# jacketsj/expANN

Measured on AMD Instinct MI355X. Metric: queries/sec at recall@10=1.0 (exact brute force), 1Mxd128 fp32, k=10, higher is better.
Workload: dtype f32; 1 GPU; brute_force_engine L2 N=1000000 d=128 fp32, 10000 batched queries, k=10 (BASELINE configs[1]); n=1000000, d=128, m=10000, k=10, metric=l2, launch=one process, one GPU, devices_visible=1, comm_ranks=0

## Files before the change

### expann_amd/csrc/expann_hip.hip

```cpp
#include "../../include/expann_hip.h"

#include <hip/hip_runtime.h>

#include <algorithm>
#include <cmath>
#include <cstdio>
#include <cstdlib>
#include <cstring>
#include <memory>
#include <mutex>
#include <string>
#include <vector>

#include "host_common.hpp"
#include "scan_f32.hpp"
#include "scan_gemm_bf16.hpp"
#include "scan_gemm_f16.hpp"
#include "scan_gemm_f16k.hpp"
#include "scan_gemm_f16x.hpp"
#include "scan_gemm_f16y.hpp"
#include "scan_gemm_f16kx.hpp"
#include "scan_gemm_f16kl.hpp"
#include "scan_direct_f16.hpp"
#include "scan_gemm_i8.hpp"
#include "scan_gemm_i8q.hpp"
#include "scan_gemm_i8x.hpp"
#include "scan_gemm_i8w.hpp"
#include "scan_int8.hpp"
#include "scan_int8_any.hpp"
#include "scan_gemm_i8kl.hpp"
#include "filter_rows.hpp"
#include "score_ids.hpp"
#include "select.hpp"

using namespace expann;

namespace expann {
thread_local std::string g_create_error;
}

namespace {

constexpr uint32_t kMaxCap = 16384;
static_assert(kMaxK == kMaxCap / 2, "the bound on k: a candidate list holds at least 2k keys");
constexpr size_t kMaxQueriesPerPass = 32768;
constexpr int kEventPairs = 64;
constexpr uint32_t kAsyncRing = 256;
constexpr uint32_t kRingWords = 10, kRingScale = 8, kRingMark = 9;
constexpr size_t kFlagCopyBytes = sizeof(uint32_t) * 7;
constexpr uint32_t kFilterListCap = kMaxCap;

struct Level {
	uint32_t n_groups_sel;
	uint32_t group_stride;
	uint32_t classmin_blocks = 0;
	uint32_t list_rows = 0;
	uint32_t list_step = 1;
};

}

struct expann_index {
	int dim = 0, dtype = 0, metric = 0, device = 0;
	size_t elem = 4;
	size_t q_elem = 4;
	int int_mode = -1;
	GrowPtr<uint8_t> d_q8;
	std::vector<unsigned char> staging;
	size_t n_staged = 0;
	void* d_base = nullptr;
	bool owns_base = false;
	size_t n = 0;
	uint64_t id_offset = 0;
	hipStream_t stream = nullptr;
	GrowPtr<uint64_t> d_cand;
	DevPtr<uint32_t> d_cnt;
	DevPtr<float> d_tau[2];
	DevPtr<float> d_tau_s;
	GrowPtr<void> d_redo;
	DevPtr<uint32_t> d_tau_row[2];
	size_t m_alloc = 0;
	DevPtr<uint32_t> d_overflow;
	unsigned long long* d_total = nullptr;
	PinPtr<uint32_t> h_flags;
	PinPtr<void> h_pin;
	bool q_in_pinned_host = false;
	DevPtr<uint32_t> d_ticket;
	size_t h_pin_bytes = 0;
	DevPtr<float> d_bnorm;
	DevPtr<float> d_bnorm_bf;
	DevPtr<float> d_bnmax;
	DevPtr<void> d_base_split;
	int u8_exact = 0;
	expann_index* u8_shadow = nullptr;
	DevPtr<void> d_base_u8;
	bool strict_u8 = false;
	double prof_extra_ms = 0;
	long opt_u8_exact = 1;
	void* d_base_i8q = nullptr;
	bool base_i8q_owned = false;
	DevPtr<int> d_bp_i8q;
	DevPtr<void> d_log;
	DevPtr<uint32_t> d_log_cnt;
	DevPtr<uint32_t> d_work_ctr;
	size_t log_bytes = 0, log_cnt_n = 0;
	struct {
		uint32_t n_logs = 0, log_cap = 0, cap = 0, n_chunks = 0, n_qtiles = 0, xcd_map = 0, m = 0;
		const float* theta = nullptr;
		float key_mul = 0.0f;
		const int *i_thp = nullptr, *i_bias = nullptr, *i_qself = nullptr;
		int i_mode = 0;
		const float* i_rw = nullptr;
	} pending_scatter;
	GrowPtr<float> d_sample;
	GrowPtr<void> d_q_split;
	DevPtr<void> d_base_f16;
	DevPtr<float> d_bnorm_f16;
	DevPtr<float> d_bns_f16;
	DevPtr<float> d_qnrm;
	DevPtr<float> d_qscale;
	float f16_scale = 0.0f;
	size_t f16_n_pad = 0;
	bool filter_on = false;
	DevPtr<uint32_t> d_filter_bits;
	size_t filter_words = 0;
	DevPtr<uint32_t> d_filter_stat;
	DevPtr<uint32_t> d_filter_list;
	uint32_t filter_list_len = 0, filter_list_stride = 1;
	size_t n_allowed = 0;
	uint32_t filter_residues = 0;
	DevPtr<float> d_bnorm_f16_m;
	DevPtr<float> d_bns_f16_m;
	bool filter_terms_valid = false;
	const float* bnorm_f16() const { return filter_on ? d_bnorm_f16_m.p : d_bnorm_f16.p; }
	const float* bns_f16() const { return filter_on ? d_bns_f16_m.p : d_bns_f16.p; }
	float f16_bnmax = 0.0f;
	DevPtr<void> d_base_i8f;
	DevPtr<int> d_bp_i8f;
	DevPtr<float> d_rw_i8f;
	DevPtr<float> d_i8f_q;
	GrowPtr<void> d_q8f;
	size_t i8f_q_m = 0;
	I8fConsts i8f{};
	int i8f_state = 0;
	DevPtr<float> d_theta;
	DevPtr<int> d_bias_i;
	DevPtr<int> d_qself;
	GrowPtr<void> d_q;
	GrowPtr<uint64_t> d_ids;
	GrowPtr<float> d_dists;
	long opt_query_tile = 0, opt_cand_capacity = 0, opt_sample_ratio = 32;
	long opt_scan_chunks = 0;
	long opt_async = 0;
	bool host_call = false;
	PinPtr<uint32_t> h_flag_ring;
	uint32_t async_pending = 0;
	hipStream_t async_stream = nullptr;
	long opt_xcd_tolerance = 3;
	long opt_latency_mode = 1;
	long opt_debug = 0;
	long opt_sample_frac = 0;
	long opt_sample_run = 1;
	long opt_sample_pass = 1;
	long opt_tail_chunks = 1;
	long opt_persist = 1;
	long opt_ip_rescale = 1;
	long opt_spec_rank = 0;
	long opt_redo_bound = 1;
	long opt_select_overlap = 1;
	hipStream_t side_stream = nullptr;
	hipEvent_t side_ev[2] = {nullptr, nullptr};
	uint64_t stat_redo_queries = 0;
	uint64_t stat_redo_candidates = 0;
	uint64_t stat_redo_overflows = 0;
	uint64_t stat_spec_rank = 0;
	long opt_i8_filter = 1;
	long opt_scan_kernel = 0;
	bool profiling = false;
	hipEvent_t ev[kEventPairs][2];
	bool ev_created = false;
	int ev_used = 0;
	expann_profile prof{};
	mutable std::string err;

	int fail(int code, const std::string& msg) const {
		err = msg;
		return code;
	}
};

inline bool f16_rows(const expann_index* h) { return h->dtype == EXPANN_DTYPE_F16; }
inline bool float_rows(const expann_index* h) { return h->dtype == EXPANN_DTYPE_F32 || f16_rows(h); }

namespace expann {
int num_cus(int device) {
	hipDeviceProp_t prop;
	if (hipGetDeviceProperties(&prop, device) != hipSuccess)
		return 256;
	return prop.multiProcessorCount > 0 ? prop.multiProcessorCount : 256;
}
}

namespace {

using ScanFn = void (*)(ScanParams);
struct ScanVariant {
	int d, tq;
	bool ip;
	ScanFn fn;
	const char* name;
	ScanFn fn_bits = nullptr;
	ScanFn fn_list = nullptr;
};
#define SCAN_V(D, TQ)                                                                      \
	{D, TQ, false, scan_filter_f32_kernel<D, TQ, false>, "scan_filter_f32<" #D "," #TQ ",L2>", \
	 scan_filter_f32_kernel<D, TQ, false, kRowsBitmap>, scan_filter_f32_kernel<D, TQ, false, kRowsList>}, \
	{D, TQ, true, scan_filter_f32_kernel<D, TQ, true>, "scan_filter_f32<" #D "," #TQ ",IP>", \
	 scan_filter_f32_kernel<D, TQ, true, kRowsBitmap>, scan_filter_f32_kernel<D, TQ, true, kRowsList>}
const ScanVariant kScanF32[] = {
    SCAN_V(64, 1),  SCAN_V(64, 4),  SCAN_V(64, 16), SCAN_V(128, 1), SCAN_V(128, 2),
    SCAN_V(128, 4), SCAN_V(128, 8), SCAN_V(128, 16), SCAN_V(256, 1), SCAN_V(256, 4),
    SCAN_V(256, 8), SCAN_V(512, 1), SCAN_V(512, 4),  SCAN_V(768, 1), SCAN_V(768, 2),
    SCAN_V(832, 1), SCAN_V(832, 2), SCAN_V(960, 1),  SCAN_V(960, 2), SCAN_V(1024, 1),
    SCAN_V(1024, 2)};
#undef SCAN_V
#define SCAN_ANY_V(TQ)                                                                           \
	{0, TQ, false, scan_filter_f32_any_kernel<TQ, false>, "scan_filter_f32_any<" #TQ ",L2>",   \
	 scan_filter_f32_any_kernel<TQ, false, kRowsBitmap>, scan_filter_f32_any_kernel<TQ, false, kRowsList>}, \
	{0, TQ, true, scan_filter_f32_any_kernel<TQ, true>, "scan_filter_f32_any<" #TQ ",IP>",     \
	 scan_filter_f32_any_kernel<TQ, true, kRowsBitmap>, scan_filter_f32_any_kernel<TQ, true, kRowsList>}
const ScanVariant kScanF32Any[] = {SCAN_ANY_V(1), SCAN_ANY_V(2), SCAN_ANY_V(4)};
#undef SCAN_ANY_V
#define SCAN_ANY_H(TQ)                                                                                              \
	{0, TQ, false, scan_filter_f32_any_kernel<TQ, false, kRowsAll, _Float16>, "scan_filter_f32_any<" #TQ ",L2,F16>", \
	 scan_filter_f32_any_kernel<TQ, false, kRowsBitmap, _Float16>, scan_filter_f32_any_kernel<TQ, false, kRowsList, _Float16>}, \
	{0, TQ, true, scan_filter_f32_any_kernel<TQ, true, kRowsAll, _Float16>, "scan_filter_f32_any<" #TQ ",IP,F16>", \
	 scan_filter_f32_any_kernel<TQ, true, kRowsBitmap, _Float16>, scan_filter_f32_any_kernel<TQ, true, kRowsList, _Float16>}
const ScanVariant kScanF16Any[] = {SCAN_ANY_H(1), SCAN_ANY_H(2), SCAN_ANY_H(4)};
#undef SCAN_ANY_H
inline bool any_dim_f32(int d) { return d >= 16 && d <= kMaxAnyDim && d % 16 == 0; }

const ScanVariant* pick_scan_f32(int d, bool ip, size_t m, long forced_tq, bool rows_f16 = false) {
	const ScanVariant* best = nullptr;
	bool compiled = false;
	for (const auto& v : kScanF32)
		compiled = compiled || (v.d == d && !rows_f16);
	if (!compiled && !any_dim_f32(d))
		return nullptr;
	static_assert(sizeof(kScanF16Any) == sizeof(kScanF32Any), "one F16 instance per run-time-dim F32 instance");
	const ScanVariant* tab = compiled ? kScanF32 : (rows_f16 ? kScanF16Any : kScanF32Any);
	const size_t n_tab = compiled ? sizeof(kScanF32) / sizeof(kScanF32[0]) : sizeof(kScanF32Any) / sizeof(kScanF32Any[0]);
	for (size_t i = 0; i < n_tab; ++i) {
		const ScanVariant& v = tab[i];
		if ((compiled && v.d != d) || v.ip != ip)
			continue;
		if (forced_tq > 0) {
			if (v.tq == forced_tq)
				return &v;
			continue;
		}
		if (!best) {
			best = &v;
			continue;
		}
		const bool v_covers = (size_t)v.tq >= m, b_covers = (size_t)best->tq >= m;
		if (v_covers && (!b_covers || v.tq < best->tq))
			best = &v;
		else if (!v_covers && !b_covers && v.tq > best->tq)
			best = &v;
	}
	return best;
}

using ScoreFn = void (*)(ScoreIdsParams);
struct ScoreVariant {
	int d;
	bool ip;
	ScoreFn fn;
};
#define SCORE_V(D) {D, false, score_ids_f32_kernel<D, false>}, {D, true, score_ids_f32_kernel<D, true>}
const ScoreVariant kScoreF32[] = {SCORE_V(64),  SCORE_V(128), SCORE_V(256), SCORE_V(512),
                                  SCORE_V(768), SCORE_V(832), SCORE_V(960), SCORE_V(1024)};
#undef SCORE_V
const ScoreVariant kScoreF32Any[] = {{0, false, score_ids_f32_any_kernel<false>}, {0, true, score_ids_f32_any_kernel<true>}};
const ScoreVariant kScoreF16Any[] = {{0, false, score_ids_f32_any_kernel<false, _Float16>},
                                     {0, true, score_ids_f32_any_kernel<true, _Float16>}};

struct ScanI8Variant {
	int d, tq, mode;
	ScanFn fn;
	const char* name;
};
#define SCAN_I8_M(D, TQ, MODE, MN) {D, TQ, MODE, scan_filter_i8_kernel<D, TQ, MODE>, "scan_filter_i8<" #D "," #TQ "," MN ">"}
#define SCAN_I8(D, TQ) SCAN_I8_M(D, TQ, kU8L2, "U8L2"), SCAN_I8_M(D, TQ, kI8L2, "I8L2"), \
	SCAN_I8_M(D, TQ, kI8L2Ref, "I8L2REF"), SCAN_I8_M(D, TQ, kI8IP, "I8IP")
#define SCAN_I16(DE, TQ) {DE, TQ, kI16L2Ref, scan_filter_i8_kernel<2 * DE, TQ, kI16L2Ref>, \
	"scan_filter_i16<" #DE "," #TQ ",L2REF>"}
const ScanI8Variant kScanI8[] = {SCAN_I8(64, 1),  SCAN_I8(64, 16), SCAN_I8(128, 1), SCAN_I8(128, 4),
                                 SCAN_I8(128, 16), SCAN_I8(256, 1), SCAN_I8(256, 8), SCAN_I8(768, 1),
                                 SCAN_I8(768, 4),  SCAN_I8(768, 8), SCAN_I8(832, 1), SCAN_I8(832, 4),
                                 SCAN_I8(960, 1),  SCAN_I8(960, 4),
                                 SCAN_I16(64, 1),  SCAN_I16(64, 4), SCAN_I16(64, 16), SCAN_I16(128, 1),
                                 SCAN_I16(128, 8)};
#undef SCAN_I16
#undef SCAN_I8
#undef SCAN_I8_M
#define SCAN_I8_ANY_M(TQ, MODE, MN) {0, TQ, MODE, scan_filter_i8_any_kernel<TQ, MODE>, "scan_filter_i8_any<" #TQ "," MN ">"}
#define SCAN_I8_ANY(TQ) SCAN_I8_ANY_M(TQ, kU8L2, "U8L2"), SCAN_I8_ANY_M(TQ, kI8L2, "I8L2"), \
	SCAN_I8_ANY_M(TQ, kI8L2Ref, "I8L2REF"), SCAN_I8_ANY_M(TQ, kI8IP, "I8IP")
const ScanI8Variant kScanI8Any[] = {SCAN_I8_ANY(1), SCAN_I8_ANY(4), SCAN_I8_ANY(8)};
#undef SCAN_I8_ANY
#undef SCAN_I8_ANY_M
inline bool any_dim_i8(int d, int mode) {
	if (mode < 0 || mode == kI16L2Ref || d < 64 || d > kMaxAnyDim || d % 64 != 0)
		return false;
	for (const auto& v : kScanI8)
		if (v.d == d && v.mode == mode)
			return false;
	return true;
}

const ScanI8Variant* pick_scan_i8(int d, int mode, size_t m, long forced_tq) {
	const ScanI8Variant* best = nullptr;
	const bool any = any_dim_i8(d, mode);
	const ScanI8Variant* tab = any ? kScanI8Any : kScanI8;
	const size_t n_tab = any ? sizeof(kScanI8Any) / sizeof(kScanI8Any[0]) : sizeof(kScanI8) / sizeof(kScanI8[0]);
// ... 317 lines not shown
	const float abs_coef = std::ldexp(1.0f, -24) / scale * std::sqrt((float)h->dim);
	const int ipm = h->metric == EXPANN_METRIC_IP ? 1 : 0;
	hipLaunchKernelGGL(f16_terms_kernel, dim3((uint32_t)((h->n + kBlock - 1) / kBlock)), dim3(kBlock),
	                   0, st, (const float*)nrm.p, (uint32_t)h->n, gemm_f16_filter_eps(h->dim), abs_coef,
	                   (const float*)nullptr, 0.5f * scale * scale, h->d_bnorm_f16, ipm, (const float*)nullptr);
	hipLaunchKernelGGL(f16_terms_kernel, dim3((uint32_t)((h->n + kBlock - 1) / kBlock)), dim3(kBlock),
	                   0, st, (const float*)nrm.p, (uint32_t)h->n, -gemm_f16_filter_eps(h->dim), -abs_coef,
	                   (const float*)nullptr, 0.5f * scale * scale, h->d_bns_f16, ipm, (const float*)nullptr);
	HIP_TRY(h, hipGetLastError());
	HIP_TRY(h, hipStreamSynchronize(st));
	h->f16_scale = scale;
	h->f16_n_pad = n_pad;
	return EXPANN_OK;
}

int ensure_filter_terms(expann_index* h, hipStream_t st) {
	if (!h->filter_on || !h->d_bnorm_f16 || (h->filter_terms_valid && h->d_bnorm_f16_m))
		return EXPANN_OK;
	if (h->f16_n_pad > h->filter_words * 32)
		return h->fail(EXPANN_ERR_HIP, "row filter: the bitmap is shorter than the fp16 copy");
	if (!h->d_bnorm_f16_m) {
		HIP_TRY(h, hipMalloc(&h->d_bnorm_f16_m, sizeof(float) * h->f16_n_pad));
		HIP_TRY(h, hipMalloc(&h->d_bns_f16_m, sizeof(float) * h->f16_n_pad));
	}
	const dim3 grid((uint32_t)std::min<size_t>((h->f16_n_pad + kBlock - 1) / kBlock, 4096));
	hipLaunchKernelGGL(filter_row_terms_kernel, grid, dim3(kBlock), 0, st, h->d_filter_bits.as<const uint32_t>(),
	                   h->d_bnorm_f16.as<const float>(), h->d_bnorm_f16_m.as<float>(), (uint32_t)h->f16_n_pad);
	hipLaunchKernelGGL(filter_row_terms_kernel, grid, dim3(kBlock), 0, st, h->d_filter_bits.as<const uint32_t>(),
	                   h->d_bns_f16.as<const float>(), h->d_bns_f16_m.as<float>(), (uint32_t)h->f16_n_pad);
	HIP_TRY(h, hipGetLastError());
	h->filter_terms_valid = true;
	return EXPANN_OK;
}
void drop_row_filter(expann_index* h) {
	h->filter_on = false;
	h->filter_terms_valid = false;
	h->d_bnorm_f16_m.reset();
	h->d_bns_f16_m.reset();
	h->d_filter_bits.reset();
	h->filter_words = 0;
	h->filter_list_len = 0;
	h->filter_list_stride = 1;
	h->n_allowed = 0;
	h->filter_residues = 0;
}

const GemmVariant* pick_gemm(const expann_index* h, size_t m) {
	if (h->opt_scan_kernel == 1 || !float_rows(h))
		return nullptr;
	if (f16_rows(h) && !f16_choice(h->opt_scan_kernel))
		return nullptr;
	if (h->metric == EXPANN_METRIC_IP) {
		const bool ok = f16_choice(h->opt_scan_kernel) && h->f16_scale >= 0.0f &&
		                !(h->opt_scan_kernel == 0 && ((m < 5 && !pick_direct_f16(h->dim, m)) || h->n < 4096));
		if (ok) {
			for (const auto& v : kGemmF16Only)
				if (v.d == h->dim)
					return &v;
			if (f16kl_dim(h->dim))
				return &kGemmF16KLOnly;
		}
		return nullptr;
	}
	bool f16_dims = f16kl_dim(h->dim) && h->f16_scale >= 0.0f;
	for (const auto& v : kGemmF16Only)
		f16_dims = f16_dims || (v.d == h->dim && h->f16_scale >= 0.0f);
	if (h->opt_scan_kernel == 0 &&
	    ((m < (f16_dims ? 5u : 24u) && !(f16_dims && pick_direct_f16(h->dim, m))) || h->n < 4096))
		return nullptr;
	for (const auto& v : kGemmF32)
		if (v.d == h->dim)
			return &v;
	if (f16_choice(h->opt_scan_kernel)) {
		for (const auto& v : kGemmF16Only)
			if (v.d == h->dim)
				return &v;
		if (f16kl_dim(h->dim))
			return &kGemmF16KLOnly;
	}
	return nullptr;
}

int ensure_bnorm(expann_index* h, const GemmVariant* gv, bool bf16, hipStream_t st) {
	DevPtr<float>& dst = bf16 ? h->d_bnorm_bf : h->d_bnorm;
	const uint32_t blocks = (uint32_t)((h->n + kRowsPerGroup - 1) / kRowsPerGroup);
	if (!dst) {
		HIP_TRY(h, hipMalloc(&dst, sizeof(float) * h->n));
		const float eps = bf16 ? gemm_bf16_filter_eps(h->dim) : gemm_filter_eps(h->dim);
		hipLaunchKernelGGL(gv->norms, dim3(blocks), dim3(kBlock), 0, st, (const float*)h->d_base,
		                   (uint32_t)h->n, 1.0f - eps, dst);
		if (!h->d_bnmax)
			HIP_TRY(h, hipMalloc(&h->d_bnmax, 4 * sizeof(float)));
		hipLaunchKernelGGL(max_f32_kernel, dim3(1), dim3(1024), 0, st, (const float*)dst, h->n,
		                   h->d_bnmax + (bf16 ? 1 : 0));
		HIP_TRY(h, hipGetLastError());
	}
	if (bf16 && !h->d_base_split) {
		const size_t nv = h->n * (size_t)h->dim;
		HIP_TRY(h, hipMalloc(&h->d_base_split, nv * 4));
		hipLaunchKernelGGL(split_bf16_kernel, dim3((uint32_t)((nv + kBlock - 1) / kBlock)),
		                   dim3(kBlock), 0, st, (const float*)h->d_base, h->n, h->dim,
		                   h->d_base_split.as<__bf16>());
		HIP_TRY(h, hipGetLastError());
	}
	return EXPANN_OK;
}

using GemmI8Fn = void (*)(GemmI8Params);
using SelfI8Fn = void (*)(const void*, uint32_t, int*);
using ThetaI8Fn = void (*)(const void*, uint32_t, const float*, int*, int*);
struct GemmI8Variant {
	int d, mode;
	GemmI8Fn scan;
	SelfI8Fn self;
	ThetaI8Fn theta;
	const char* name;
};
#define GEMM_I8(D, MODE, MN) {D, MODE, scan_gemm_i8_kernel<D, MODE>, row_self_i8_kernel<D, MODE>, \
	query_theta_i8_kernel<D, MODE>, "scan_gemm_i8<" #D "," MN ">"}
const GemmI8Variant kGemmI8[] = {
    GEMM_I8(128, kU8L2, "U8L2"), GEMM_I8(128, kI8L2, "I8L2"), GEMM_I8(128, kI8IP, "I8IP"),
    GEMM_I8(256, kU8L2, "U8L2"), GEMM_I8(256, kI8L2, "I8L2"), GEMM_I8(256, kI8IP, "I8IP"),
    GEMM_I8(768, kU8L2, "U8L2"), GEMM_I8(768, kI8L2, "I8L2"), GEMM_I8(768, kI8IP, "I8IP")};
#undef GEMM_I8

const GemmI8Variant* pick_gemm_i8(const expann_index* h, size_t m) {
	if (h->opt_scan_kernel == 1 || float_rows(h))
		return nullptr;
	if (h->opt_scan_kernel == 0 && (m < 96 || h->n < 4096))
		return nullptr;
	for (const auto& v : kGemmI8)
		if (v.d == h->dim && v.mode == h->int_mode)
			return &v;
	return nullptr;
}

int ensure_bias_i8(expann_index* h, const GemmI8Variant* gv, hipStream_t st) {
	if (h->d_bias_i || h->int_mode == kI8IP)
		return EXPANN_OK;
	HIP_TRY(h, hipMalloc(&h->d_bias_i, sizeof(int) * h->n));
	const uint32_t blocks = (uint32_t)((h->n + kRowsPerGroup - 1) / kRowsPerGroup);
	hipLaunchKernelGGL(gv->self, dim3(blocks), dim3(kBlock), 0, st, (const void*)h->d_base,
	                   (uint32_t)h->n, h->d_bias_i);
	HIP_TRY(h, hipGetLastError());
	return EXPANN_OK;
}

uint32_t select_longest_list(double expect, uint32_t spec_j) {
	return spec_j ? (uint32_t)(expect * (1.0 + 4.5 / std::sqrt((double)spec_j))) : 2u * (uint32_t)expect;
}
void launch_select_wave(SelectParams& sel, size_t m, uint32_t cap, hipStream_t st, uint32_t longest, bool rows_f16 = false,
                        hipStream_t side = nullptr) {
	using WaveFn = void (*)(SelectParams, uint32_t);
	const WaveFn w8 = rows_f16 ? select_wave_kernel<8, 4, _Float16> : select_wave_kernel<8, 4>;
	const WaveFn w16 = rows_f16 ? select_wave_kernel<16, 2, _Float16> : select_wave_kernel<16, 2>;
	const WaveFn w32 = rows_f16 ? select_wave_kernel<32, 1, _Float16> : select_wave_kernel<32, 1>;
	const hipStream_t st2 = side ? side : st;
	sel.wave_done = 0;
	hipLaunchKernelGGL(w8, dim3((uint32_t)((m + 3) / 4)), dim3(256), 0, st, sel, (uint32_t)m);
	sel.wave_done = 512;
	if (longest <= 512)
		return;
	if (cap > 512) {
		hipLaunchKernelGGL(w16, dim3((uint32_t)((m + 1) / 2)), dim3(128), 0, st2, sel, (uint32_t)m);
		sel.wave_done = 1024;
	}
	if (cap > 1024 && longest > 1024) {
		hipLaunchKernelGGL(w32, dim3((uint32_t)m), dim3(64), 0, st2, sel, (uint32_t)m);
		sel.wave_done = 2048;
	}
}
using SelectTopkFn = void (*)(SelectParams);
inline SelectTopkFn select_topk_fn(const expann_index* h) {
	return f16_rows(h) ? select_topk_kernel<_Float16> : select_topk_kernel<float>;
}
int launch_select(expann_index* h, SelectParams& sel, size_t m, uint32_t cap, hipStream_t st, uint32_t longest,
                  bool sum_counts) {
	hipStream_t side = nullptr;
	if (h->opt_select_overlap && longest > 512 && cap > 512) {
		if (!h->side_stream) {
			HIP_TRY(h, hipStreamCreateWithFlags(&h->side_stream, hipStreamNonBlocking));
			for (hipEvent_t& e : h->side_ev)
				HIP_TRY(h, hipEventCreateWithFlags(&e, hipEventDisableTiming));
		}
		side = h->side_stream;
		HIP_TRY(h, hipEventRecord(h->side_ev[0], st));
		HIP_TRY(h, hipStreamWaitEvent(side, h->side_ev[0], 0));
	}
	const hipStream_t st2 = side ? side : st;
	if (sum_counts)
		hipLaunchKernelGGL(sum_u32_kernel, dim3(1), dim3(1024), 0, st2, sel.cand_cnt, (uint32_t)m, h->d_total);
	launch_select_wave(sel, m, cap, st, longest, f16_rows(h), side);
	hipLaunchKernelGGL(select_topk_fn(h), dim3((uint32_t)m), dim3(kBlock), sizeof(uint64_t) * cap + 16, st2, sel);
	HIP_TRY(h, hipGetLastError());
	if (side) {
		HIP_TRY(h, hipEventRecord(h->side_ev[1], side));
		HIP_TRY(h, hipStreamWaitEvent(st, h->side_ev[1], 0));
	}
	return EXPANN_OK;
}

int ensure_hit_logs(expann_index* h, uint32_t grid, int waves, size_t m, uint32_t cap, uint32_t n_chunks,
                    uint32_t n_qtiles, uint32_t xcd_map, hipStream_t st, uint4** log, uint32_t** log_cnt,
                    uint32_t* log_cap_out) {
	const uint32_t n_logs = grid * (uint32_t)waves;
	const uint32_t log_cap = std::max<uint32_t>(
	    4096, pow2ceil((uint32_t)std::min<size_t>(4 * ((m * (size_t)cap + n_logs - 1) / n_logs), 1u << 20)));
	const size_t need = (size_t)n_logs * log_cap * 16;
	if (need > h->log_bytes || n_logs > h->log_cnt_n) {
		HIP_TRY(h, hipStreamSynchronize(st));
		h->d_log.reset();
		h->d_log_cnt.reset();
		h->log_bytes = h->log_cnt_n = 0;
		HIP_TRY(h, hipMalloc(&h->d_log, need));
		HIP_TRY(h, hipMalloc(&h->d_log_cnt, sizeof(uint32_t) * n_logs));
		h->log_bytes = need;
		h->log_cnt_n = n_logs;
	}
	*log = h->d_log.as<uint4>();
	*log_cnt = h->d_log_cnt;
	*log_cap_out = log_cap;
	h->pending_scatter.n_logs = n_logs;
	h->pending_scatter.log_cap = log_cap;
	h->pending_scatter.cap = cap;
	h->pending_scatter.n_chunks = n_chunks;
	h->pending_scatter.n_qtiles = n_qtiles;
	h->pending_scatter.xcd_map = xcd_map;
	h->pending_scatter.m = (uint32_t)m;
	h->pending_scatter.theta = nullptr;
	h->pending_scatter.key_mul = 0.0f;
	h->pending_scatter.i_mode = 0;
	return EXPANN_OK;
}

void launch_gather_logs(expann_index* h, hipStream_t st) {
	if (!h->pending_scatter.n_logs)
		return;
	const auto ps = h->pending_scatter;
	h->pending_scatter.n_logs = 0;
	const uint32_t want = std::max<uint32_t>(1, (1024 + ps.n_qtiles * 4 - 1) / (ps.n_qtiles * 4));
	const uint32_t cpb = std::max<uint32_t>(1, (ps.n_chunks + want - 1) / want);
	const uint32_t n_groups = (ps.n_chunks + cpb - 1) / cpb;
	GatherLogParams gp{h->d_log.as<const uint4>(), h->d_log_cnt.as<const uint32_t>(), ps.log_cap, ps.n_chunks,
	                   ps.n_qtiles, ps.xcd_map, ps.m, n_groups, cpb, h->d_cnt, h->d_cand, ps.cap, ps.theta, ps.key_mul,
	                   ps.i_thp, ps.i_bias, ps.i_qself, ps.i_mode, ps.i_rw};
	hipLaunchKernelGGL(gather_logs_kernel, dim3(ps.n_qtiles * 4 * n_groups), dim3(kBlock), 0, st, gp);
}

bool defer_flags(expann_index* h, hipStream_t st, int attempt) {
	if (!h->opt_async || h->host_call || attempt != 0 || h->strict_u8 || h->async_pending >= kAsyncRing)
		return false;
	if (hipMemcpyAsync(h->h_flag_ring + kRingWords * h->async_pending, h->d_overflow, kFlagCopyBytes,
	                   hipMemcpyDeviceToHost, st) != hipSuccess)
		return false;
	h->h_flag_ring[kRingWords * h->async_pending + kRingScale] = 0;
	h->h_flag_ring[kRingWords * h->async_pending + kRingMark] = h->dtype == EXPANN_DTYPE_U8 ? 1u : 0u;
	h->async_pending++;
	h->async_stream = st;
	h->prof.deferred_searches++;
	return true;
}

uint32_t pick_row_chunks(uint32_t n_tiles, uint32_t n_qtiles, uint32_t slots, double overhead, uint32_t min_tiles,
                         uint32_t g_limit, long tol_pct, uint32_t* xcd) {
	const uint32_t gmax = std::max<uint32_t>(1, n_tiles / min_tiles);
	uint32_t chunks = 1, g8 = 0;
	double best = 1e300, best8 = 1e300;
	for (uint32_t g = 1; g <= std::min<uint32_t>(gmax, g_limit); ++g) {
		const uint32_t steps = (n_tiles + g - 1) / g;
		const uint64_t rounds = ((uint64_t)g * n_qtiles + slots - 1) / slots;
		const double cost = (double)rounds * (steps + overhead);
		if (cost < best * 0.999) {
			best = cost;
			chunks = g;
		}
		if (xcd && g % 8 == 0 && cost < best8 * 0.999 && (n_tiles + steps - 1) / steps == g) {
			best8 = cost;
			g8 = g;
		}
	}
	if (xcd) {
		*xcd = 0;
		if (g8 && best8 <= best * (1.0 + 0.01 * (double)tol_pct)) {
			chunks = g8;
			*xcd = 1;
		}
	}
	return chunks;
}

bool pick_tail_chunks(uint32_t n_tiles, uint32_t g, uint32_t n_qtiles, uint32_t slots, uint32_t min_tiles,
                      uint32_t* tiles_big, uint32_t* n_big, uint32_t* tiles_small, uint32_t* n_small) {
	const uint64_t rounds = ((uint64_t)g * n_qtiles + slots - 1) / slots;
	if (rounds < 3 || g % 8 != 0 || g < 24)
		return false;
	uint32_t nb = (uint32_t)(((rounds - 1) * slots / n_qtiles) / 8) * 8;
	nb = std::min(nb, g - 8);
	if (nb < 8)
		return false;
	const uint32_t ns = (3 * (g - nb) + 7) / 8 * 8;
	const uint32_t big = (uint32_t)(((uint64_t)n_tiles * 3 + (3 * nb + ns) - 1) / (3 * nb + ns));
	if ((uint64_t)nb * big >= n_tiles)
		return false;
	const uint32_t rest = n_tiles - nb * big;
	const uint32_t small = (rest + ns - 1) / ns;
	if (small < min_tiles || (uint64_t)(ns - 1) * small >= rest)
		return false;
	*tiles_big = big;
	*n_big = nb;
	*tiles_small = small;
	*n_small = ns;
	return true;
}

constexpr double kSpecFailTarget = 0.01;
double spec_fail_share(size_t k, double f, uint32_t j) {
	if (j == 0)
		return 1.0;
	if (k <= 1 || j > k - 1)
		return 0.0;
	f = std::min(1.0, std::max(0.0, f));
	const double n = (double)(k - 1);
	double term = std::pow(1.0 - f, n), below = 0.0;
	for (uint32_t i = 0; i < j; ++i) {
		below += term;
		term = f < 1.0 ? term * (n - i) / (i + 1.0) * f / (1.0 - f) : 0.0;
	}
	return f < 1.0 ? std::max(0.0, 1.0 - below) : 1.0;
}
uint32_t spec_rank_auto(size_t k, double f) {
	for (uint32_t j = 1; j < k; ++j)
		if (spec_fail_share(k, f, j) <= kSpecFailTarget)
			return j;
	return (uint32_t)k;
}
uint32_t spec_redo_slots(size_t m) {
	const size_t want = (size_t)std::ceil(4.0 * kSpecFailTarget * (double)m);
	return (uint32_t)(std::max<size_t>(1, (want + kF16TQ - 1) / kF16TQ) * kF16TQ);
}

uint32_t sample_frac_for(const expann_index* h, size_t k) {
	if (h->opt_sample_frac > 0)
		return (uint32_t)h->opt_sample_frac;
	const double expo = float_rows(h) ? 0.3 : 0.5;
	const double bytes = (double)h->n * (double)h->dim * (float_rows(h) ? 2.0 : 1.0);
	double size = (bytes >= 8 * 2.56e8 && k <= 32) ? std::min(3.0, std::pow(bytes / 2.56e8, 0.3)) : 1.0;
// ... 600 lines not shown
	fp.n_tiles_sel = nt;
	fp.tile_stride = 1;
	fp.tile_run = 1;
	fp.n_qtiles = nqt;
	fp.queries = h->d_q8f;
	fp.thp = reinterpret_cast<const int*>(h->d_i8f_q + 3 * h->i8f_q_m);
	fp.m = (uint32_t)m;
	fp.cand_cnt = h->d_cnt;
	fp.cand = h->d_cand;
	fp.cap = cap;
	uint32_t fchunks = pick_row_chunks(nt, nqt, (uint32_t)gs->wg_per_cu_w * (uint32_t)cus, 4.0, 8, 2048,
	                                   h->opt_xcd_tolerance, (h->opt_debug & 1024) ? nullptr : &fp.xcd_map);
	fp.tiles_per_block = (nt + fchunks - 1) / fchunks;
	fchunks = (nt + fp.tiles_per_block - 1) / fp.tiles_per_block;
	GemmI8wParams wp{};
	wp.q = fp;
	const int rc = ensure_hit_logs(h, fchunks * nqt, 4, m, cap, fchunks, nqt, fp.xcd_map, st, &wp.log, &wp.log_cnt,
	                               &wp.log_cap);
	if (rc != EXPANN_OK)
		return rc;
	wp.lost = h->d_overflow;
	h->pending_scatter.i_thp = fp.thp;
	h->pending_scatter.i_bias = fp.bp;
	h->pending_scatter.i_qself = nullptr;
	h->pending_scatter.i_rw = h->d_rw_i8f;
	h->pending_scatter.i_mode = 3;
	hipLaunchKernelGGL(gs->scan_w, dim3(fchunks * nqt), dim3((uint32_t)gs->threads_w), gs->lds_w, st, wp);
	return EXPANN_OK;
}

int launch_scan_f16(expann_index* h, const GemmF16Variant* gvf, uint32_t rows_sel, bool last, size_t m, int cus,
                    bool ip, uint32_t cap, hipStream_t st, const char** kname, uint32_t* n_qtiles,
                    uint32_t* query_tile) {
	*query_tile = (uint32_t)gvf->wgq;
	GemmF16Params fp{};
	fp.base_f16 = h->d_base_f16;
	fp.bnorm = h->bnorm_f16();
	fp.n_rows = (uint32_t)h->n;
	const uint32_t nt = (uint32_t)((h->n + gvf->tb - 1) / gvf->tb);
	fp.n_tiles_sel = last ? nt : std::min(nt, (rows_sel + gvf->tb - 1) / gvf->tb);
	fp.tile_stride = std::max<uint32_t>(1, nt / fp.n_tiles_sel);
	fp.tile_run = 1;
	if (!last && fp.tile_stride >= 16 && fp.n_tiles_sel >= 16) {
		fp.tile_run = 16;
		fp.n_tiles_sel = (fp.n_tiles_sel / 16) * 16;
	}
	fp.n_qtiles = (uint32_t)((m + gvf->wgq - 1) / gvf->wgq);
	uint32_t fchunks = pick_row_chunks(fp.n_tiles_sel, fp.n_qtiles, (uint32_t)gvf->wg_per_cu * (uint32_t)cus,
	                                   4.0, 8, 2048, h->opt_xcd_tolerance,
	                                   (h->opt_debug & 1024) ? nullptr : &fp.xcd_map);
	if (h->opt_scan_chunks > 0) {
		fchunks = (uint32_t)std::min<long>(h->opt_scan_chunks, std::max<uint32_t>(1, fp.n_tiles_sel / 8));
		fp.xcd_map = (fchunks % 8 == 0 && !(h->opt_debug & 1024)) ? 1 : 0;
		const uint32_t tpb = (fp.n_tiles_sel + fchunks - 1) / fchunks;
		if ((fp.n_tiles_sel + tpb - 1) / tpb != fchunks)
			fp.xcd_map = 0;
	}
	fp.tiles_per_block = (fp.n_tiles_sel + fchunks - 1) / fchunks;
	fchunks = (fp.n_tiles_sel + fp.tiles_per_block - 1) / fp.tiles_per_block;
	if (gvf->hit_log && fp.xcd_map && h->opt_tail_chunks && !h->opt_scan_chunks) {
		uint32_t big, nb, small, ns;
		if (pick_tail_chunks(fp.n_tiles_sel, fchunks, fp.n_qtiles, (uint32_t)gvf->wg_per_cu * (uint32_t)cus, 64, &big, &nb,
		                     &small, &ns)) {
			fp.tiles_per_block = big;
			fp.n_big = nb;
			fp.tiles_small = small;
			fchunks = nb + ns;
		}
	}
	fp.queries_f16 = h->d_q_split;
	fp.ksteps = (uint32_t)f16_ld(h->dim) / 32;
	fp.theta = h->d_theta;
	fp.two_inv_s2 = (ip ? 1.0f : 2.0f) / (h->f16_scale * h->f16_scale);
	fp.m = (uint32_t)m;
	fp.cand_cnt = h->d_cnt;
	fp.cand = h->d_cand;
	fp.cap = cap;
	fp.debug = (uint32_t)h->opt_debug & ~16u;
	DevBuf clk;
	if (h->opt_debug & 16) {
		HIP_TRY(h, clk.alloc((18 + 3 * 65536) * 8));
		HIP_TRY(h, hipMemsetAsync(clk.p, 0, (18 + 3 * 65536) * 8, st));
		fp.clk = clk.as<unsigned long long>();
	}
	const DirectF16Variant* dv =
	    (last && h->opt_scan_kernel == 0) ? pick_direct_f16(h->dim, m) : nullptr;
	if (dv) {
		fp.n_qtiles = (uint32_t)((m + dv->tq - 1) / dv->tq);
		fp.n_tiles_sel = (uint32_t)((h->n + dv->rps - 1) / dv->rps);
		const uint32_t want = std::max<uint32_t>(1, (16u * (uint32_t)cus) / fp.n_qtiles);
		fp.tiles_per_block = std::max<uint32_t>(8, (fp.n_tiles_sel + want - 1) / want);
		fchunks = (fp.n_tiles_sel + fp.tiles_per_block - 1) / fp.tiles_per_block;
		fp.xcd_map = 0;
		hipLaunchKernelGGL(dv->fn, dim3(fchunks * fp.n_qtiles), dim3(kBlock), 0, st, fp);
		*kname = dv->name;
		*query_tile = (uint32_t)dv->tq;
	} else {
		const uint32_t grid = fchunks * fp.n_qtiles;
		if (gvf->hit_log) {
			const int lrc = ensure_hit_logs(h, grid, gvf->threads / 64, m, cap, fchunks, fp.n_qtiles, fp.xcd_map, st,
			                                &fp.log, &fp.log_cnt, &fp.log_cap);
			if (lrc != EXPANN_OK)
				return lrc;
			fp.lost = h->d_overflow;
			h->pending_scatter.theta = fp.theta;
			h->pending_scatter.key_mul = fp.two_inv_s2;
		}
		uint32_t launch_grid = grid;
		const uint32_t resident = (uint32_t)gvf->wg_per_cu * (uint32_t)cus;
		if (gvf->hit_log && gvf->d == 128 && h->opt_persist && grid > resident &&
		    (fp.tiles_per_block >= 160 || h->opt_persist > 1)) {
			if (!h->d_work_ctr)
				HIP_TRY(h, hipMalloc(&h->d_work_ctr, sizeof(uint32_t) * 8 * 16));
			HIP_TRY(h, hipMemsetAsync(h->d_work_ctr, 0, sizeof(uint32_t) * 8 * 16, st));
			fp.work_ctr = h->d_work_ctr;
			fp.n_items = grid;
			launch_grid = resident;
		}
		hipLaunchKernelGGL(gvf->scan, dim3(launch_grid), dim3((uint32_t)gvf->threads), gvf->lds, st, fp);
		*kname = gvf->name;
	}
	*n_qtiles = fp.n_qtiles;
	if (fp.clk) {
		int occ = -1;
		hipOccupancyMaxActiveBlocksPerMultiprocessor(&occ, (const void*)gvf->scan, gvf->threads, gvf->lds);
		std::fprintf(stderr, "scan_gemm_f16: %d workgroups per CU resident, grid %u\n", occ,
		             fchunks * fp.n_qtiles);
		unsigned long long c[18] = {0};
		HIP_TRY(h, hipMemcpy(c, fp.clk, sizeof(c), hipMemcpyDeviceToHost));
		std::fprintf(stderr, "scan_gemm_f16 wg0: %llu shader clocks in %.1f us = %.0f MHz\n", c[0],
		             c[1] / 100.0, c[1] ? c[0] * 100.0 / c[1] : 0.0);
		if (c[6])
			std::fprintf(stderr, "  per step (%llu steps): columns 0-1 %.0f, stage wait + barrier %.0f, columns 2-3 %.0f, tail + queue work %.0f cycles\n",
			             c[6], (double)c[2] / c[6], (double)c[3] / c[6], (double)c[4] / c[6], (double)c[5] / c[6]);
		if (const char* dump = std::getenv("EXPANN_WG_TIMES")) {
			const uint32_t grid = std::min<uint32_t>(fchunks * fp.n_qtiles, 65536);
			std::vector<unsigned long long> rec(3 * (size_t)grid);
			HIP_TRY(h, hipMemcpy(rec.data(), fp.clk + 18, rec.size() * 8, hipMemcpyDeviceToHost));
			if (FILE* f = std::fopen(dump, "w")) {
				for (uint32_t b = 0; b < grid; ++b)
					std::fprintf(f, "%u %llu %llu %llu\n", b, rec[3 * b], rec[3 * b + 1], rec[3 * b + 2]);
				std::fclose(f);
			}
		}
		if (c[14])
			std::fprintf(stderr, "scan_gemm_f16 last wg: %llu shader clocks in %.1f us = %.0f MHz, started %.1f us after wg0; per step (%llu): %.0f / %.0f / %.0f / %.0f\n",
			             c[8], c[9] / 100.0, c[9] ? c[8] * 100.0 / c[9] : 0.0, (double)(c[15] - c[7]) / 100.0, c[14],
			             (double)c[10] / c[14], (double)c[11] / c[14], (double)c[12] / c[14], (double)c[13] / c[14]);
	}
	return EXPANN_OK;
}

struct RedoWs {
	size_t list, cnt, theta, qnrm, wq, thp, bound, q16, q8, cand, total;
	RedoWs(uint32_t R, int dim, uint32_t cap) {
		list = 0;
		cnt = 4 * (size_t)R;
		theta = 8 * (size_t)R;
		qnrm = 12 * (size_t)R;
		wq = 16 * (size_t)R;
		thp = 20 * (size_t)R;
		bound = 24 * (size_t)R;
		q16 = 28 * (size_t)R;
		q8 = q16 + 2 * (size_t)R * (size_t)dim;
		cand = q8 + (size_t)R * (size_t)dim;
		total = cand + 8 * (size_t)R * (size_t)cap;
	}
};
bool spec_auto_region(const expann_index* h, size_t m, size_t k, bool i8f) {
	(void)h;
	if (m < 4096)
		return false;
	return i8f || k > 32;
}

struct ScanSel {
	ScanFn fn = nullptr;
	int tq = 0;
	const char* name = "";
	ScanFn fn_bits = nullptr, fn_list = nullptr;
};
struct SearchPass {
	expann_index* h;
	const void* d_queries;
	size_t m, k;
	uint64_t* d_ids;
	float* d_dists;
	hipStream_t st;
	bool ip;
	int cus;
	uint32_t cap;
	ScanSel svs;
	const ScanSel* sv = &svs;
	const GemmVariant* gv = nullptr;
	const GemmI8Variant* gvi = nullptr;
	const GemmBf16Variant* gvb = nullptr;
	const GemmF16Variant* gvf = nullptr;
	bool i8f = false;
	bool i8f_ready = false;
	bool i8f_off = false;
	bool i8f_ran = false;
	bool flags_clean = false;
	bool force_direct = false;
	bool no_f16 = false;
	std::vector<Level> levels;
	uint32_t n_qtiles = 0;
	size_t li_start = 0;
	bool theta_ready = false;
	uint32_t spec_j = 0;
	bool spec_off = false;
	uint32_t redo_slots = 0;

	enum Next { kDone, kRestart, kRetry };
	int choose_kernels();
	int prepare_queries(bool* restart);
	int plan_thresholds();
	int run_level(size_t li);
	int run_redo(bool use_i8f);
	int check(int attempt, Next* next);
	int run();
};

int SearchPass::choose_kernels() {
	const bool filt = h->filter_on;
	gv = force_direct ? nullptr : pick_gemm(h, m);
	if (filt && (no_f16 || !f16_choice(h->opt_scan_kernel) || h->n_allowed <= cap))
		gv = nullptr;
	gvi = force_direct ? nullptr : pick_gemm_i8(h, m);
	gvb = nullptr;
	gvf = nullptr;
	if (h->opt_scan_kernel == 2 && !gvi)
		return h->fail(EXPANN_ERR_UNSUPPORTED,
		               "GEMM-form scan (scan_kernel=2): 8-bit L2/IP with dim 128/256/768 (the fp32-input MFMA form of "
		               "rounds 1-2 is gone: scan_kernel 3 = bf16x3, 4 = fp16)");
	if (gvi) {
		int rc = ensure_bias_i8(h, gvi, st);
		if (rc != EXPANN_OK)
			return rc;
	}
	if (gv && h->dtype == EXPANN_DTYPE_F32)
		for (const auto& v : kGemmBf16)
			if (v.d == h->dim)
				gvb = &v;
	if (h->opt_scan_kernel == 3 && !gvb && !filt && !f16_rows(h))
		return h->fail(EXPANN_ERR_UNSUPPORTED, "bf16x3 GEMM-form scan: f32 L2 with dim 64 or 128 only");
	if (gv && !no_f16 && f16_choice(h->opt_scan_kernel)) {
		const bool dbg = (h->opt_debug & ~16L) != 0;
		for (const auto& v : kGemmF16X)
			if (v.d == h->dim && !(dbg && v.d == kGemmF16XDbg[0].d))
				gvf = &v;
		if (dbg && kGemmF16XDbg[0].d == h->dim)
			gvf = &kGemmF16XDbg[0];
		if (!gvf && f16kl_dim(h->dim))
			gvf = &kGemmF16KL;
	}
	i8f = gvf && !i8f_off && !filt && i8f_wanted(h, m, k);
	if (filt && !gvf)
		gv = nullptr;
	if ((h->opt_scan_kernel == 4 || h->opt_scan_kernel == 6) && !gvf && !no_f16 && !(filt && h->n_allowed <= cap))
		return h->fail(EXPANN_ERR_UNSUPPORTED, "fp16 GEMM-form scan: f32 with dim a multiple of 16 from 64 to 4096 only");
	if (gvf)
		gvb = nullptr;
	else if ((h->opt_scan_kernel == 0 && m < 24) || !gvb)
		gv = nullptr, gvb = nullptr;
	if (gv && !gvf) {
		int rc = ensure_bnorm(h, gv, gvb != nullptr, st);
		if (rc != EXPANN_OK)
			return rc;
	}
	return EXPANN_OK;
}

int SearchPass::prepare_queries(bool* restart) {
	*restart = false;
	if (gvf) {
		int rc = ensure_f16(h, gvf, st);
		if (rc != EXPANN_OK)
			return rc;
		if (h->f16_scale < 0.0f) {
			no_f16 = true;
			*restart = true;
			return EXPANN_OK;
		}
		rc = ensure_filter_terms(h, st);
		if (rc != EXPANN_OK)
			return rc;
		rc = ensure_workspace(h, m, cap);
		if (rc != EXPANN_OK)
			return rc;
		I8fQueryArgs qa{};
		if (i8f) {
			rc = ensure_i8f(h, st);
			if (rc != EXPANN_OK)
				return rc;
			i8f = h->i8f_state > 0;
			if (i8f && h->opt_cand_capacity <= 0)
				cap = std::max<uint32_t>(cap, 4096);
		}
		if (i8f) {
			HIP_TRY(h, grow_ws(h, h->d_q8f, m * (size_t)h->dim));
			if (m > h->i8f_q_m) {
				if (h->async_pending > 0)
					HIP_TRY(h, hipStreamSynchronize(h->async_stream));
				h->d_i8f_q.reset();
				h->i8f_q_m = 0;
				HIP_TRY(h, hipMalloc(&h->d_i8f_q, 4 * sizeof(float) * m));
				h->i8f_q_m = m;
			}
			qa.q8 = h->d_q8f.as<int8_t>();
			qa.aq = h->d_i8f_q;
			qa.wq = h->d_i8f_q + h->i8f_q_m;
			qa.k = h->i8f;
		}
		const size_t nv = m * (size_t)h->dim;
		HIP_TRY(h, grow_ws(h, h->d_q_split, nv * 4));
		const bool one_wg = m <= (size_t)kRowsPerGroup;
		const bool from_host = h->q_in_pinned_host && one_wg;
		if (!one_wg)
			HIP_TRY(h, hipMemsetAsync(h->d_overflow, 0, 32, st));
		flags_clean = true;
		const dim3 prep_grid((uint32_t)((m + kRowsPerGroup - 1) / kRowsPerGroup));
		const float* ip_ref = (ip && h->opt_ip_rescale) ? (const float*)(h->d_bnmax + 2) : (const float*)nullptr;
		if (gvf->d == 0)
			hipLaunchKernelGGL(f16_query_prep_any_kernel, prep_grid, dim3(kBlock), 0, st, (const float*)d_queries,
			                   (uint32_t)m, (uint32_t)h->dim, (uint32_t)f16_ld(h->dim), h->f16_scale,
			                   h->d_q_split.as<_Float16>(), h->d_qnrm, h->d_overflow + 2,
			                   from_host ? h->d_q.as<float>() : (float*)nullptr, one_wg ? h->d_overflow : (uint32_t*)nullptr,
			                   ip_ref, h->d_qscale.as<float>());
		else
			hipLaunchKernelGGL(gvf->prep, prep_grid, dim3(kBlock), 0, st, (const float*)d_queries, (uint32_t)m,
			                   h->f16_scale, h->d_q_split.as<_Float16>(), h->d_qnrm, h->d_overflow + 2,
			                   from_host ? h->d_q.as<float>() : (float*)nullptr, one_wg ? h->d_overflow : (uint32_t*)nullptr,
			                   ip_ref, h->d_qscale.as<float>(), qa);
		HIP_TRY(h, hipGetLastError());
		if (from_host) {
			d_queries = h->d_q;
			h->q_in_pinned_host = false;
		}
	}
	if (gvb) {
		const size_t nv = m * (size_t)h->dim;
		HIP_TRY(h, grow_ws(h, h->d_q_split, nv * 4));
		hipLaunchKernelGGL(split_bf16_kernel, dim3((uint32_t)((nv + kBlock - 1) / kBlock)),
		                   dim3(kBlock), 0, st, (const float*)d_queries, m, h->dim,
		                   h->d_q_split.as<__bf16>());
		HIP_TRY(h, hipGetLastError());
	}
	return EXPANN_OK;
}

int SearchPass::plan_thresholds() {
	int rc = ensure_workspace(h, m, cap);
	if (rc != EXPANN_OK)
		return rc;
	const bool filt = h->filter_on;
	levels = filt ? plan_levels_filtered(h->n, h->n_allowed, h->filter_list_len, k, cap, h->opt_sample_ratio)
	              : plan_levels(h->n, k, cap, h->opt_sample_ratio);
	n_qtiles = (uint32_t)((m + sv->tq - 1) / sv->tq);
	if (!gv && !gvi && levels.size() >= 3 && h->opt_sample_pass && !filt) {
		const uint32_t n_groups = (uint32_t)((h->n + kRowsPerGroup - 1) / kRowsPerGroup);
		const uint32_t sel = n_groups / 16;
		uint32_t blocks = std::min<uint32_t>({128u, cap / 16, sel / 8});
		if (blocks * 16 >= 8 * k && blocks >= 16) {
			Level l0;
// ... 96 lines not shown
			hipLaunchKernelGGL(gv->theta, dim3((uint32_t)((m + kRowsPerGroup - 1) / kRowsPerGroup)),
			                   dim3(kBlock), 0, st, (const float*)d_queries, (uint32_t)m,
			                   (const float*)sp.tau,
			                   1.0f - (gvb ? gemm_bf16_filter_eps(h->dim) : gemm_filter_eps(h->dim)),
			                   h->d_theta);
		GemmScanParams gp{};
		gp.base = (const float*)h->d_base;
		gp.bnorm = h->d_bnorm;
		gp.n_rows = (uint32_t)h->n;
		const uint32_t n_tiles = (uint32_t)((h->n + kGemmTB - 1) / kGemmTB);
		gp.n_tiles_sel = last ? n_tiles
		                      : std::min(n_tiles, (L.n_groups_sel * kRowsPerGroup + kGemmTB - 1) / kGemmTB);
		gp.tile_stride = std::max<uint32_t>(1, n_tiles / gp.n_tiles_sel);
		const uint32_t tq_wg = gvf ? (uint32_t)gvf->wgq : (gvb ? kGemmBf16TQ : kGemmTQ);
		uint32_t tq_small = 0;
		gp.n_qtiles = (uint32_t)((m + tq_wg - 1) / tq_wg);
		gp.queries = (const float*)d_queries;
		gp.theta = h->d_theta;
		gp.m = (uint32_t)m;
		gp.cand_cnt = h->d_cnt;
		gp.cand = h->d_cand;
		gp.cap = cap;
		uint32_t gchunks = pick_row_chunks(gp.n_tiles_sel, gp.n_qtiles, (uint32_t)cus, 2.0, 4, 1024, 0, nullptr);
		gp.tiles_per_block = (gp.n_tiles_sel + gchunks - 1) / gchunks;
		gchunks = (gp.n_tiles_sel + gp.tiles_per_block - 1) / gp.tiles_per_block;
		if (timed)
			HIP_TRY(h, hipEventRecord(h->ev[h->ev_used][0], st));
		if (use_i8f) {
			const int rl = launch_scan_i8f(h, m, cus, cap, st);
			if (rl != EXPANN_OK)
				return rl;
			kname = kGemmI8F.name;
			gp.n_qtiles = (uint32_t)((m + kF16TQ - 1) / kF16TQ);
		} else if (gvf) {
			const int rl = launch_scan_f16(h, gvf, L.n_groups_sel * kRowsPerGroup, last, m, cus, ip, cap, st, &kname,
			                               &gp.n_qtiles, &tq_small);
			if (rl != EXPANN_OK)
				return rl;
		} else if (gvb) {
			GemmBf16Params bp{};
			bp.base_split = h->d_base_split;
			bp.bnorm = h->d_bnorm_bf;
			bp.n_rows = gp.n_rows;
			bp.n_tiles_sel = gp.n_tiles_sel;
			bp.tile_stride = gp.tile_stride;
			bp.tile_run = 1;
			if (!last && gp.tile_stride >= 8) {
				bp.tile_run = 8;
				bp.n_tiles_sel = (gp.n_tiles_sel / 8) * 8;
				if (bp.n_tiles_sel == 0) {
					bp.n_tiles_sel = gp.n_tiles_sel;
					bp.tile_run = 1;
				}
			}
			bp.tiles_per_block = gp.tiles_per_block;
			bp.n_qtiles = gp.n_qtiles;
			bp.queries_split = h->d_q_split;
			bp.theta = gp.theta;
			bp.m = gp.m;
			bp.cand_cnt = gp.cand_cnt;
			bp.cand = gp.cand;
			bp.cap = gp.cap;
			bp.debug = (uint32_t)h->opt_debug;
			hipLaunchKernelGGL(gvb->scan, dim3(gchunks * gp.n_qtiles), dim3(kGemmThreads),
			                   2 * kGemmTB * h->dim * sizeof(float), st, bp);
			kname = gvb->name;
		} else {
			return h->fail(EXPANN_ERR_UNSUPPORTED, "no GEMM-form scan kernel for this index");
		}
		passes = gp.n_qtiles;
		qt_used = tq_small ? tq_small : tq_wg;
	} else if (gvi && !first) {
		hipLaunchKernelGGL(gvi->theta, dim3((uint32_t)((m + kRowsPerGroup - 1) / kRowsPerGroup)),
		                   dim3(kBlock), 0, st, d_queries, (uint32_t)m, (const float*)sp.tau,
		                   h->d_theta.as<int>(), h->d_qself);
		const uint32_t tb = (uint32_t)gemm_i8_tb(h->dim);
		GemmI8Params gp{};
		gp.base = h->d_base;
		gp.bias = h->d_bias_i;
		gp.n_rows = (uint32_t)h->n;
		const uint32_t n_tiles = (uint32_t)((h->n + tb - 1) / tb);
		gp.n_tiles_sel = last ? n_tiles
		                      : std::min(n_tiles, (L.n_groups_sel * kRowsPerGroup + tb - 1) / tb);
		gp.tile_stride = std::max<uint32_t>(1, n_tiles / gp.n_tiles_sel);
		gp.n_qtiles = (uint32_t)((m + kGemmI8TQ - 1) / kGemmI8TQ);
		gp.queries = d_queries;
		gp.theta = h->d_theta.as<const int>();
		gp.qself = h->d_qself;
		gp.m = (uint32_t)m;
		gp.cand_cnt = h->d_cnt;
		gp.cand = h->d_cand;
		gp.cap = cap;
		uint32_t gchunks = pick_row_chunks(gp.n_tiles_sel, gp.n_qtiles, (uint32_t)cus, 2.0, 4, 4096, 0, nullptr);
		gp.tiles_per_block = (gp.n_tiles_sel + gchunks - 1) / gchunks;
		gchunks = (gp.n_tiles_sel + gp.tiles_per_block - 1) / gp.tiles_per_block;
		if (timed)
			HIP_TRY(h, hipEventRecord(h->ev[h->ev_used][0], st));
		hipLaunchKernelGGL(gvi->scan, dim3(gchunks * gp.n_qtiles), dim3(kGemmThreads),
		                   2 * tb * h->dim, st, gp);
		passes = gp.n_qtiles;
		kname = gvi->name;
		qt_used = kGemmI8TQ;
	} else {
		if (timed)
			HIP_TRY(h, hipEventRecord(h->ev[h->ev_used][0], st));
		hipLaunchKernelGGL(scan_fn, dim3(n_chunks * n_qtiles), dim3(kBlock), 0, st, sp);
	}
	if (timed) {
		HIP_TRY(h, hipEventRecord(h->ev[h->ev_used][1], st));
		h->ev_used++;
	}
	launch_gather_logs(h, st);
	if (last && (timed || !h->profiling)) {
		h->prof.scan_launches++;
		h->prof.scan_rows += h->n;
		h->prof.scan_query_tiles += passes;
		h->prof.query_tile = qt_used;
		h->prof.levels = (uint32_t)(levels.size() - li_start + (li_start ? 1 : 0));
		std::snprintf(h->prof.scan_kernel, sizeof(h->prof.scan_kernel), "%s", kname);
	}
	HIP_TRY(h, hipGetLastError());

	SelectParams sel{};
	sel.cand = h->d_cand;
	sel.cand_cnt = first ? nullptr : h->d_cnt;
	sel.fixed_count = (first && L.classmin_blocks) ? n_chunks * 16 : L.n_groups_sel * kRowsPerGroup;
	sel.cap = cap;
	sel.k = (uint32_t)k;
	sel.id_offset = h->id_offset;
	sel.out_ids = last ? d_ids : nullptr;
	sel.out_dists = last ? d_dists : nullptr;
	sel.tau_out = last ? nullptr : h->d_tau[li & 1];
	sel.tau_prev = first ? nullptr : h->d_tau[(li + 1) & 1];
	sel.tau_row_out = last ? nullptr : h->d_tau_row[li & 1];
	sel.tau_row_prev = first ? nullptr : h->d_tau_row[(li + 1) & 1];
	sel.rerank_base = use_gemm ? (const float*)h->d_base : nullptr;
	sel.rerank_queries = use_gemm ? (const float*)d_queries : nullptr;
	sel.dim = (uint32_t)h->dim;
	sel.metric_ip = ip ? 1u : 0u;
	const float pr = ip ? 1.0f : 2.0f;
	sel.prune_eps = use_gemm ? (gvf ? pr * gemm_f16_filter_eps(h->dim)
	                                : (gvb ? gemm_bf16_filter_eps(h->dim) : gemm_filter_eps(h->dim)))
	                         : 0.0f;
	sel.prune_abs = (use_gemm && gvf)
	                    ? pr * std::ldexp(1.0f, -24) / h->f16_scale * std::sqrt((float)h->dim)
	                    : 0.0f;
	sel.bn_max = h->d_bnmax ? h->d_bnmax + (gvf ? 2 : (gvb ? 1 : 0)) : nullptr;
	sel.qnrm = (use_gemm && gvf) ? h->d_qnrm : nullptr;
	if (use_i8f) {
		sel.prune_eps = 0.0f;
		sel.prune_abs = 0.0f;
		sel.row_w = h->d_rw_i8f;
		sel.q_w = h->d_i8f_q + 2 * h->i8f_q_m;
	}
	sel.overflow = h->d_overflow;
	if (last && spec_j) {
		const RedoWs ws(redo_slots, h->dim, cap);
		sel.spec_tau = h->d_tau_s;
		sel.redo_word = h->d_overflow + 3;
		sel.redo_list = reinterpret_cast<uint32_t*>(h->d_redo.as<unsigned char>() + ws.list);
		sel.redo_cap = redo_slots;
		sel.redo_bound = reinterpret_cast<float*>(h->d_redo.as<unsigned char>() + ws.bound);
	}
	const bool sum_counts = last && sel.cand_cnt && (h->profiling || use_i8f);
	if (m > 64 && sel.rerank_base && sel.cand_cnt) {
		const uint32_t sj = last ? spec_j : 0u;
		const double expect = (use_i8f ? kI8fListRatio : 1.0) * 1.2 * (sj ? (double)sj : (double)k) * sample_frac_for(h, k);
		const int rs = launch_select(h, sel, m, cap, st, select_longest_list(expect, sj), sum_counts);
		if (rs != EXPANN_OK)
			return rs;
	} else {
		if (sum_counts)
			hipLaunchKernelGGL(sum_u32_kernel, dim3(1), dim3(1024), 0, st, sel.cand_cnt, (uint32_t)m, h->d_total);
		if (m <= 64)
			sel.wave0_short = 1;
		hipLaunchKernelGGL(select_topk_fn(h), dim3((uint32_t)m), dim3(kBlock), sizeof(uint64_t) * cap + 16, st, sel);
		HIP_TRY(h, hipGetLastError());
	}
	if (last && spec_j)
		return run_redo(use_i8f);
	return EXPANN_OK;
}

int SearchPass::run_redo(bool use_i8f) {
	const RedoWs ws(redo_slots, h->dim, cap);
	unsigned char* const b = h->d_redo.as<unsigned char>();
	uint32_t* const word = h->d_overflow + 3;
	const uint32_t R = redo_slots;
	RedoCompactParams cp{};
	cp.word = word;
	cp.list = reinterpret_cast<const uint32_t*>(b + ws.list);
	cp.n_slots = R;
	cp.row_bytes = (uint32_t)h->dim * 2;
	cp.q16 = h->d_q_split;
	cp.rq16 = b + ws.q16;
	cp.qnrm = h->d_qnrm;
	cp.r_qnrm = reinterpret_cast<float*>(b + ws.qnrm);
	cp.tau = h->d_tau[levels.size() & 1];
	cp.bound = h->opt_redo_bound ? reinterpret_cast<const float*>(b + ws.bound) : nullptr;
	cp.qscale = (ip && h->opt_ip_rescale) ? h->d_qscale.as<const float>() : nullptr;
	cp.eps = gemm_f16_filter_eps(h->dim);
	cp.abs_coef = std::ldexp(1.0f, -24) / h->f16_scale * std::sqrt((float)h->dim);
	cp.mul = 0.5f * h->f16_scale * h->f16_scale;
	cp.ip = ip ? 1 : 0;
	cp.r_theta = reinterpret_cast<float*>(b + ws.theta);
	cp.r_cnt = reinterpret_cast<uint32_t*>(b + ws.cnt);
	if (use_i8f) {
		cp.q8 = h->d_q8f;
		cp.rq8 = b + ws.q8;
		cp.i8_aq = h->d_i8f_q;
		cp.i8_wq_in = h->d_i8f_q + h->i8f_q_m;
		cp.r_thp = reinterpret_cast<int*>(b + ws.thp);
		cp.r_wq = reinterpret_cast<float*>(b + ws.wq);
		cp.i8_inv_2s2 = h->i8f.inv_2s2;
	}
	hipLaunchKernelGGL(redo_compact_kernel, dim3(R / (kBlock / 64)), dim3(kBlock), 0, st, cp);

	const uint32_t nt = (uint32_t)((h->n + kF16TB - 1) / kF16TB);
	const uint32_t nqt = R / kF16TQ;
	const uint32_t wg_per_cu = use_i8f ? (uint32_t)kGemmI8F.wg_per_cu_w : (uint32_t)gvf->wg_per_cu;
	uint32_t chunks = pick_row_chunks(nt, 1, wg_per_cu * (uint32_t)cus, 4.0, 8, 2048, 0, nullptr);
	chunks = std::min<uint32_t>(chunks, (uint32_t)(h->log_cnt_n / (4 * (size_t)nqt)));
	if (chunks == 0 || !h->d_log)
		return h->fail(EXPANN_ERR_HIP, "redo pass: the main scan left no hit logs");
	const uint32_t tpb = (nt + chunks - 1) / chunks;
	chunks = (nt + tpb - 1) / tpb;
	const uint32_t n_logs = chunks * nqt * 4;
	const uint32_t log_cap = (uint32_t)std::min<size_t>(1u << 16, h->log_bytes / ((size_t)n_logs * 16));
	GatherLogParams gp{};
	gp.log = h->d_log.as<const uint4>();
	gp.log_cnt = h->d_log_cnt.as<const uint32_t>();
	gp.log_cap = log_cap;
	gp.n_chunks = chunks;
	gp.n_qtiles = nqt;
	gp.m = R;
	gp.cand_cnt = cp.r_cnt;
	gp.cand = reinterpret_cast<uint64_t*>(b + ws.cand);
	gp.cap = cap;
	gp.live_q = word;
	if (use_i8f) {
		GemmI8wParams wp{};
		wp.q.base = h->d_base_i8f;
		wp.q.bp = h->d_bp_i8f;
		wp.q.n_rows = (uint32_t)h->n;
		wp.q.n_tiles_sel = nt;
		wp.q.tile_stride = 1;
		wp.q.tile_run = 1;
		wp.q.tiles_per_block = tpb;
		wp.q.n_qtiles = nqt;
		wp.q.queries = cp.rq8;
		wp.q.thp = cp.r_thp;
		wp.q.m = R;
		wp.q.cand_cnt = gp.cand_cnt;
		wp.q.cand = gp.cand;
		wp.q.cap = cap;
		wp.q.live_q = word;
		wp.log = h->d_log.as<uint4>();
		wp.log_cnt = h->d_log_cnt;
		wp.log_cap = log_cap;
		wp.lost = h->d_overflow;
		hipLaunchKernelGGL(kGemmI8FRedo, dim3(chunks * nqt), dim3((uint32_t)kGemmI8F.threads_w), kGemmI8F.lds_w, st, wp);
		gp.i_thp = cp.r_thp;
		gp.i_bias = h->d_bp_i8f;
		gp.i_rw = h->d_rw_i8f;
		gp.i_mode = 3;
	} else {
		GemmF16Params fp{};
		fp.base_f16 = h->d_base_f16;
		fp.bnorm = h->bnorm_f16();
		fp.n_rows = (uint32_t)h->n;
		fp.n_tiles_sel = nt;
		fp.tile_stride = 1;
		fp.tile_run = 1;
		fp.tiles_per_block = tpb;
		fp.n_qtiles = nqt;
		fp.queries_f16 = cp.rq16;
		fp.theta = cp.r_theta;
		fp.two_inv_s2 = (ip ? 1.0f : 2.0f) / (h->f16_scale * h->f16_scale);
		fp.m = R;
		fp.cand_cnt = gp.cand_cnt;
		fp.cand = gp.cand;
		fp.cap = cap;
		fp.ksteps = (uint32_t)f16_ld(h->dim) / 32;
		fp.log = h->d_log.as<uint4>();
		fp.log_cnt = h->d_log_cnt;
		fp.log_cap = log_cap;
		fp.lost = h->d_overflow;
		fp.live_q = word;
		hipLaunchKernelGGL(gvf->scan_redo, dim3(chunks * nqt), dim3((uint32_t)gvf->threads), gvf->lds, st, fp);
		gp.theta = cp.r_theta;
		gp.key_mul = fp.two_inv_s2;
	}
	const uint32_t want = std::max<uint32_t>(1, (1024 + nqt * 4 - 1) / (nqt * 4));
	gp.chunks_per_block = std::max<uint32_t>(1, (chunks + want - 1) / want);
	gp.n_groups = (chunks + gp.chunks_per_block - 1) / gp.chunks_per_block;
	hipLaunchKernelGGL(gather_logs_kernel, dim3(nqt * 4 * gp.n_groups), dim3(kBlock), 0, st, gp);

	SelectParams sel{};
	sel.cand = gp.cand;
	sel.cand_cnt = gp.cand_cnt;
	sel.cap = cap;
	sel.k = (uint32_t)k;
	sel.id_offset = h->id_offset;
	sel.out_ids = d_ids;
	sel.out_dists = d_dists;
	sel.rerank_base = (const float*)h->d_base;
	sel.rerank_queries = (const float*)d_queries;
	sel.dim = (uint32_t)h->dim;
	sel.metric_ip = ip ? 1u : 0u;
	const float pr = ip ? 1.0f : 2.0f;
	sel.bn_max = h->d_bnmax + 2;
	sel.qnrm = cp.r_qnrm;
	if (use_i8f) {
		sel.row_w = h->d_rw_i8f;
		sel.q_w = cp.r_wq;
	} else {
		sel.prune_eps = pr * gemm_f16_filter_eps(h->dim);
		sel.prune_abs = pr * std::ldexp(1.0f, -24) / h->f16_scale * std::sqrt((float)h->dim);
	}
	sel.overflow = word;
	sel.wave0_short = 1;
	sel.slot_map = cp.list;
	sel.live_slots = word;
	sel.redo_cand = h->d_overflow + 6;
	hipLaunchKernelGGL(select_topk_fn(h), dim3(R), dim3(kBlock), sizeof(uint64_t) * cap + 16, st, sel);
	HIP_TRY(h, hipGetLastError());
	return EXPANN_OK;
}

int SearchPass::check(int attempt, Next* next) {
	*next = kDone;
	if (defer_flags(h, st, attempt)) {
		float sc = gvf ? h->f16_scale : 0.0f;
		uint32_t* const slot = h->h_flag_ring + kRingWords * (h->async_pending - 1);
		std::memcpy(&slot[kRingScale], &sc, sizeof(float));
		if (i8f_ran && h->opt_i8_filter == 1)
			slot[kRingMark] = 0x80000000u | (uint32_t)std::min<uint64_t>(i8f_cand_limit(h, m, k, spec_j), 0x3FFFFFFFu);
		if (spec_j)
			slot[kRingMark] |= 0x40000000u;
		return EXPANN_OK;
	}
	HIP_TRY(h, hipMemcpyAsync(h->h_flags, h->d_overflow, kFlagCopyBytes, hipMemcpyDeviceToHost, st));
	HIP_TRY(h, hipStreamSynchronize(st));
	unsigned long long tot;
	std::memcpy(&tot, h->h_flags + 4, sizeof(tot));
	h->prof.candidates = tot;
	if (i8f_ran && h->opt_i8_filter == 1 && tot > i8f_cand_limit(h, m, k, spec_j))
		h->i8f_state = 2;
	if (std::getenv("EXPANN_DEBUG_LISTS")) {
		std::vector<uint32_t> cnt(m);
		HIP_TRY(h, hipMemcpy(cnt.data(), h->d_cnt, sizeof(uint32_t) * m, hipMemcpyDeviceToHost));
		std::sort(cnt.begin(), cnt.end());
		std::fprintf(stderr, "[lists] attempt %d cap %u: min %u median %u p90 %u p99 %u max %u, overflow flag %u\n", attempt, cap,
		             cnt.front(), cnt[m / 2], cnt[m * 9 / 10], cnt[m * 99 / 100], cnt.back(), h->h_flags[0]);
	}
	if (gvf) {
		float qmax;
		std::memcpy(&qmax, &h->h_flags[2], sizeof(float));
		if (!(qmax * h->f16_scale <= 60000.0f)) {
			no_f16 = true;
			h->prof.retries++;
			*next = kRestart;
			return EXPANN_OK;
		}
	}
	if (h->strict_u8 && (h->h_flags[1] != 0 || h->h_flags[3] != 0))
		return kStrictReject;
	if (h->dtype == EXPANN_DTYPE_U8 && h->h_flags[1] != 0)
		return h->fail(EXPANN_ERR_UNSUPPORTED,
		               std::to_string(h->h_flags[1]) +
		                   " query values outside [0,255]: the uint8 metric "
		                   "(dist2_compressed) is only defined for 8-bit valued queries");
	const uint32_t redo_word = spec_j ? h->h_flags[3] : 0u;
	if (h->h_flags[0] == 0 && redo_word < kRedoOverflowUnit) {
		h->stat_redo_queries += redo_word;
		h->stat_redo_candidates += spec_j ? h->h_flags[6] : 0u;
		return EXPANN_OK;
	}
	h->prof.retries++;
	if (spec_j) {
		spec_off = true;
		if (redo_word >= kRedoOverflowUnit)
			h->stat_redo_overflows++;
		if (h->h_flags[0] == 0) {
			*next = kRestart;
			return EXPANN_OK;
		}
	}
	if (i8f_ran) {
		i8f_off = true;
		*next = kRestart;
		return EXPANN_OK;
	}
	if ((cap >= kMaxCap || attempt >= 3) && (gv || gvi) && h->opt_scan_kernel == 0) {
		force_direct = true;
		*next = kRestart;
		return EXPANN_OK;
	}
	if (cap >= kMaxCap || attempt >= 3)
		return h->fail(EXPANN_ERR_OVERFLOW,
		               "candidate lists overflowed (" + std::to_string(h->h_flags[0]) +
		                   " queries) at capacity " + std::to_string(cap) +
		                   "; the data has more near-ties than the threshold filter supports");
	cap = std::min(cap * 4, kMaxCap);
	*next = kRetry;
	return EXPANN_OK;
}

int SearchPass::run() {
	for (;;) {
		int rc = choose_kernels();
		if (rc != EXPANN_OK)
			return rc;
		bool restart = false;
		rc = prepare_queries(&restart);
		if (rc != EXPANN_OK)
			return rc;
		if (restart)
			continue;
		Next next = kDone;
		for (int attempt = 0;; ++attempt) {
			rc = ensure_workspace(h, m, cap);
			if (rc == EXPANN_OK)
				rc = plan_thresholds();
			for (size_t li = li_start; rc == EXPANN_OK && li < levels.size(); ++li)
				rc = run_level(li);
			if (rc == EXPANN_OK)
				rc = check(attempt, &next);
			if (rc != EXPANN_OK || next != kRetry)
				break;
		}
		if (rc != EXPANN_OK || next == kDone)
			return rc;
	}
}

int search_pass(expann_index* h, const void* d_queries, size_t m, size_t k, uint64_t* d_ids,
                float* d_dists, hipStream_t st) {
	const bool ip = (h->metric == EXPANN_METRIC_IP);
	if (h->filter_on && h->n_allowed == 0) {
		hipLaunchKernelGGL(fill_pad_kernel, dim3((uint32_t)std::min<size_t>((m * k + kBlock - 1) / kBlock, 1024)), dim3(kBlock),
		                   0, st, d_ids, d_dists, m * k);
		HIP_TRY(h, hipGetLastError());
		if (!h->opt_async || h->host_call)
			HIP_TRY(h, hipStreamSynchronize(st));
		return EXPANN_OK;
	}
	if (h->dtype == EXPANN_DTYPE_F32 && !ip && h->opt_scan_kernel == 0 && h->opt_u8_exact && !h->filter_on &&
	    (h->dim == 128 || h->dim == 256) && m >= 96 && h->n >= 65536 && k <= 256 && h->u8_exact >= 0) {
		if (h->u8_exact == 0) {
			const int rb = build_u8_shadow(h, st);
			if (rb != EXPANN_OK)
				return rb;
		}
		if (h->u8_exact == 1) {
			const int rq = search_pass(h->u8_shadow, d_queries, m, k, d_ids, d_dists, st);
			const int ra = absorb_shadow_profile(h);
			if (rq == EXPANN_OK)
				return ra;
			if (rq != kStrictReject)
				return h->fail(rq, h->u8_shadow->err);
		}
	}
	ScanSel svs;
	if (float_rows(h)) {
		const ScanVariant* v = pick_scan_f32(h->dim, ip, m, h->opt_query_tile, f16_rows(h));
		if (v)
			svs = ScanSel{v->fn, v->tq, v->name, v->fn_bits, v->fn_list};
	} else {
		const ScanI8Variant* v = pick_scan_i8(h->dim, h->int_mode, m, h->opt_query_tile);
		if (v)
			svs = ScanSel{v->fn, v->tq, v->name};
	}
	if (!svs.fn)
		return h->fail(EXPANN_ERR_UNSUPPORTED,
		               "no scan kernel for dim " + std::to_string(h->dim) +
		                   " / query_tile " + std::to_string(h->opt_query_tile));
	if (h->dtype == EXPANN_DTYPE_U8) {
		const size_t nv = m * (size_t)h->dim;
		HIP_TRY(h, grow_ws(h, h->d_q8, nv));
		int rcw = ensure_workspace(h, m, 2048);
		if (rcw != EXPANN_OK)
			return rcw;
		HIP_TRY(h, hipMemsetAsync(h->d_overflow + 1, 0, sizeof(uint32_t), st));
		HIP_TRY(h, hipMemsetAsync(h->d_overflow + 3, 0, sizeof(uint32_t), st));
		hipLaunchKernelGGL(u8_query_prep_kernel, dim3((uint32_t)((nv + kBlock - 1) / kBlock)),
		                   dim3(kBlock), 0, st, (const float*)d_queries, nv, h->d_q8,
		                   h->d_overflow + 1, h->strict_u8 ? h->d_overflow + 3 : (uint32_t*)nullptr);
		HIP_TRY(h, hipGetLastError());
		d_queries = h->d_q8;
	}
	uint32_t cap = h->opt_cand_capacity > 0
	                   ? (uint32_t)h->opt_cand_capacity
	                   : pow2ceil((uint32_t)std::max<size_t>(2048, 64 * k));
	cap = std::min(pow2ceil(cap), kMaxCap);
	if (h->opt_cand_capacity > 0 && (size_t)cap < 2 * k)
		cap = std::min(pow2ceil((uint32_t)(2 * k)), kMaxCap);
	if ((size_t)cap < 2 * k)
		return h->fail(EXPANN_ERR_UNSUPPORTED, k_too_large());
	const int cus = num_cus(h->device);
	if (const GemmI8qVariant* gq = pick_gemm_i8q(h, m, k)) {
		const int rq = search_i8q(h, gq, d_queries, m, k, d_ids, d_dists, st, cap);
		if (rq != kRetryGeneric)
			return rq;
	}
	SearchPass pass{h, d_queries, m, k, d_ids, d_dists, st, ip, cus, cap, svs};
	return pass.run();
}

}

extern "C" {

int expann_abi_version(void) { return EXPANN_ABI_VERSION; }

int expann_device_count(void) {
	int n = 0;
	if (hipGetDeviceCount(&n) != hipSuccess)
		return 0;
	return n;
}

int expann_create(int dim, int dtype, int metric, int device, expann_index** out) {
	if (!out) {
		g_create_error = "out == NULL";
		return EXPANN_ERR_INVALID_ARG;
	}
	*out = nullptr;
	if (dim <= 0 || dim % 16 != 0) {
		g_create_error = "dim must be a positive multiple of 16 (the reference kernels require it)";
		return EXPANN_ERR_INVALID_ARG;
	}
	int int_mode = -1;
	if (dtype == EXPANN_DTYPE_F32 || dtype == EXPANN_DTYPE_F16) {
		if (metric != EXPANN_METRIC_L2 && metric != EXPANN_METRIC_IP) {
			g_create_error = "metric must be EXPANN_METRIC_L2 or EXPANN_METRIC_IP for f32 / f16 rows";
			return EXPANN_ERR_INVALID_ARG;
		}
		if (dim > kMaxAnyDim) {
			g_create_error = "unsupported dim " + std::to_string(dim) + ": f32 / f16 rows take dim <= " +
			                 std::to_string(kMaxAnyDim);
			return EXPANN_ERR_UNSUPPORTED;
		}
	} else if (dtype == EXPANN_DTYPE_U8) {
		if (metric != EXPANN_METRIC_L2) {
			g_create_error = "uint8 rows support EXPANN_METRIC_L2 only (dist2_compressed)";
			return EXPANN_ERR_INVALID_ARG;
		}
		int_mode = kU8L2;
	} else if (dtype == EXPANN_DTYPE_I16) {
		if (metric != EXPANN_METRIC_L2) {
			g_create_error = "int16 rows support EXPANN_METRIC_L2 only (src/distance.h:14-27 semantics)";
			return EXPANN_ERR_INVALID_ARG;
		}
		int_mode = kI16L2Ref;
	} else if (dtype == EXPANN_DTYPE_I8) {
		if (metric == EXPANN_METRIC_L2)
			int_mode = kI8L2;
		else if (metric == EXPANN_METRIC_IP)
			int_mode = kI8IP;
		else if (metric == EXPANN_METRIC_L2_I8_REFCOMPAT)
			int_mode = kI8L2Ref;
		else {
			g_create_error = "unknown metric for int8 rows";
			return EXPANN_ERR_INVALID_ARG;
		}
	} else {
		g_create_error = "unknown dtype";
		return EXPANN_ERR_INVALID_ARG;
	}
	if (int_mode >= 0 && dim % 64 != 0) {
		g_create_error = "8-bit rows need dim % 64 == 0 (src/distance.h:29-53, antitopo_engine.h:726)";
		return EXPANN_ERR_INVALID_ARG;
	}
	if (int_mode >= 0 && int_mode != kI16L2Ref && dim > kMaxAnyDim) {
		g_create_error = "unsupported dim " + std::to_string(dim) + ": 8-bit rows take dim <= " +
		                 std::to_string(kMaxAnyDim);
		return EXPANN_ERR_UNSUPPORTED;
	}
	int ndev = expann_device_count();
	if (ndev <= 0) {
		g_create_error = "no HIP device visible: libexpann_hip has no CPU fallback";
		return EXPANN_ERR_NO_DEVICE;
	}
	if (device < 0 || device >= ndev) {
		g_create_error = "device index out of range";
		return EXPANN_ERR_INVALID_ARG;
	}
	if ((int_mode < 0 && !pick_scan_f32(dim, metric == EXPANN_METRIC_IP, 1, 0, dtype == EXPANN_DTYPE_F16)) ||
	    (int_mode >= 0 && !pick_scan_i8(dim, int_mode, 1, 0))) {
		g_create_error = "unsupported dim " + std::to_string(dim) +
		                 " (built: f32 any multiple of 16 up to 4096; 8-bit any multiple of 64 up to 4096; int16 64,128)";
		return EXPANN_ERR_UNSUPPORTED;
	}
	expann_index* h = new expann_index();
	h->dim = dim;
	h->dtype = dtype;
	h->metric = metric;
	h->device = device;
	h->elem = (dtype == EXPANN_DTYPE_F32) ? 4 : ((dtype == EXPANN_DTYPE_I16 || dtype == EXPANN_DTYPE_F16) ? 2 : 1);
	h->q_elem = (dtype == EXPANN_DTYPE_I8) ? 1 : (dtype == EXPANN_DTYPE_I16 ? 2 : 4);
	h->int_mode = int_mode;
	if (const char* e = std::getenv("EXPANN_TAIL_CHUNKS"))
		h->opt_tail_chunks = std::atol(e);
	if (const char* e = std::getenv("EXPANN_PERSIST"))
		h->opt_persist = std::atol(e);
	if (const char* e = std::getenv("EXPANN_SPEC_RANK"))
		h->opt_spec_rank = std::max(0L, std::atol(e));
	if (const char* e = std::getenv("EXPANN_REDO_BOUND"))
		h->opt_redo_bound = std::atol(e);
	if (const char* e = std::getenv("EXPANN_SELECT_OVERLAP"))
		h->opt_select_overlap = std::atol(e);
	if (const char* e = std::getenv("EXPANN_I8_FILTER"))
		h->opt_i8_filter = std::min(2L, std::max(0L, std::atol(e)));
	if (hipSetDevice(device) != hipSuccess || hipStreamCreate(&h->stream) != hipSuccess) {
		g_create_error = "hipSetDevice/hipStreamCreate failed";
		delete h;
		return EXPANN_ERR_HIP;
	}
	if (hipFuncSetAttribute((const void*)select_topk_kernel<float>, hipFuncAttributeMaxDynamicSharedMemorySize,
	                        (int)(sizeof(uint64_t) * kMaxCap + 16)) != hipSuccess ||
	    hipFuncSetAttribute((const void*)select_topk_kernel<_Float16>, hipFuncAttributeMaxDynamicSharedMemorySize,
	                        (int)(sizeof(uint64_t) * kMaxCap + 16)) != hipSuccess) {
		g_create_error = "hipFuncSetAttribute(select_topk_kernel) failed";
		hipStreamDestroy(h->stream);
		delete h;
		return EXPANN_ERR_HIP;
	}
	for (const auto& v : kGemmF16X)
		if (v.d == dim &&
		    (hipFuncSetAttribute((const void*)v.scan, hipFuncAttributeMaxDynamicSharedMemorySize, v.lds) != hipSuccess ||
		     hipFuncSetAttribute((const void*)v.sample, hipFuncAttributeMaxDynamicSharedMemorySize, v.lds) != hipSuccess ||
		     (v.scan_redo &&
		      hipFuncSetAttribute((const void*)v.scan_redo, hipFuncAttributeMaxDynamicSharedMemorySize, v.lds) != hipSuccess))) {
			g_create_error = "hipFuncSetAttribute(scan_gemm_f16x_kernel) failed";
			hipStreamDestroy(h->stream);
			delete h;
			return EXPANN_ERR_HIP;
		}
	if ((dtype == EXPANN_DTYPE_F32 || dtype == EXPANN_DTYPE_F16) && f16kl_dim(dim) &&
	    (hipFuncSetAttribute((const void*)kGemmF16KL.scan, hipFuncAttributeMaxDynamicSharedMemorySize, kGemmF16KL.lds) != hipSuccess ||
	     hipFuncSetAttribute((const void*)kGemmF16KL.sample, hipFuncAttributeMaxDynamicSharedMemorySize, kGemmF16KL.lds) != hipSuccess)) {
		g_create_error = "hipFuncSetAttribute(scan_gemm_f16kl_kernel) failed";
		hipStreamDestroy(h->stream);
		delete h;
		return EXPANN_ERR_HIP;
	}
	for (const auto* tab : {kGemmF16XDbg})
		if (tab[0].d == dim)
			if (hipFuncSetAttribute((const void*)tab[0].scan, hipFuncAttributeMaxDynamicSharedMemorySize, tab[0].lds) !=
			    hipSuccess) {
				g_create_error = "hipFuncSetAttribute(scan_gemm_f16x_kernel) failed";
				hipStreamDestroy(h->stream);
				delete h;
				return EXPANN_ERR_HIP;
			}
	for (const auto& v : kGemmI8x)
		if (v.d == dim &&
		    (hipFuncSetAttribute((const void*)v.scan, hipFuncAttributeMaxDynamicSharedMemorySize, v.lds) != hipSuccess ||
		     hipFuncSetAttribute((const void*)v.sample, hipFuncAttributeMaxDynamicSharedMemorySize, v.lds) != hipSuccess)) {
			g_create_error = "hipFuncSetAttribute(scan_gemm_i8x_kernel) failed";
			hipStreamDestroy(h->stream);
			delete h;
			return EXPANN_ERR_HIP;
		}
	for (const auto& v : kGemmI8w)
		if (v.d == dim &&
		    (hipFuncSetAttribute((const void*)v.scan_w, hipFuncAttributeMaxDynamicSharedMemorySize, v.lds_w) != hipSuccess ||
		     hipFuncSetAttribute((const void*)v.sample_w, hipFuncAttributeMaxDynamicSharedMemorySize, v.lds_w) != hipSuccess)) {
			g_create_error = "hipFuncSetAttribute(scan_gemm_i8w_kernel) failed";
			hipStreamDestroy(h->stream);
			delete h;
			return EXPANN_ERR_HIP;
		}
	if (dim == kGemmI8F.d && hipFuncSetAttribute((const void*)kGemmI8FRedo, hipFuncAttributeMaxDynamicSharedMemorySize,
	                                             kGemmI8F.lds_w) != hipSuccess) {
		g_create_error = "hipFuncSetAttribute(scan_gemm_i8w_kernel, redo instance) failed";
		hipStreamDestroy(h->stream);
		delete h;
		return EXPANN_ERR_HIP;
	}
	if (any_dim_i8(dim, int_mode))
		for (const auto& v : kGemmI8KL)
			if (v.mode == int_mode &&
			    (hipFuncSetAttribute((const void*)v.scan_w, hipFuncAttributeMaxDynamicSharedMemorySize, v.lds_w) != hipSuccess ||
			     hipFuncSetAttribute((const void*)v.sample_w, hipFuncAttributeMaxDynamicSharedMemorySize, v.lds_w) != hipSuccess)) {
				g_create_error = "hipFuncSetAttribute(scan_gemm_i8kl_kernel) failed";
				hipStreamDestroy(h->stream);
				delete h;
				return EXPANN_ERR_HIP;
			}
	for (const auto& v : kGemmBf16)
		if (v.d == dim)
			if (hipFuncSetAttribute((const void*)v.scan, hipFuncAttributeMaxDynamicSharedMemorySize,
			                        2 * kGemmTB * dim * (int)sizeof(float)) != hipSuccess) {
				g_create_error = "hipFuncSetAttribute(scan_gemm_bf16x3_kernel) failed";
				hipStreamDestroy(h->stream);
				delete h;
				return EXPANN_ERR_HIP;
			}
	for (const auto& v : kGemmI8)
		if (v.d == dim && v.mode == int_mode)
			if (hipFuncSetAttribute((const void*)v.scan, hipFuncAttributeMaxDynamicSharedMemorySize,
			                        2 * gemm_i8_tb(dim) * dim) != hipSuccess) {
				g_create_error = "hipFuncSetAttribute(scan_gemm_i8_kernel) failed";
				hipStreamDestroy(h->stream);
				delete h;
				return EXPANN_ERR_HIP;
			}
	*out = h;
	return EXPANN_OK;
}

void expann_destroy(expann_index* h) {
	if (!h)
		return;
	hipSetDevice(h->device);
	if (h->stream) hipStreamSynchronize(h->stream);
	drop_u8_shadow(h);
	if (h->owns_base && h->d_base) hipFree(h->d_base);
	if (h->d_base_i8q && h->base_i8q_owned) hipFree(h->d_base_i8q);
	if (h->ev_created)
		for (int i = 0; i < kEventPairs; ++i) {
			hipEventDestroy(h->ev[i][0]);
			hipEventDestroy(h->ev[i][1]);
		}
	if (h->side_stream) {
		hipStreamSynchronize(h->side_stream);
		hipStreamDestroy(h->side_stream);
	}
	for (hipEvent_t e : h->side_ev)
		if (e) hipEventDestroy(e);
	if (h->stream) hipStreamDestroy(h->stream);
	delete h;
}

const char* expann_last_error(const expann_index* h) {
	return h ? h->err.c_str() : g_create_error.c_str();
}

int expann_add(expann_index* h, const void* rows, size_t n) {
	if (!h)
		return EXPANN_ERR_INVALID_ARG;
	if (!rows && n)
		return h->fail(EXPANN_ERR_INVALID_ARG, "rows == NULL");
	if (h->d_base)
		return h->fail(EXPANN_ERR_INVALID_ARG, "index already built");
	const size_t bytes = n * (size_t)h->dim * h->elem;
	const unsigned char* src = static_cast<const unsigned char*>(rows);
	h->staging.insert(h->staging.end(), src, src + bytes);
	h->n_staged += n;
	return EXPANN_OK;
}

int expann_build(expann_index* h) {
	if (!h)
		return EXPANN_ERR_INVALID_ARG;
	if (h->d_base)
		return h->fail(EXPANN_ERR_INVALID_ARG, "index already built");
	if (h->n_staged == 0)
		return h->fail(EXPANN_ERR_INVALID_ARG, "build() on an empty index");
	if (h->n_staged >= (1ull << 32) - 32)
		return h->fail(EXPANN_ERR_UNSUPPORTED, "more than 2^32 rows per shard");
	HIP_TRY(h, hipSetDevice(h->device));
	drop_row_filter(h);
	HIP_TRY(h, hipMalloc(&h->d_base, h->staging.size()));
	h->owns_base = true;
	HIP_TRY(h, hipMemcpy(h->d_base, h->staging.data(), h->staging.size(), hipMemcpyHostToDevice));
	h->n = h->n_staged;
	std::vector<unsigned char>().swap(h->staging);
	if (float_rows(h) && h->n >= 4096 && h->opt_scan_kernel == 0) {
		for (const auto& v : kGemmF16X)
			if (v.d == h->dim) {
				const int rc = ensure_f16(h, &v, h->stream);
				if (rc != EXPANN_OK)
					return rc;
			}
		if (f16kl_dim(h->dim)) {
			const int rc = ensure_f16(h, &kGemmF16KL, h->stream);
			if (rc != EXPANN_OK)
				return rc;
		}
	}
	return EXPANN_OK;
}

int expann_set_base_device(expann_index* h, const void* d_rows, size_t n, uint64_t id_offset) {
	if (!h)
		return EXPANN_ERR_INVALID_ARG;
	if (!d_rows || n == 0)
		return h->fail(EXPANN_ERR_INVALID_ARG, "empty device base");
	if (n >= (1ull << 32) - 32)
		return h->fail(EXPANN_ERR_UNSUPPORTED, "more than 2^32 rows per shard");
	if (h->owns_base && h->d_base)
		hipFree(h->d_base);
	drop_u8_shadow(h);
	h->d_bnorm.reset();
	h->d_bias_i.reset();
	h->d_bnorm_bf.reset();
	h->d_base_split.reset();
	h->d_base_f16.reset();
	h->d_base_i8f.reset();
	h->d_bp_i8f.reset();
	h->d_rw_i8f.reset();
	h->i8f_state = 0;
	if (h->d_base_i8q && h->base_i8q_owned)
		hipFree(h->d_base_i8q);
	h->d_base_i8q = nullptr;
	h->base_i8q_owned = false;
	h->d_bp_i8q.reset();
	h->d_bnorm_f16.reset();
	h->d_bns_f16.reset();
	h->f16_scale = 0.0f;
	h->f16_n_pad = 0;
	drop_row_filter(h);
	h->d_base = const_cast<void*>(d_rows);
	h->owns_base = false;
	h->n = n;
	h->id_offset = id_offset;
	return EXPANN_OK;
}

size_t expann_size(const expann_index* h) { return h ? (h->d_base ? h->n : h->n_staged) : 0; }

int expann_search_device(expann_index* h, const void* d_queries, size_t m, size_t k,
                         uint64_t* d_ids, float* d_dists, void* stream) {
	if (!h)
		return EXPANN_ERR_INVALID_ARG;
	if (!h->d_base)
		return h->fail(EXPANN_ERR_NOT_BUILT, "search before build()");
	if (k == 0)
		return h->fail(EXPANN_ERR_INVALID_ARG, "k == 0");
	if (k > kMaxK)
		return h->fail(EXPANN_ERR_UNSUPPORTED, k_too_large());
	if (m == 0)
		return EXPANN_OK;
	if (!d_queries || !d_ids)
		return h->fail(EXPANN_ERR_INVALID_ARG, "NULL query/ids pointer");
	HIP_TRY(h, hipSetDevice(h->device));
	hipStream_t st = stream ? (hipStream_t)stream : h->stream;
	if (h->async_pending > 0 && h->async_stream != st) {
		HIP_TRY(h, hipStreamSynchronize(h->async_stream));
		h->async_stream = st;
	}
	const size_t qbytes = (size_t)h->dim * h->q_elem;
	h->stat_redo_queries = 0;
	h->stat_redo_candidates = 0;
	for (size_t q0 = 0; q0 < m; q0 += kMaxQueriesPerPass) {
		const size_t mm = std::min(kMaxQueriesPerPass, m - q0);
		int rc = search_pass(h, (const char*)d_queries + q0 * qbytes, mm, k, d_ids + q0 * k,
		                     d_dists ? d_dists + q0 * k : nullptr, st);
		if (rc != EXPANN_OK)
			return rc;
	}
	return EXPANN_OK;
}

int expann_sync(expann_index* h) {
	if (!h)
		return EXPANN_ERR_INVALID_ARG;
	if (h->async_pending == 0)
		return EXPANN_OK;
	HIP_TRY(h, hipSetDevice(h->device));
	const uint32_t n = h->async_pending;
	h->async_pending = 0;
	HIP_TRY(h, hipStreamSynchronize(h->async_stream));
	uint32_t bad = 0;
	uint64_t redo_queries = 0, redo_candidates = 0;
	for (uint32_t i = 0; i < n; ++i) {
		const uint32_t* f = h->h_flag_ring + kRingWords * i;
		const uint32_t mark = f[kRingMark];
		float qmax, scale;
		std::memcpy(&qmax, &f[2], sizeof(float));
		std::memcpy(&scale, &f[kRingScale], sizeof(float));
		const bool redo_word = (mark & 0x40000000u) != 0;
		if (redo_word && f[3] >= kRedoOverflowUnit)
			h->stat_redo_overflows++;
		else if (redo_word)
			redo_queries += f[3], redo_candidates += f[6];
		if (f[0] != 0 || (mark == 1 && f[1] != 0) || (scale > 0.0f && !(qmax * scale <= 60000.0f)) ||
		    (redo_word && f[3] >= kRedoOverflowUnit))
			++bad;
		unsigned long long tot;
		std::memcpy(&tot, f + 4, sizeof(tot));
		h->prof.candidates = tot;
		if ((mark & 0x80000000u) && tot > (mark & 0x3FFFFFFFu) && h->i8f_state == 1)
			h->i8f_state = 2;
	}
	h->stat_redo_queries = redo_queries;
	h->stat_redo_candidates = redo_candidates;
	if (bad)
		return h->fail(EXPANN_ERR_OVERFLOW, std::to_string(bad) + " of " + std::to_string(n) +
		                                        " deferred searches need the synchronous retry "
		                                        "(candidate overflow or queries outside the filter's range): "
		                                        "repeat them with async_search = 0");
	return EXPANN_OK;
}

int expann_search(expann_index* h, const void* queries, size_t m, size_t k, uint64_t* ids,
                  float* dists) {
	if (!h)
		return EXPANN_ERR_INVALID_ARG;
	if (!h->d_base)
		return h->fail(EXPANN_ERR_NOT_BUILT, "search before build()");
	if (k == 0)
		return h->fail(EXPANN_ERR_INVALID_ARG, "k == 0");
	if (k > kMaxK)
		return h->fail(EXPANN_ERR_UNSUPPORTED, k_too_large());
	if (m == 0)
		return EXPANN_OK;
	if (!queries || !ids)
		return h->fail(EXPANN_ERR_INVALID_ARG, "NULL query/ids pointer");
	if (h->async_pending) {
		const int rs = expann_sync(h);
		if (rs != EXPANN_OK)
			return rs;
	}
	HIP_TRY(h, hipSetDevice(h->device));
	const size_t qbytes = m * (size_t)h->dim * h->q_elem;
	HIP_TRY(h, h->d_q.ensure(qbytes));
	if (m * k <= 16384 && qbytes <= (256u << 10) && m <= kMaxQueriesPerPass && h->opt_latency_mode) {
		const size_t ids_off = (qbytes + 63) / 64 * 64;
		const size_t dists_off = ids_off + sizeof(uint64_t) * m * k;
		const size_t need = dists_off + sizeof(float) * m * k;
		if (need > h->h_pin_bytes) {
			h->h_pin.reset();
			h->h_pin_bytes = 0;
			const size_t want = std::max<size_t>(need, 64u << 10);
			HIP_TRY(h, hipHostMalloc(&h->h_pin, want, hipHostMallocDefault));
			h->h_pin_bytes = want;
		}
		char* pin = h->h_pin.as<char>();
		std::memcpy(pin, queries, qbytes);
		const void* dq = h->d_q;
		if (float_rows(h) && h->d_base_f16 && h->f16_scale > 0.0f && h->opt_scan_kernel == 0 &&
		    m <= (size_t)kRowsPerGroup && h->n >= 4096 && pick_gemm(h, m) != nullptr &&
		    !(h->filter_on && h->n_allowed <= kMaxCap)) {
			h->q_in_pinned_host = true;
			dq = pin;
		} else {
			HIP_TRY(h, hipMemcpyAsync(h->d_q, pin, qbytes, hipMemcpyHostToDevice, h->stream));
		}
		h->host_call = true;
		int rc = expann_search_device(h, dq, m, k, (uint64_t*)(pin + ids_off), (float*)(pin + dists_off),
		                              h->stream);
		h->host_call = false;
		if (h->q_in_pinned_host) {
			h->q_in_pinned_host = false;
		}
		if (rc != EXPANN_OK)
			return rc;
		std::memcpy(ids, pin + ids_off, sizeof(uint64_t) * m * k);
		if (dists)
			std::memcpy(dists, pin + dists_off, sizeof(float) * m * k);
		return EXPANN_OK;
	}
	HIP_TRY(h, h->d_ids.ensure(sizeof(uint64_t) * m * k));
	HIP_TRY(h, h->d_dists.ensure(sizeof(float) * m * k));
	HIP_TRY(h, hipMemcpyAsync(h->d_q, queries, qbytes, hipMemcpyHostToDevice, h->stream));
	h->host_call = true;
	int rc = expann_search_device(h, h->d_q, m, k, h->d_ids, h->d_dists, h->stream);
	h->host_call = false;
	if (rc != EXPANN_OK)
		return rc;
	HIP_TRY(h, hipMemcpyAsync(ids, h->d_ids, sizeof(uint64_t) * m * k, hipMemcpyDeviceToHost,
	                          h->stream));
	if (dists)
		HIP_TRY(h, hipMemcpyAsync(dists, h->d_dists, sizeof(float) * m * k,
		                          hipMemcpyDeviceToHost, h->stream));
	HIP_TRY(h, hipStreamSynchronize(h->stream));
	return EXPANN_OK;
}

int expann_merge_topk_strided_device(int device, const uint64_t* d_in_ids, const float* d_in_dists,
                                     size_t ids_stride, size_t dists_stride, size_t n_lists, size_t m,
                                     size_t k, uint64_t* d_out_ids, float* d_out_dists, void* stream) {
	if (!d_in_ids || !d_in_dists || !d_out_ids || !d_out_dists || n_lists == 0 || n_lists > 64 ||
	    k == 0) {
		g_create_error = "expann_merge_topk_device: bad arguments (1 <= n_lists <= 64)";
		return EXPANN_ERR_INVALID_ARG;
	}
	if (m == 0)
		return EXPANN_OK;
	if (hipSetDevice(device) != hipSuccess) {
		g_create_error = "hipSetDevice failed";
		return EXPANN_ERR_HIP;
	}
	if (m >= (1ull << 31) || n_lists * k >= (1ull << 31)) {
		g_create_error = "expann_merge_topk_device: m or n_lists * k beyond 2^31";
		return EXPANN_ERR_INVALID_ARG;
	}
	const size_t lds = n_lists * k * 12;
	if (lds <= (48u << 10))
		hipLaunchKernelGGL(merge_topk_kernel<true>, dim3((uint32_t)m), dim3(kWave), lds, (hipStream_t)stream, d_in_ids,
		                   d_in_dists, ids_stride, dists_stride, (uint32_t)n_lists, (uint32_t)m, (uint32_t)k, d_out_ids,
		                   d_out_dists);
	else
		hipLaunchKernelGGL(merge_topk_kernel<false>, dim3((uint32_t)m), dim3(kWave), 0, (hipStream_t)stream, d_in_ids,
		                   d_in_dists, ids_stride, dists_stride, (uint32_t)n_lists, (uint32_t)m, (uint32_t)k, d_out_ids,
		                   d_out_dists);
// ... 4 lines not shown
	return EXPANN_OK;
}

int expann_merge_topk_device(int device, const uint64_t* d_in_ids, const float* d_in_dists,
                             size_t n_lists, size_t m, size_t k, uint64_t* d_out_ids,
                             float* d_out_dists, void* stream) {
	return expann_merge_topk_strided_device(device, d_in_ids, d_in_dists, m * k, m * k, n_lists, m, k,
	                                        d_out_ids, d_out_dists, stream);
}

int expann_score_ids(expann_index* h, const void* query, const uint64_t* ids, size_t n_ids,
                     float cutoff, uint64_t* kept_ids, float* kept_scores, size_t* n_kept) {
	if (!h)
		return EXPANN_ERR_INVALID_ARG;
	if (!h->d_base)
		return h->fail(EXPANN_ERR_NOT_BUILT, "score_ids before build()");
	if (!n_kept || (n_ids && (!query || !ids || !kept_ids || !kept_scores)))
		return h->fail(EXPANN_ERR_INVALID_ARG, "NULL pointer");
	*n_kept = 0;
	if (n_ids == 0)
		return EXPANN_OK;
	if (n_ids >= (1ull << 32))
		return h->fail(EXPANN_ERR_INVALID_ARG, "more than 2^32 ids");
	for (size_t i = 0; i < n_ids; ++i)
		if (ids[i] < h->id_offset || ids[i] - h->id_offset >= h->n)
			return h->fail(EXPANN_ERR_INVALID_ARG, "id out of range");
	HIP_TRY(h, hipSetDevice(h->device));
	DevBuf b_query, b_idl, b_sc, b_q8s, b_bad;
	const size_t qb = (size_t)h->dim * h->q_elem;
	HIP_TRY(h, b_query.alloc(qb));
	HIP_TRY(h, b_idl.alloc(sizeof(uint64_t) * n_ids));
	HIP_TRY(h, b_sc.alloc(sizeof(float) * n_ids));
	void *d_query = b_query.p, *d_idl = b_idl.p, *d_sc = b_sc.p, *d_q8s = nullptr;
	uint32_t* d_bad = nullptr;
	HIP_TRY(h, hipMemcpyAsync(d_query, query, qb, hipMemcpyHostToDevice, h->stream));
	HIP_TRY(h, hipMemcpyAsync(d_idl, ids, sizeof(uint64_t) * n_ids, hipMemcpyHostToDevice, h->stream));
	const uint32_t blocks = (uint32_t)((n_ids + kRowsPerGroup - 1) / kRowsPerGroup);
	uint32_t bad_host = 0;
	if (float_rows(h)) {
		const ScoreVariant* sv = nullptr;
		for (const auto& v : kScoreF32)
			if (v.d == h->dim && v.ip == (h->metric == EXPANN_METRIC_IP) && !f16_rows(h))
				sv = &v;
		if (!sv && any_dim_f32(h->dim))
			sv = f16_rows(h) ? &kScoreF16Any[h->metric == EXPANN_METRIC_IP ? 1 : 0]
			                 : &kScoreF32Any[h->metric == EXPANN_METRIC_IP ? 1 : 0];
		if (!sv)
			return h->fail(EXPANN_ERR_UNSUPPORTED, "no score kernel for this dim");
		ScoreIdsParams sp{h->d_base, d_query, (const uint64_t*)d_idl, h->id_offset,
		                  (uint32_t)n_ids, (float*)d_sc, (uint32_t)h->dim};
		hipLaunchKernelGGL(sv->fn, dim3(blocks), dim3(kBlock), 0, h->stream, sp);
	} else {
		const ScoreI8Variant* sv = nullptr;
		for (const auto& v : kScoreI8)
			if (v.d == h->dim && v.mode == h->int_mode)
				sv = &v;
		if (!sv && any_dim_i8(h->dim, h->int_mode))
			for (const auto& v : kScoreI8Any)
				if (v.mode == h->int_mode)
					sv = &v;
		if (!sv)
			return h->fail(EXPANN_ERR_UNSUPPORTED, "no 8-bit score kernel for this dim");
		const void* qptr = d_query;
		if (h->dtype == EXPANN_DTYPE_U8) {
			HIP_TRY(h, b_q8s.alloc((size_t)h->dim));
			HIP_TRY(h, b_bad.alloc(sizeof(uint32_t)));
			d_q8s = b_q8s.p;
			d_bad = b_bad.as<uint32_t>();
			HIP_TRY(h, hipMemsetAsync(d_bad, 0, sizeof(uint32_t), h->stream));
			hipLaunchKernelGGL(u8_query_prep_kernel, dim3((uint32_t)((h->dim + kBlock - 1) / kBlock)),
			                   dim3(kBlock), 0, h->stream, (const float*)d_query, (size_t)h->dim,
			                   (uint8_t*)d_q8s, d_bad, (uint32_t*)nullptr);
			HIP_TRY(h, hipMemcpyAsync(&bad_host, d_bad, sizeof(uint32_t), hipMemcpyDeviceToHost,
			                          h->stream));
			qptr = d_q8s;
		}
		ScoreIdsI8Params sp{h->d_base, qptr, (const uint64_t*)d_idl, h->id_offset, (uint32_t)n_ids,
		                    (float*)d_sc, (uint32_t)h->dim};
		hipLaunchKernelGGL(sv->fn, dim3(blocks), dim3(kBlock), 0, h->stream, sp);
	}
	DevBuf b_kid, b_ksc, b_cnt;
	HIP_TRY(h, b_kid.alloc(sizeof(uint64_t) * n_ids));
	HIP_TRY(h, b_ksc.alloc(sizeof(float) * n_ids));
	HIP_TRY(h, b_cnt.alloc(sizeof(uint32_t)));
	FilterScoresParams fp{(const uint64_t*)d_idl, (const float*)d_sc, (uint32_t)n_ids, cutoff, b_kid.as<uint64_t>(),
	                      b_ksc.as<float>(), b_cnt.as<uint32_t>()};
	hipLaunchKernelGGL(filter_scores_kernel, dim3(1), dim3(1024), 0, h->stream, fp);
	HIP_TRY(h, hipGetLastError());
	uint32_t kept = 0;
	HIP_TRY(h, hipMemcpyAsync(&kept, b_cnt.p, sizeof(uint32_t), hipMemcpyDeviceToHost, h->stream));
	HIP_TRY(h, hipStreamSynchronize(h->stream));
	if (bad_host)
		return h->fail(EXPANN_ERR_UNSUPPORTED, "query values outside [0,255] for the uint8 metric");
	if (kept) {
		HIP_TRY(h, hipMemcpyAsync(kept_ids, b_kid.p, sizeof(uint64_t) * kept, hipMemcpyDeviceToHost, h->stream));
		HIP_TRY(h, hipMemcpyAsync(kept_scores, b_ksc.p, sizeof(float) * kept, hipMemcpyDeviceToHost, h->stream));
		HIP_TRY(h, hipStreamSynchronize(h->stream));
	}
	*n_kept = kept;
	return EXPANN_OK;
}


int expann_set_profiling(expann_index* h, int enable) {
	if (!h)
		return EXPANN_ERR_INVALID_ARG;
	HIP_TRY(h, hipSetDevice(h->device));
	if (enable && !h->ev_created) {
		for (int i = 0; i < kEventPairs; ++i) {
			HIP_TRY(h, hipEventCreate(&h->ev[i][0]));
			HIP_TRY(h, hipEventCreate(&h->ev[i][1]));
		}
		h->ev_created = true;
	}
	h->profiling = enable != 0;
	h->ev_used = 0;
	h->prof = expann_profile{};
	h->prof_extra_ms = 0;
	if (h->u8_shadow)
		return expann_set_profiling(h->u8_shadow, enable);
	return EXPANN_OK;
}

int expann_get_profile(expann_index* h, expann_profile* out) {
	if (!h || !out)
		return EXPANN_ERR_INVALID_ARG;
	HIP_TRY(h, hipSetDevice(h->device));
	double ms = 0;
	for (int i = 0; i < h->ev_used; ++i) {
		HIP_TRY(h, hipEventSynchronize(h->ev[i][1]));
		float t = 0;
		HIP_TRY(h, hipEventElapsedTime(&t, h->ev[i][0], h->ev[i][1]));
		ms += t;
	}
	h->prof.scan_ms = ms + h->prof_extra_ms;
	*out = h->prof;
	h->ev_used = 0;
	h->prof_extra_ms = 0;
	h->prof = expann_profile{};
	return EXPANN_OK;
}

int expann_get_stat(expann_index* h, const char* name, uint64_t* out) {
	if (!h || !name || !out)
		return EXPANN_ERR_INVALID_ARG;
	if (!std::strcmp(name, "redo_queries"))
		*out = h->stat_redo_queries;
	else if (!std::strcmp(name, "redo_candidates"))
		*out = h->stat_redo_candidates;
	else if (!std::strcmp(name, "redo_overflows"))
		*out = h->stat_redo_overflows;
	else if (!std::strcmp(name, "spec_rank"))
		*out = h->stat_spec_rank;
	else if (!std::strcmp(name, "base_bytes"))
		*out = h->d_base ? (uint64_t)h->n * (uint64_t)h->dim * h->elem : 0;
	else if (!std::strcmp(name, "filter_active"))
		*out = h->filter_on ? 1 : 0;
	else if (!std::strcmp(name, "filter_rows"))
		*out = h->filter_on ? h->n_allowed : expann_size(h);
	else
		return h->fail(EXPANN_ERR_INVALID_ARG, std::string("unknown statistic ") + name);
	return EXPANN_OK;
}

uint32_t expann_spec_rank_auto(size_t k, uint32_t sample_frac) {
	return spec_rank_auto(k, sample_frac ? 1.0 / (double)sample_frac : 1.0);
}

namespace {
int set_row_filter(expann_index* h, const uint32_t* bits, size_t n_words, bool on_device, hipStream_t user_st) {
	if (!h)
		return EXPANN_ERR_INVALID_ARG;
	if (!bits)
		return h->fail(EXPANN_ERR_INVALID_ARG, "row filter: NULL bits");
	if (!float_rows(h))
		return h->fail(EXPANN_ERR_UNSUPPORTED,
		               "row filter: fp32 / fp16 rows only (8-bit and int16 rows have integer row terms)");
	if (!h->d_base)
		return h->fail(EXPANN_ERR_NOT_BUILT, "row filter before build()");
	const size_t need_words = (h->n + 31) / 32;
	if (n_words < need_words)
		return h->fail(EXPANN_ERR_INVALID_ARG, "row filter: " + std::to_string(n_words) + " words for " +
		                                           std::to_string(h->n) + " rows (need " + std::to_string(need_words) + ")");
	HIP_TRY(h, hipSetDevice(h->device));
	if (h->async_pending > 0)
		HIP_TRY(h, hipStreamSynchronize(h->async_stream));
	HIP_TRY(h, hipStreamSynchronize(h->stream));
	hipStream_t st = user_st ? user_st : h->stream;
	const size_t words = (h->n + 127) / 128 * 4;
	if (words != h->filter_words || !h->d_filter_bits) {
		h->filter_on = false;
		h->d_filter_bits.reset();
		h->filter_words = 0;
		HIP_TRY(h, hipMalloc(&h->d_filter_bits, sizeof(uint32_t) * words));
		h->filter_words = words;
	}
	if (!h->d_filter_stat)
		HIP_TRY(h, hipMalloc(&h->d_filter_stat, sizeof(uint32_t) * (2 + kFilterSegs)));
	if (!h->d_filter_list)
		HIP_TRY(h, hipMalloc(&h->d_filter_list, sizeof(uint32_t) * kFilterListCap));
	h->filter_on = false;
	h->filter_terms_valid = false;
	HIP_TRY(h, hipMemsetAsync(h->d_filter_bits, 0, sizeof(uint32_t) * words, st));
	HIP_TRY(h, hipMemcpyAsync(h->d_filter_bits, bits, sizeof(uint32_t) * need_words,
	                          on_device ? hipMemcpyDeviceToDevice : hipMemcpyHostToDevice, st));
	HIP_TRY(h, hipMemsetAsync(h->d_filter_stat, 0, sizeof(uint32_t) * (2 + kFilterSegs), st));
	hipLaunchKernelGGL(filter_count_kernel, dim3(kFilterSegs), dim3(kBlock), 0, st, h->d_filter_bits.as<uint32_t>(),
	                   (uint32_t)h->n, (uint32_t)words, h->d_filter_stat.as<uint32_t>(), h->d_filter_stat + 2);
	HIP_TRY(h, hipGetLastError());
	uint32_t stat[2] = {0, 0};
	HIP_TRY(h, hipMemcpyAsync(stat, h->d_filter_stat, sizeof(stat), hipMemcpyDeviceToHost, st));
	HIP_TRY(h, hipStreamSynchronize(st));
	h->n_allowed = stat[0];
	h->filter_residues = stat[1];
	h->filter_list_stride = (uint32_t)std::max<size_t>(1, (h->n_allowed + kFilterListCap - 1) / kFilterListCap);
	h->filter_list_len = (uint32_t)((h->n_allowed + h->filter_list_stride - 1) / h->filter_list_stride);
	if (h->n_allowed) {
		hipLaunchKernelGGL(filter_compact_kernel, dim3(kFilterSegs), dim3(kBlock), 0, st, h->d_filter_bits.as<const uint32_t>(),
		                   (uint32_t)words, h->d_filter_stat.as<const uint32_t>() + 2, h->filter_list_stride,
		                   h->d_filter_list.as<uint32_t>(), kFilterListCap);
		HIP_TRY(h, hipGetLastError());
		HIP_TRY(h, hipStreamSynchronize(st));
	}
	h->filter_on = true;
	return EXPANN_OK;
}
}

int expann_set_row_filter(expann_index* h, const uint32_t* allow_bits, size_t n_words) {
	return set_row_filter(h, allow_bits, n_words, false, nullptr);
}

int expann_set_row_filter_device(expann_index* h, const uint32_t* d_allow_bits, size_t n_words, void* stream) {
	return set_row_filter(h, d_allow_bits, n_words, true, (hipStream_t)stream);
}

int expann_clear_row_filter(expann_index* h) {
	if (!h)
		return EXPANN_ERR_INVALID_ARG;
	if (h->async_pending > 0) {
		HIP_TRY(h, hipSetDevice(h->device));
		HIP_TRY(h, hipStreamSynchronize(h->async_stream));
	}
	h->filter_on = false;
	return EXPANN_OK;
}

int expann_set_option(expann_index* h, const char* name, long value) {
	if (!h || !name)
		return EXPANN_ERR_INVALID_ARG;
	if (!std::strcmp(name, "query_tile"))
		h->opt_query_tile = value;
	else if (!std::strcmp(name, "cand_capacity"))
		h->opt_cand_capacity = value;
	else if (!std::strcmp(name, "debug"))
		h->opt_debug = value;
	else if (!std::strcmp(name, "scan_kernel"))
		h->opt_scan_kernel = value;
	else if (!std::strcmp(name, "f16x") || !std::strcmp(name, "i8x") || !std::strcmp(name, "i8w")) {
		if (value == 0)
			return h->fail(EXPANN_ERR_UNSUPPORTED, std::string(name) + " = 0: the 32 x 32 MFMA forms of rounds 1-2 were removed in round 3");
	}
	else if (!std::strcmp(name, "tail_chunks"))
		h->opt_tail_chunks = value;
	else if (!std::strcmp(name, "persist"))
		h->opt_persist = value;
	else if (!std::strcmp(name, "i8_filter"))
		h->opt_i8_filter = value < 0 ? 0 : (value > 2 ? 2 : value);
	else if (!std::strcmp(name, "spec_rank"))
		h->opt_spec_rank = value < 0 ? 0 : value;
	else if (!std::strcmp(name, "redo_bound"))
		h->opt_redo_bound = value;
	else if (!std::strcmp(name, "select_overlap"))
		h->opt_select_overlap = value;
	else if (!std::strcmp(name, "ip_rescale"))
		h->opt_ip_rescale = value;
	else if (!std::strcmp(name, "sample_pass"))
		h->opt_sample_pass = value;
	else if (!std::strcmp(name, "u8_exact"))
		h->opt_u8_exact = value;
	else if (!std::strcmp(name, "latency_mode"))
		h->opt_latency_mode = value;
	else if (!std::strcmp(name, "async_search"))
		h->opt_async = value;
	else if (!std::strcmp(name, "scan_chunks"))
		h->opt_scan_chunks = value;
	else if (!std::strcmp(name, "xcd_tolerance"))
		h->opt_xcd_tolerance = value < 0 ? 0 : value;
	else if (!std::strcmp(name, "sample_run"))
		h->opt_sample_run = value < 1 ? 1 : (value > 64 ? 64 : value);
	else if (!std::strcmp(name, "sample_frac"))
		h->opt_sample_frac = value < 0 ? 0 : value;
	else if (!std::strcmp(name, "sample_ratio"))
		h->opt_sample_ratio = value < 2 ? 2 : value;
	else
		return h->fail(EXPANN_ERR_INVALID_ARG, std::string("unknown option ") + name);
	return EXPANN_OK;
}

}
```

### expann_amd/csrc/scan_gemm_f16.hpp

```cpp
#pragma once
#include "common.hpp"
#include "scan_gemm_bf16.hpp"
#include "scan_gemm_i8f.hpp"
#include "select.hpp"

namespace expann {

typedef _Float16 f16x8 __attribute__((ext_vector_type(8)));

__host__ __device__ inline float gemm_f16_filter_eps(int d) {
	return d <= 256 ? 1.125f * 0.0009765625f
	                : 0.0009765625f + (4.0f + 4.25f * (float)d + 256.0f) * 5.9604644775390625e-08f;
}

__global__ __launch_bounds__(kBlock) void convert_f16_kernel(const float* in, size_t n_values,
                                                             float scale, _Float16* out,
                                                             uint32_t* maxabs_bits) {
	uint32_t b = 0;
	for (size_t i = (size_t)blockIdx.x * kBlock + threadIdx.x; i < n_values;
	     i += (size_t)gridDim.x * kBlock) {
		const float v = in[i];
		out[i] = (_Float16)(v * scale);
		const uint32_t vb = __builtin_bit_cast(uint32_t, v) & 0x7fffffffu;
		b = vb > b ? vb : b;
// ... 163 lines not shown
		const uint32_t vb = __builtin_bit_cast(uint32_t, v) & 0x7fffffffu;
		b = vb > b ? vb : b;
	}
	acc = reduce16_ref_order(acc);
	acc = __shfl(acc, lane & ~15);
	float c = 1.0f;
	if (ip_ref) {
		const float ref = ip_ref[0];
		if (acc > 0.0f && ref > 0.0f && acc < 3.0e38f && ref < 3.0e38f) {
			int e = (int)__builtin_rintf(0.5f * (__builtin_log2f(ref) - __builtin_log2f(acc)));
			e = e < -40 ? -40 : (e > 40 ? 40 : e);
			c = __builtin_ldexpf(1.0f, e);
		}
	}
	if (i < m) {
		for (uint32_t t = 0; t < ld / 16; ++t) {
			const uint32_t col = l + 16 * t;
			const float v = col < d ? src[16 * t] : 0.0f;
			q16[(size_t)i * ld + col] = (_Float16)(v * c * scale);
			if (q_copy && col < d)
				q_copy[(size_t)i * d + col] = v;
		}
		if (l == 0) {
			qnrm[i] = acc * c * c;
			if (qscale)
				qscale[i] = c;
		}
	}
	b = __builtin_bit_cast(uint32_t, __builtin_bit_cast(float, b) * c);
	for (int off = 32; off > 0; off >>= 1) {
		const uint32_t o = (uint32_t)__shfl_xor((int)b, off);
		b = o > b ? o : b;
	}
	if (lane == 0)
		red[wave] = b;
	__syncthreads();
	if (threadIdx.x == 0) {
		for (int w = 1; w < kBlock / 64; ++w)
			b = red[w] > b ? red[w] : b;
		if (b != 0)
			atomicMax(maxabs_bits, b);
	}
}

__global__ __launch_bounds__(kBlock) void f16_terms_kernel(const float* nrm, uint32_t n, float eps,
                                                           float abs_coef, const float* tau,
                                                           float mul, float* out, int ip, const float* qscale) {
	const uint32_t i = blockIdx.x * kBlock + threadIdx.x;
	if (i >= n)
		return;
	const float v = nrm[i];
	if (ip) {
		const float e = v * eps + abs_coef * __builtin_sqrtf(v);
		out[i] = (tau ? 2.0f * tau[i] * (qscale ? qscale[i] : 1.0f) + e : -e) * mul;
		return;
	}
	const float t = v * (1.0f - eps) - abs_coef * __builtin_sqrtf(v);
	out[i] = (tau ? tau[i] - t : t) * mul;
}

struct GemmF16Params {
	const void* base_f16;
	const float* bnorm;
	uint32_t n_rows;
	uint32_t n_tiles_sel;
	uint32_t tile_stride;
	uint32_t tile_run;
	uint32_t tiles_per_block;
	uint32_t n_qtiles;
	const void* queries_f16;
	const float* theta;
	float two_inv_s2;
	uint32_t m;
	uint32_t* cand_cnt;
	uint64_t* cand;
	uint32_t cap;
	uint32_t debug;
	unsigned long long* clk;
	float* sample_out;
	uint32_t n_chunks;
	uint32_t xcd_map;
	uint32_t n_big, tiles_small;
	uint4* log;
	uint32_t* log_cnt;
	uint32_t log_cap;
	uint32_t* lost;
	uint32_t* work_ctr;
	uint32_t n_items;
	uint32_t ksteps;
	const uint32_t* live_q;
};

struct GatherLogParams {
	const uint4* log;
	const uint32_t* log_cnt;
	uint32_t log_cap, n_chunks, n_qtiles, xcd_map, m;
	uint32_t n_groups, chunks_per_block;
	uint32_t* cand_cnt;
	uint64_t* cand;
	uint32_t cap;
	const float* theta;
	float key_mul;
	const int* i_thp;
	const int* i_bias;
	const int* i_qself;
	int i_mode;
	const float* i_rw;
	const uint32_t* live_q;
};
__global__ __launch_bounds__(kBlock) void gather_logs_kernel(GatherLogParams p) {
	__shared__ uint32_t cnt[64], base[64];
	const uint32_t grp = blockIdx.x % p.n_groups, qw = blockIdx.x / p.n_groups;
	const uint32_t qtile = qw >> 2, w = qw & 3;
	const uint32_t q0 = qtile * 256 + w * 64;
	if (p.live_q && qtile * 256 >= (*p.live_q & kRedoCountMask))
		return;
	if (threadIdx.x < 64)
		cnt[threadIdx.x] = 0;
	__syncthreads();
	const uint32_t lane = threadIdx.x & 63, wv = threadIdx.x >> 6;
	const uint32_t c0 = grp * p.chunks_per_block;
	const uint32_t c1 = c0 + p.chunks_per_block < p.n_chunks ? c0 + p.chunks_per_block : p.n_chunks;
	auto log_of = [&](uint32_t c, uint32_t& n) -> const uint4* {
		const uint32_t bid = p.xcd_map ? ((c >> 3) * p.n_qtiles + qtile) * 8 + (c & 7) : c * p.n_qtiles + qtile;
		const uint32_t li = bid * 4 + w;
		n = p.log_cnt[li];
		if (n > p.log_cap)
			n = p.log_cap;
		return p.log + (size_t)li * p.log_cap;
	};
	for (uint32_t c = c0 + wv; c < c1; c += kBlock / 64) {
		uint32_t n;
		const uint4* src = log_of(c, n);
		for (uint32_t i = lane; i < n; i += 64)
			atomicAdd(&cnt[(src[i].z - q0) & 63], 1u);
	}
	__syncthreads();
	if (threadIdx.x < 64) {
		const uint32_t n = cnt[threadIdx.x];
		base[threadIdx.x] = n ? atomicAdd(&p.cand_cnt[q0 + threadIdx.x], n) : 0u;
		cnt[threadIdx.x] = 0;
	}
	__syncthreads();
	for (uint32_t c = c0 + wv; c < c1; c += kBlock / 64) {
		uint32_t n;
		const uint4* src = log_of(c, n);
		for (uint32_t i = lane; i < n; i += 64) {
			const uint4 e = src[i];
			const uint32_t ql = (e.z - q0) & 63;
			const uint32_t slot = base[ql] + atomicAdd(&cnt[ql], 1u);
			if (slot < p.cap) {
				uint64_t key;
				if (p.i_mode == 3) {
					const float kappa = (float)(p.i_bias[e.y] - (int)e.x);
					key = make_key(p.i_rw[e.y] < __builtin_inff() ? kappa : -__builtin_inff(), e.y);
				} else if (p.i_mode) {
					const int dot = (int)e.x - p.i_thp[e.z];
					const int score = p.i_mode == 1 ? p.i_bias[e.y] - 2 * dot + p.i_qself[e.z] : -dot;
					key = make_key((float)score, e.y);
				} else {
					key = make_key((__builtin_bit_cast(float, e.x) + p.theta[e.z]) * p.key_mul, e.y);
				}
				p.cand[(size_t)e.z * p.cap + slot] = key;
			}
		}
	}
}

__device__ inline float max3f(float a, float b, float c) {
	return __builtin_fmaxf(__builtin_fmaxf(a, b), c);
}

template <int N> __device__ inline void wait_vm_then_barrier() {
	asm volatile("s_waitcnt vmcnt(%0) lgkmcnt(0)\n\ts_barrier" ::"n"(N) : "memory");
}

#ifndef EXPANN_F16_THREADS
#define EXPANN_F16_THREADS 256
#endif
constexpr int kF16Threads = EXPANN_F16_THREADS;
constexpr int kF16WgPerCu = 512 / kF16Threads;
constexpr int kF16Waves = kF16Threads / 64;
constexpr int kF16TQ = 64 * kF16Waves;
static_assert(kF16Waves == 4 && kF16TQ == 256, "gather_logs_kernel files the logs of 4 waves x 64 queries per workgroup");
constexpr int kF16TB = 64;
constexpr int kF16Prefetch = 2;
constexpr int kF16Bufs = kF16Prefetch + 1;
constexpr int kF16WaveQueue = 88;
constexpr int kF16EntryBytes = 80;
constexpr int kF16FlushEvery = 8;
template <int D> struct F16Geom {
	static constexpr int THREADS = D >= 256 ? 512 : kF16Threads;
	static constexpr int WAVES = THREADS / 64;
	static constexpr int TQW = D >= 256 ? 1 : 2;
	static constexpr int WGQ = WAVES * 32 * TQW;
	static constexpr int NBUF = D >= 512 ? 2 : kF16Bufs;
	static constexpr bool TH_LDS = D == 64;
	static constexpr int QCAP = D >= 512 ? 32 : ((D >= 256 || TH_LDS) ? 56 : kF16WaveQueue);
	static constexpr bool NATURAL = D >= 256;
	static constexpr int WG_PER_CU = TH_LDS ? 3 : 512 / THREADS;
};
static_assert(F16Geom<128>::WGQ == kF16TQ && F16Geom<256>::WGQ == kF16TQ, "one query-tile size");
template <int D> constexpr int gemm_f16_lds_bytes() {
	using G = F16Geom<D>;
	return G::NBUF * (kF16TB * D * 2 + G::WAVES * 256) + G::WAVES * G::QCAP * kF16EntryBytes + G::WGQ * 4 + 64 +
	       (G::TH_LDS ? G::WAVES * 2 * G::TQW * 16 * 4 : 0);
}
static_assert(gemm_f16_lds_bytes<64>() * 3 <= 160 * 1024 &&
                  gemm_f16_lds_bytes<128>() * F16Geom<128>::WG_PER_CU <= 160 * 1024 &&
                  gemm_f16_lds_bytes<256>() <= 160 * 1024 && gemm_f16_lds_bytes<512>() <= 160 * 1024,
              "LDS budget per CU");


struct SampleTauParams {
	const float* vals;
	uint32_t n_vals;
	uint32_t m;
	uint32_t k;
	const float* qnrm;
	float eps, abs_coef, inv_mul;
	int ip;
	float* tau;
	uint32_t* tau_row;
	float* theta;
	float mul;
	uint32_t* cand_cnt;
	const float* qscale;
	int* i8_thp;
	const float* i8_aq;
	const float* i8_wq_in;
	float* i8_wq;
	double i8_inv_2s2;
	uint32_t j;
	float* tau_s;
};
__device__ inline float sample_tau_of(const SampleTauParams& p, float qn, uint32_t ord) {
	float tau = __builtin_inff();
	if (ord != 0) {
		const float g = ordered_to_float(ord);
		if (p.ip)
			tau = 0.5f * (qn * p.eps + p.abs_coef * __builtin_sqrtf(qn)) - g * (0.5f * p.inv_mul);
		else
			tau = qn * (1.0f + p.eps) + p.abs_coef * __builtin_sqrtf(qn) - g * p.inv_mul;
		if (!(tau == tau))
			tau = __builtin_inff();
	}
	return tau;
}
__device__ inline void sample_tau_finish(const SampleTauParams& p, uint32_t qi, uint32_t ord, uint32_t ord_s) {
	const float qn = p.qnrm[qi];
	const float tau_k = sample_tau_of(p, qn, ord);
	const float tau = (p.tau_s && ord_s != ord) ? sample_tau_of(p, qn, ord_s) : tau_k;
	p.tau[qi] = (p.ip && p.qscale) ? tau_k / p.qscale[qi] : tau_k;
	if (p.tau_s)
		p.tau_s[qi] = (p.ip && p.qscale) ? tau / p.qscale[qi] : tau;
	p.tau_row[qi] = 0xFFFFFFFFu;
	p.theta[qi] = p.ip ? (2.0f * tau + qn * p.eps + p.abs_coef * __builtin_sqrtf(qn)) * p.mul
	                   : (tau - (qn * (1.0f - p.eps) - p.abs_coef * __builtin_sqrtf(qn))) * p.mul;
	if (p.i8_thp)
		i8f_thresholds(p.i8_aq[qi], p.i8_wq_in[qi], tau, p.i8_inv_2s2, &p.i8_thp[qi], &p.i8_wq[qi]);
	p.cand_cnt[qi] = 0;
}
__device__ inline void sample_tau_query_wg(const SampleTauParams& p, uint32_t qi, uint32_t* hist, uint32_t* ctl) {
	const uint32_t tid = threadIdx.x;
	const float* v = p.vals + (size_t)qi * p.n_vals;
	uint32_t ord[8];
#pragma unroll
	for (int j = 0; j < 8; ++j) {
		const uint32_t i = j * kBlock + tid;
		ord[j] = i < p.n_vals ? float_to_ordered(v[i]) : 0u;
	}
	uint32_t prefix = 0, mask = 0, krem = p.k;
	for (int pass = 3; pass >= 0; --pass) {
		const int sh = 8 * pass;
		__syncthreads();
		hist[tid] = 0;
		if (tid == 0)
			ctl[0] = 0xFFFFFFFFu;
		__syncthreads();
#pragma unroll
		for (int j = 0; j < 8; ++j)
			if ((ord[j] & mask) == prefix)
				atomicAdd(&hist[(ord[j] >> sh) & 255u], 1u);
		__syncthreads();
		const uint32_t mine = hist[tid];
		for (int off = 1; off < 256; off <<= 1) {
			const uint32_t add = tid + off < 256 ? hist[tid + off] : 0u;
			__syncthreads();
			hist[tid] += add;
			__syncthreads();
		}
		const uint32_t above = hist[tid] - mine;
		if (mine != 0 && above < krem && krem <= above + mine) {
			ctl[0] = tid;
			ctl[1] = krem - above;
		}
		__syncthreads();
		const uint32_t digit = ctl[0];
		if (digit == 0xFFFFFFFFu) {
			prefix = 0;
			break;
		}
		krem = ctl[1];
		prefix |= digit << sh;
		mask |= 0xFFu << sh;
	}
	if (tid == 0)
		sample_tau_finish(p, qi, prefix, prefix);
}
template <int PER>
__device__ inline void sample_tau_query(const SampleTauParams& p, uint32_t qi, int lane, uint32_t* scratch) {
	const float* v = p.vals + (size_t)qi * p.n_vals;
	uint64_t keys[PER];
#pragma unroll
	for (int j = 0; j < PER; ++j) {
		const uint32_t i = j * 64 + lane;
		keys[j] = i < p.n_vals ? ((uint64_t)float_to_ordered(v[i]) << 32) | (0xFFFFFFFFu - i) : 0ull;
	}
	uint32_t ord[PER];
#pragma unroll
	for (int j = 0; j < PER; ++j)
		ord[j] = (uint32_t)(keys[j] >> 32);
	const bool spec = p.tau_s != nullptr && p.j < p.k;
	uint2 kj;
	if (p.k <= 64) {
		kj = wave_kth_largest_sparse_u32<PER>(ord, p.k, scratch, lane, spec ? p.j : 0u);
	} else {
		kj.x = wave_kth_largest_u32<PER>(ord, p.k);
		kj.y = spec ? wave_kth_largest_u32<PER>(ord, p.j) : 0u;
	}
	if (lane == 0)
		sample_tau_finish(p, qi, kj.x, spec ? kj.y : kj.x);
}
template <int PER>
__global__ __launch_bounds__(kBlock) void sample_tau_kernel(SampleTauParams p) {
	__shared__ uint32_t scratch[kBlock / 64][64];
	const uint32_t qi = blockIdx.x * (kBlock / 64) + (threadIdx.x >> 6);
	if (qi >= p.m)
		return;
	sample_tau_query<PER>(p, qi, threadIdx.x & 63, scratch[threadIdx.x >> 6]);
}

struct RedoCompactParams {
	uint32_t* word;
	const uint32_t* list;
	uint32_t n_slots;
	uint32_t row_bytes;
	const void* q16;
	void* rq16;
	const float* qnrm;
	float* r_qnrm;
	const float* tau;
	const float* bound;
	const float* qscale;
	float eps, abs_coef, mul;
	int ip;
	float* r_theta;
	uint32_t* r_cnt;
	const void* q8;
	void* rq8;
	const float* i8_aq;
	const float* i8_wq_in;
	int* r_thp;
	float* r_wq;
	double i8_inv_2s2;
};
__global__ __launch_bounds__(kBlock) void redo_compact_kernel(RedoCompactParams p) {
	const uint32_t lane = threadIdx.x & 63;
	const uint32_t s = blockIdx.x * (kBlock / 64) + (threadIdx.x >> 6);
	const uint32_t failed = *p.word & kRedoCountMask;
	if (blockIdx.x == 0 && threadIdx.x == 0 && failed > p.n_slots)
		atomicAdd(p.word, kRedoOverflowUnit);
	if (s >= p.n_slots)
		return;
	const bool live = s < failed;
	const uint32_t qi = live ? p.list[s] : 0u;
	const uint4* src = reinterpret_cast<const uint4*>((const unsigned char*)p.q16 + (size_t)qi * p.row_bytes);
	uint4* dst = reinterpret_cast<uint4*>((unsigned char*)p.rq16 + (size_t)s * p.row_bytes);
	for (uint32_t i = lane; i < p.row_bytes / 16; i += 64) {
		uint4 v = make_uint4(0u, 0u, 0u, 0u);
		if (live)
			v = src[i];
		dst[i] = v;
	}
	if (p.q8) {
		const uint32_t rb = p.row_bytes / 2;
		const uint32_t* s8 = reinterpret_cast<const uint32_t*>((const unsigned char*)p.q8 + (size_t)qi * rb);
		uint32_t* d8 = reinterpret_cast<uint32_t*>((unsigned char*)p.rq8 + (size_t)s * rb);
		for (uint32_t i = lane; i < rb / 4; i += 64)
			d8[i] = live ? s8[i] : 0u;
	}
	if (lane != 0)
		return;
	p.r_cnt[s] = 0;
	if (!live) {
		p.r_qnrm[s] = 0.0f;
		p.r_theta[s] = -__builtin_inff();
		if (p.q8) {
			p.r_thp[s] = (-2147483647 - 1) / 2;
			p.r_wq[s] = __builtin_inff();
		}
		return;
	}
	const float qn = p.qnrm[qi];
	const float tau = p.bound ? __builtin_fminf(p.tau[qi], p.bound[s]) : p.tau[qi];
	const float tau_f = (p.ip && p.qscale) ? tau * p.qscale[qi] : tau;
	p.r_qnrm[s] = qn;
	p.r_theta[s] = p.ip ? (2.0f * tau_f + qn * p.eps + p.abs_coef * __builtin_sqrtf(qn)) * p.mul
	                    : (tau_f - (qn * (1.0f - p.eps) - p.abs_coef * __builtin_sqrtf(qn))) * p.mul;
	if (p.q8)
		i8f_thresholds(p.i8_aq[qi], p.i8_wq_in[qi], tau, p.i8_inv_2s2, p.r_thp + s, p.r_wq + s);
}

}
```

### expann_amd/csrc/scan_gemm_i8w.hpp

```cpp
#pragma once
#include "scan_gemm_i8q.hpp"

namespace expann {

template <int D> struct I8wGeom {
	static constexpr int WG_PER_CU = D == 128 ? 3 : 2;
	static constexpr int QCAP = D == 128 ? 64 : kF16WaveQueue;
};
template <int D> constexpr int gemm_i8w_lds_bytes() {
	return kF16Bufs * (kF16TB * D + kF16Waves * 256) + kF16Waves * I8wGeom<D>::QCAP * kF16EntryBytes + kF16TQ * 4 + 64;
}
static_assert(gemm_i8w_lds_bytes<128>() * 3 <= 160 * 1024 && gemm_i8w_lds_bytes<256>() * 2 <= 160 * 1024,
              "LDS budget per CU");

struct GemmI8wParams {
	GemmI8qParams q;
	uint4* log;
	uint32_t* log_cnt;
	uint32_t log_cap;
	uint32_t* lost;
};

template <int D, bool L2FORM, bool SAMPLE = false, bool REDO = false>
__global__ __launch_bounds__(kF16Threads, I8wGeom<D>::WG_PER_CU) void scan_gemm_i8w_kernel(GemmI8wParams pw) {
	static_assert(D == 128 || D == 256, "built for d = 128, 256");
	const GemmI8qParams& p = pw.q;
	constexpr int THREADS = kF16Threads, WAVES = kF16Waves, WGQ = kF16TQ, QCAP = I8wGeom<D>::QCAP;
	constexpr int ROWB = D, CH = ROWB / 16;
	constexpr int KS = D / 64;
	constexpr int TILE_BYTES = kF16TB * ROWB;
	constexpr int RPB = (ROWB < 256) ? 256 / ROWB : 1;
	constexpr int SWM = (CH < 16 ? CH : 16) - 1;
	constexpr int NBUF = kF16Bufs;
	constexpr int kNever = -2147483647 - 1;
	extern __shared__ __attribute__((aligned(16))) unsigned char smem[];

	const int tid = threadIdx.x;
	const int lane = tid & 63;
	const int wave = __builtin_amdgcn_readfirstlane(tid >> 6);
	const int l15 = lane & 15, lq = lane >> 4;
	uint32_t qtile = blockIdx.x % p.n_qtiles;
	uint32_t chunk = blockIdx.x / p.n_qtiles;
	if (p.xcd_map) {
		const uint32_t j = blockIdx.x >> 3;
		qtile = j % p.n_qtiles;
		chunk = (blockIdx.x & 7) + 8 * (j / p.n_qtiles);
	}
	const uint32_t wg_q0 = qtile * WGQ;
	if (!SAMPLE && p.live_q && wg_q0 >= (*p.live_q & kRedoCountMask))
		return;
	const uint32_t q0 = wg_q0 + wave * 64;

	const uint32_t t0 = chunk * p.tiles_per_block;
	uint32_t t1 = t0 + p.tiles_per_block;
	if (t1 > p.n_tiles_sel)
		t1 = p.n_tiles_sel;
	uint32_t* const my_log_cnt = SAMPLE ? nullptr : pw.log_cnt + (size_t)blockIdx.x * WAVES + wave;
	if (t0 >= t1) {
		if (SAMPLE) {
			for (uint32_t i = lane; i < 64 * 32; i += 64)
				if (q0 + (i >> 5) < p.m)
					p.sample_out[((size_t)(q0 + (i >> 5)) * p.n_chunks + chunk) * 32 + (i & 31)] = kNever;
		} else if (lane == 0) {
			*my_log_cnt = 0;
		}
		return;
	}

	unsigned char* const bn_slots = smem + NBUF * TILE_BYTES;
	struct QEntry {
		int acc[16];
		int bp;
		uint32_t row;
		uint32_t qrow0;
		uint32_t pad;
	};
	static_assert(sizeof(QEntry) == kF16EntryBytes, "queue entry size");
	QEntry* const queue = reinterpret_cast<QEntry*>(bn_slots + NBUF * WAVES * 256) + wave * QCAP;
	uint32_t* const fills = reinterpret_cast<uint32_t*>(bn_slots + NBUF * WAVES * 256 + WAVES * QCAP * kF16EntryBytes) + WGQ;

	i32x4 a[4][KS];
#pragma unroll
	for (int tq = 0; tq < 4; ++tq) {
		uint32_t qi = q0 + tq * 16 + l15;
		if (qi >= p.m)
			qi = p.m - 1;
		const i32x4* src = reinterpret_cast<const i32x4*>((const unsigned char*)p.queries + (size_t)qi * ROWB);
#pragma unroll
		for (int s = 0; s < KS; ++s)
			a[tq][s] = src[4 * s + lq];
	}
	i32x4 th[4];
#pragma unroll
	for (int tq = 0; tq < 4; ++tq)
#pragma unroll
		for (int r = 0; r < 4; ++r) {
			const uint32_t qi = q0 + tq * 16 + 4 * lq + r;
			th[tq][r] = (qi < p.m && !SAMPLE) ? p.thp[qi] : kNever / 2;
		}
#pragma unroll
	for (int tq = 0; tq < 4; ++tq) {
#pragma unroll
		for (int s = 0; s < KS; ++s)
			asm volatile("" : "+v"(a[tq][s]));
		asm volatile("" : "+v"(th[tq]));
	}
	uint32_t aoff[KS];
#pragma unroll
	for (int s = 0; s < KS; ++s)
		aoff[s] = l15 * ROWB + (((4 * s + lq) ^ ((l15 / RPB) & SWM)) * 16);
	static_assert((16 / RPB) % (SWM + 1) == 0, "the swizzle term repeats every 16 rows");

	auto tile_row0 = [&](uint32_t t) -> uint32_t {
		return ((t / p.tile_run) * (p.tile_stride * p.tile_run) + (t % p.tile_run)) * kF16TB;
	};
	constexpr int N_STAGE = kF16TB * CH / THREADS;
	static_assert(kF16TB * CH % THREADS == 0, "whole staging rounds");
	constexpr int LOADS = N_STAGE + 1;
	uint32_t soff[N_STAGE];
#pragma unroll
	for (int i = 0; i < N_STAGE; ++i) {
		const uint32_t S = i * THREADS + tid;
		const uint32_t r = S / CH, pc = S % CH;
		soff[i] = r * ROWB + ((pc ^ ((r / RPB) & SWM)) * 16);
	}
	auto stage_piece = [&](const unsigned char* tb, uint32_t row0, int buf, int i) {
		if (i < N_STAGE) {
			unsigned char* dst0 = smem + buf * TILE_BYTES + wave * 64 * 16;
			__builtin_amdgcn_global_load_lds((const __attribute__((address_space(1))) void*)(tb + soff[i < N_STAGE ? i : 0]),
			                                 (__attribute__((address_space(3))) void*)(dst0 + i * THREADS * 16), 16, 0, 0);
		} else {
			__builtin_amdgcn_global_load_lds((const __attribute__((address_space(1))) void*)(p.bp + row0 + lane),
			                                 (__attribute__((address_space(3))) void*)(bn_slots + (buf * WAVES + wave) * 256),
			                                 4, 0, 0);
		}
	};
	auto stage_src = [&](uint32_t t, uint32_t& row0) -> const unsigned char* {
		if (t > t1 - 1)
			t = t1 - 1;
		row0 = tile_row0(t);
		return (const unsigned char*)p.base + (size_t)row0 * ROWB;
	};
	auto stage = [&](uint32_t t, int buf) {
		uint32_t row0;
		const unsigned char* tb = stage_src(t, row0);
#pragma unroll
		for (int i = 0; i < LOADS; ++i)
			stage_piece(tb, row0, buf, i);
	};

	uint32_t wfill = 0;
	uint32_t glog_n = 0;
	uint4* const my_log = SAMPLE ? nullptr : pw.log + ((size_t)blockIdx.x * WAVES + wave) * pw.log_cap;
	auto flush_own = [&]() {
		const uint32_t n = wfill < (uint32_t)QCAP ? wfill : (uint32_t)QCAP;
		for (uint32_t base = 0; base < n * 16; base += 128) {
			bool hit[2];
			int cv[2];
			uint32_t row[2], qi[2];
#pragma unroll
			for (int u = 0; u < 2; ++u) {
				const uint32_t i = base + 64 * u + lane;
				const QEntry& e = queue[i < n * 16 ? i >> 4 : 0];
				const uint32_t v = i & 15;
				cv[u] = e.acc[v];
				row[u] = e.row;
				hit[u] = i < n * 16 && cv[u] >= e.bp && row[u] < p.n_rows;
				qi[u] = e.qrow0 + 16 * (v >> 2) + (v & 3);
			}
#pragma unroll
			for (int u = 0; u < 2; ++u) {
				const unsigned long long mask = __builtin_amdgcn_ballot_w64(hit[u]);
				if (mask == 0)
					continue;
				const uint32_t pos = glog_n + __builtin_amdgcn_mbcnt_hi((uint32_t)(mask >> 32),
				                                                        __builtin_amdgcn_mbcnt_lo((uint32_t)mask, 0u));
				if (hit[u] && pos < pw.log_cap)
					my_log[pos] = make_uint4((uint32_t)cv[u], row[u], qi[u], 0u);
				glog_n += (uint32_t)__builtin_popcountll(mask);
			}
		}
		wfill = 0;
	};
	auto push_hits = [&](const i32x4 (&acc)[4][4], int tc, unsigned long long mask, bool mine, int bp,
	                     uint32_t row0) {
		static_assert(QCAP >= 64, "a tile column's hits fit an empty queue");
		if (wfill + (uint32_t)__builtin_popcountll(mask) > (uint32_t)QCAP)
			flush_own();
		uint32_t qrow0 = q0 + 4 * lq;
		asm volatile("" : "+v"(qrow0));
		const uint32_t brow = row0 + tc * 16 + l15;
		const uint32_t slot = wfill + __builtin_amdgcn_mbcnt_hi((uint32_t)(mask >> 32),
		                                                        __builtin_amdgcn_mbcnt_lo((uint32_t)mask, 0u));
		if (mine) {
			if (slot < (uint32_t)QCAP) {
				QEntry& e = queue[slot];
#pragma unroll
				for (int tq = 0; tq < 4; ++tq)
#pragma unroll
					for (int r = 0; r < 4; ++r)
						e.acc[tq * 4 + r] = acc[tq][tc][r];
				e.bp = bp;
				e.row = brow;
				e.qrow0 = qrow0;
			}
		}
		wfill += (uint32_t)__builtin_popcountll(mask);
	};

	const bool idle = REDO && p.live_q && q0 >= (*p.live_q & kRedoCountMask);
	if (REDO && idle && lane == 0)
		fills[wave] = 0;
	stage(t0, 0);
	stage(t0 + 1, 1);
	asm volatile("s_waitcnt vmcnt(0) lgkmcnt(0)\n\ts_barrier" ::: "memory");
	if (REDO && idle) {
		int ibuf = 0;
		for (uint32_t t = t0; t < t1; ++t) {
			const int pbuf = ibuf == 0 ? NBUF - 1 : ibuf - 1;
			asm volatile("" ::: "memory");
			__builtin_amdgcn_s_waitcnt(0x0070);
			__builtin_amdgcn_s_barrier();
			asm volatile("" ::: "memory");
			stage(t + 2, pbuf);
			ibuf = ibuf + 1 == NBUF ? 0 : ibuf + 1;
		}
		if (lane == 0)
			*my_log_cnt = 0;
		asm volatile("s_waitcnt vmcnt(0)" ::: "memory");
		return;
	}

	i32x4 acc[4][4];
	int buf = 0;
	uint32_t since_look = 0;
	auto frag_at = [&](int b, int tc, int s) -> i32x4 {
		return *reinterpret_cast<const i32x4*>(smem + ((uint32_t)b * TILE_BYTES + aoff[s]) + tc * 16 * ROWB);
	};
	auto read_bp = [&](int (&bp)[4], int b) {
		const int* slot = reinterpret_cast<const int*>(bn_slots + (b * WAVES + wave) * 256);
#pragma unroll
		for (int tc = 0; tc < 4; ++tc)
			bp[tc] = slot[tc * 16 + l15];
	};
	auto col_max = [&](int pc) -> int {
		int m0 = max3i(acc[0][pc][0], acc[0][pc][1], acc[0][pc][2]);
		int m1 = max3i(acc[0][pc][3], acc[1][pc][0], acc[1][pc][1]);
		int m2 = max3i(acc[1][pc][2], acc[1][pc][3], acc[2][pc][0]);
		int m3 = max3i(acc[2][pc][1], acc[2][pc][2], acc[2][pc][3]);
		int m4 = max3i(acc[3][pc][0], acc[3][pc][1], acc[3][pc][2]);
		m0 = max3i(m0, m1, acc[3][pc][3]);
		m2 = max3i(m2, m3, m4);
		return max(m0, m2);
	};
	int bpv[4];
	i32x4 smax[2][4];
#pragma unroll
	for (int par = 0; par < 2; ++par)
#pragma unroll
		for (int tq = 0; tq < 4; ++tq)
			smax[par][tq] = i32x4{kNever, kNever, kNever, kNever};
	auto fold = [&](int par) {
#pragma unroll
		for (int tq = 0; tq < 4; ++tq)
#pragma unroll
			for (int r = 0; r < 4; ++r)
				smax[par][tq][r] = max3i(smax[par][tq][r], acc[tq][par][r], acc[tq][par + 2][r]);
	};
	auto mfma_part = [&](int tc, const i32x4 (&f)[KS], int s0, int s1) {
		const int nb = -bpv[tc];
		const i32x4 c0 = {nb, nb, nb, nb};
#pragma unroll
		for (int s = s0; s < s1; ++s)
#pragma unroll
			for (int tq = 0; tq < 4; ++tq)
				acc[tq][tc] = __builtin_amdgcn_mfma_i32_16x16x64_i8(a[tq][s], f[s], s == 0 ? (SAMPLE ? c0 : th[tq]) : acc[tq][tc], 0, 0, 0);
	};

	i32x4 fb[2][KS];
#pragma unroll
	for (int s = 0; s < KS; ++s)
		fb[0][s] = frag_at(0, 0, s);
	read_bp(bpv, 0);
	__builtin_amdgcn_s_waitcnt(0xC07F);
	for (uint32_t t = t0; t < t1; ++t) {
		const int nbuf = buf + 1 == NBUF ? 0 : buf + 1;
		const int pbuf = buf == 0 ? NBUF - 1 : buf - 1;
		int gmax[4];
		int bpn[4];
		__builtin_amdgcn_s_setprio(1);
		mfma_part(0, fb[0], 0, 1);
		__builtin_amdgcn_sched_barrier(0);
#pragma unroll
		for (int s = 0; s < KS; ++s)
			fb[1][s] = frag_at(buf, 1, s);
		__builtin_amdgcn_sched_barrier(0);
		mfma_part(0, fb[0], 1, KS);
		__builtin_amdgcn_sched_barrier(0);
		mfma_part(1, fb[1], 0, 1);
		__builtin_amdgcn_sched_barrier(0);
#pragma unroll
		for (int s = 0; s < KS; ++s)
			fb[0][s] = frag_at(buf, 2, s);
		__builtin_amdgcn_sched_barrier(0);
		mfma_part(1, fb[1], 1, KS);
		if (!SAMPLE) {
			gmax[0] = col_max(0);
			asm volatile("" : "+v"(gmax[0]));
		}
		__builtin_amdgcn_sched_barrier(0);
		__builtin_amdgcn_s_setprio(0);
		const bool look = !SAMPLE && ++since_look == kF16FlushEvery;
		if (look && lane == 0)
			fills[wave] = wfill;
		asm volatile("" ::: "memory");
		__builtin_amdgcn_s_waitcnt(0x0070);
		__builtin_amdgcn_s_barrier();
		asm volatile("" ::: "memory");
		if (look) {
			since_look = 0;
			const uint32_t f = fills[lane & (WAVES - 1)];
			if (__builtin_amdgcn_ballot_w64(f >= (uint32_t)QCAP / 2) != 0)
				flush_own();
		}
		uint32_t srow0;
		const unsigned char* stb = stage_src(t + 2, srow0);
		__builtin_amdgcn_s_setprio(1);
		mfma_part(2, fb[0], 0, 1);
		__builtin_amdgcn_sched_barrier(0);
#pragma unroll
		for (int s = 0; s < KS; ++s)
// ... 72 lines not shown
```

### expann_amd/csrc/select.hpp

```cpp
#pragma once
#include "common.hpp"

namespace expann {

struct SelectParams {
	const uint64_t* cand;
	const uint32_t* cand_cnt;
	uint32_t fixed_count;
	uint32_t cap;
	uint32_t k;
	uint64_t id_offset;
	uint64_t* out_ids;
	float* out_dists;
	float* tau_out;
	const float* tau_prev;
	uint32_t* tau_row_out;
	const uint32_t* tau_row_prev;
	const float* rerank_base;
	const float* rerank_queries;
	uint32_t dim;
	uint32_t metric_ip;
	float prune_eps;
	float prune_abs;
	const float* bn_max;
	uint32_t* overflow;
	uint32_t wave_done;
	uint32_t wave0_short;
	const float* qnrm;
	const float* row_w;
	const float* q_w;
	const float* spec_tau;
	uint32_t* redo_word;
	uint32_t* redo_list;
	uint32_t redo_cap;
	float* redo_bound;
	const uint32_t* slot_map;
	const uint32_t* live_slots;
	uint32_t* redo_cand;
};
constexpr uint32_t kRedoCountMask = 0xFFFFFu;
constexpr uint32_t kRedoOverflowUnit = 1u << 20;

__device__ inline void spec_check(const SelectParams& p, uint32_t qi, bool has_kth, float s_k) {
	if (!p.spec_tau || (has_kth && s_k <= p.spec_tau[qi]))
		return;
	const uint32_t slot = atomicAdd(p.redo_word, 1u) & kRedoCountMask;
	if (slot < p.redo_cap) {
		p.redo_list[slot] = qi;
		p.redo_bound[slot] = has_kth ? s_k : __builtin_inff();
	}
}

__device__ inline float i8f_cutoff(uint32_t kth_ord, float wq) {
	if (kth_ord >= 0xFF800000u)
		return __builtin_inff();
	const float c = ordered_to_float(kth_ord) + wq;
	return c + __builtin_fabsf(c) * 0x1p-18f + 1.0f;
}
__device__ inline uint32_t i8f_upper_ord(const SelectParams& p, uint64_t key) {
	const float v = key_score(key) + p.row_w[key_idx(key)];
	return float_to_ordered(v == v ? v : __builtin_inff());
}

__global__ __launch_bounds__(1024) void sum_u32_kernel(const uint32_t* in, uint32_t n,
                                                       unsigned long long* out) {
	__shared__ unsigned long long red[16];
	unsigned long long s = 0;
	for (uint32_t i = threadIdx.x; i < n; i += 1024)
		s += in[i];
	for (int off = 32; off > 0; off >>= 1)
		s += __shfl_xor(s, off);
	if ((threadIdx.x & 63) == 0)
		red[threadIdx.x >> 6] = s;
	__syncthreads();
	if (threadIdx.x == 0) {
		for (int w = 1; w < 16; ++w)
			s += red[w];
		out[0] = s;
	}
}

__device__ inline uint32_t wave_min_u32(uint32_t v) {
	v = min(v, (uint32_t)row_ror_i<8>((int)v));
	v = min(v, (uint32_t)row_ror_i<4>((int)v));
	v = min(v, (uint32_t)row_ror_i<2>((int)v));
	v = min(v, (uint32_t)row_ror_i<1>((int)v));
	v = min(v, (uint32_t)__shfl_xor((int)v, 16));
	v = min(v, (uint32_t)__shfl_xor((int)v, 32));
	return v;
}
__device__ inline uint64_t wave_min_u64(uint64_t v) {
	const uint32_t hi = (uint32_t)(v >> 32);
	const uint32_t mhi = wave_min_u32(hi);
	const uint32_t lo = hi == mhi ? (uint32_t)v : 0xFFFFFFFFu;
	return ((uint64_t)mhi << 32) | wave_min_u32(lo);
}


template <int NE>
__device__ inline void wave_emit_sorted(const SelectParams& p, const uint64_t* list, uint32_t n_s,
                                        uint32_t qi, int lane) {
	uint64_t e[NE];
#pragma unroll
	for (int j = 0; j < NE; ++j)
		e[j] = lane + 64 * j < (int)n_s ? list[lane + 64 * j] : kSentinelKey;
	if (p.k > 16) {
		uint32_t r[NE];
#pragma unroll
		for (int j = 0; j < NE; ++j)
			r[j] = 0;
		for (uint32_t i = 0; i < n_s; ++i) {
			const uint64_t x = list[i];
#pragma unroll
			for (int j = 0; j < NE; ++j)
				r[j] += x < e[j] ? 1u : 0u;
		}
#pragma unroll
		for (int j = 0; j < NE; ++j) {
			if (e[j] == kSentinelKey || r[j] >= p.k)
				continue;
			if (p.out_ids)
				p.out_ids[(size_t)qi * p.k + r[j]] = (uint64_t)key_idx(e[j]) + p.id_offset;
			if (p.out_dists)
				p.out_dists[(size_t)qi * p.k + r[j]] = key_score(e[j]);
			if (r[j] == p.k - 1)
				spec_check(p, qi, true, key_score(e[j]));
			if (r[j] == p.k - 1 && p.tau_out) {
				p.tau_out[qi] = key_score(e[j]);
				if (p.tau_row_out)
					p.tau_row_out[qi] = key_idx(e[j]);
			}
		}
		for (uint32_t i = n_s + lane; i < p.k; i += 64) {
			if (p.out_ids)
				p.out_ids[(size_t)qi * p.k + i] = ~0ull;
			if (p.out_dists)
				p.out_dists[(size_t)qi * p.k + i] = __builtin_inff();
		}
		if (lane == 0 && n_s < p.k)
			spec_check(p, qi, false, 0.0f);
		if (lane == 0 && n_s < p.k && p.tau_out) {
			p.tau_out[qi] = p.tau_prev ? p.tau_prev[qi] : __builtin_inff();
			if (p.tau_row_out)
				p.tau_row_out[qi] = p.tau_row_prev ? p.tau_row_prev[qi] : 0xFFFFFFFFu;
		}
		return;
	}
	for (uint32_t r = 0; r < p.k; ++r) {
		uint64_t mn = e[0];
#pragma unroll
		for (int j = 1; j < NE; ++j)
			mn = e[j] < mn ? e[j] : mn;
		mn = wave_min_u64(mn);
		const bool ok = mn != kSentinelKey;
		if (lane == 0) {
			if (p.out_ids)
				p.out_ids[(size_t)qi * p.k + r] = ok ? (uint64_t)key_idx(mn) + p.id_offset : ~0ull;
			if (p.out_dists)
				p.out_dists[(size_t)qi * p.k + r] = ok ? key_score(mn) : __builtin_inff();
			if (r == p.k - 1)
				spec_check(p, qi, ok, key_score(mn));
			if (r == p.k - 1 && p.tau_out) {
				p.tau_out[qi] = ok ? key_score(mn) : (p.tau_prev ? p.tau_prev[qi] : __builtin_inff());
				if (p.tau_row_out)
					p.tau_row_out[qi] = ok ? key_idx(mn) : (p.tau_row_prev ? p.tau_row_prev[qi] : 0xFFFFFFFFu);
			}
		}
#pragma unroll
		for (int j = 0; j < NE; ++j)
			e[j] = e[j] == mn ? kSentinelKey : e[j];
	}
}

template <int PER> __device__ inline uint32_t wave_kth_smallest_u32(const uint32_t (&v)[PER], uint32_t k) {
	uint32_t lo = 0, hi = 0xFFFFFFFFu;
	while (lo < hi) {
		const uint32_t mid = lo + ((hi - lo) >> 1);
		uint32_t cnt = 0;
#pragma unroll
		for (int j = 0; j < PER; ++j)
			cnt += (uint32_t)__builtin_popcountll(__builtin_amdgcn_ballot_w64(v[j] <= mid));
		if (cnt >= k)
			hi = mid;
		else
			lo = mid + 1;
	}
	return lo;
}

template <int PER> __device__ inline uint32_t wave_kth_largest_u32(const uint32_t (&v)[PER], uint32_t k) {
	uint32_t lo = 0, hi = 0xFFFFFFFFu;
	while (lo < hi) {
		const uint32_t mid = lo + ((hi - lo) >> 1) + ((hi - lo) & 1);
		uint32_t cnt = 0;
#pragma unroll
		for (int j = 0; j < PER; ++j)
			cnt += (uint32_t)__builtin_popcountll(__builtin_amdgcn_ballot_w64(v[j] >= mid));
		if (cnt >= k)
			lo = mid;
		else
			hi = mid - 1;
	}
	return lo;
}

template <int PER>
__device__ inline uint2 wave_kth_largest_sparse_u32(const uint32_t (&v)[PER], uint32_t k, uint32_t* scratch,
                                                    int lane, uint32_t j = 0) {
	uint32_t mx[1] = {v[0]};
#pragma unroll
	for (int j = 1; j < PER; ++j)
		mx[0] = v[j] > mx[0] ? v[j] : mx[0];
	const uint32_t B = wave_kth_largest_u32<1>(mx, k);
	uint32_t total = 0;
#pragma unroll
	for (int j = 0; j < PER; ++j)
		total += (uint32_t)__builtin_popcountll(__builtin_amdgcn_ballot_w64(v[j] >= B));
	if (total > 64)
		return make_uint2(wave_kth_largest_u32<PER>(v, k), j ? wave_kth_largest_u32<PER>(v, j) : 0u);
	uint32_t base = 0;
#pragma unroll
	for (int j = 0; j < PER; ++j) {
		const unsigned long long mask = __builtin_amdgcn_ballot_w64(v[j] >= B);
		if (v[j] >= B)
			scratch[base + __builtin_amdgcn_mbcnt_hi((uint32_t)(mask >> 32),
			                                         __builtin_amdgcn_mbcnt_lo((uint32_t)mask, 0u))] = v[j];
		base += (uint32_t)__builtin_popcountll(mask);
	}
	__builtin_amdgcn_fence(__ATOMIC_RELEASE, "wavefront");
	__builtin_amdgcn_wave_barrier();
	__builtin_amdgcn_fence(__ATOMIC_ACQUIRE, "wavefront");
	uint32_t w[1] = {lane < (int)total ? scratch[lane] : 0u};
	return make_uint2(wave_kth_largest_u32<1>(w, k), j ? wave_kth_largest_u32<1>(w, j) : 0u);
}

template <int PER, typename TR = float>
__device__ inline void select_wave_body(const SelectParams& p, uint32_t qi, uint32_t c, uint64_t* list,
                                        int lane) {
	const uint64_t* src = p.cand + (size_t)qi * p.cap;
	uint64_t kk[PER];
#pragma unroll
	for (int j = 0; j < PER; ++j)
		kk[j] = lane + 64 * j < (int)c ? src[lane + 64 * j] : kSentinelKey;
	const uint32_t l = lane & 15, grp = lane >> 4;
	const uint32_t qo = p.slot_map ? p.slot_map[qi] : qi;
	const float* q = p.rerank_queries + (size_t)qo * p.dim + l;
	float cutoff = __builtin_inff();
	const bool final_scores = p.rerank_base == nullptr;
	if ((p.prune_eps > 0.0f || final_scores || p.row_w) && c > p.k) {
		float qn = 0.0f;
		if (final_scores || p.row_w) {
		} else if (p.qnrm) {
			qn = p.qnrm[qi];
		} else {
			for (uint32_t t = 0; t < p.dim / 16; ++t)
				qn = __builtin_fmaf(q[16 * t], q[16 * t], qn);
			qn = reduce16_ref_order(qn);
		}
		uint32_t sc[PER];
#pragma unroll
		for (int j = 0; j < PER; ++j)
			sc[j] = (p.row_w && kk[j] != kSentinelKey) ? i8f_upper_ord(p, kk[j]) : (uint32_t)(kk[j] >> 32);
		uint32_t kth = 0xFFFFFFFFu;
		if (p.k > 24) {
			kth = wave_kth_smallest_u32<PER>(sc, p.k);
		} else
		for (uint32_t r = 0; r < p.k; ++r) {
			uint32_t mn = sc[0];
#pragma unroll
			for (int j = 1; j < PER; ++j)
				mn = min(mn, sc[j]);
			mn = wave_min_u32(mn);
			if (mn == 0xFFFFFFFFu)
				break;
			kth = mn;
#pragma unroll
			for (int j = 0; j < PER; ++j)
				sc[j] = sc[j] == mn ? 0xFFFFFFFFu : sc[j];
		}
		if (final_scores) {
			cutoff = ordered_to_float(kth);
		} else if (p.row_w) {
			cutoff = i8f_cutoff(kth, p.q_w[qi]);
		} else {
			const float bmax = p.bn_max[0];
			cutoff = ordered_to_float(kth) + p.prune_eps * (qn + 1.5f * bmax) +
			         p.prune_abs * (__builtin_sqrtf(qn) + __builtin_sqrtf(bmax));
		}
	}
	uint32_t n_s = 0;
#pragma unroll
	for (int j = 0; j < PER; ++j) {
		const bool hit = lane + 64 * j < (int)c && key_score(kk[j]) <= cutoff;
		const unsigned long long mask = __builtin_amdgcn_ballot_w64(hit);
		const uint32_t pos = n_s + __builtin_amdgcn_mbcnt_hi((uint32_t)(mask >> 32),
		                                                      __builtin_amdgcn_mbcnt_lo((uint32_t)mask, 0u));
		if (hit)
			list[pos] = kk[j];
		n_s += (uint32_t)__builtin_popcountll(mask);
	}
	asm volatile("s_waitcnt lgkmcnt(0)" ::: "memory");
	for (uint32_t i0 = 0; p.rerank_base && i0 < n_s; i0 += 16) {
		constexpr int U = 4;
		float acc[U];
		uint32_t row[U];
		const TR* r[U];
#pragma unroll
		for (int u = 0; u < U; ++u) {
			const uint32_t i = i0 + 4 * u + grp;
			row[u] = key_idx(list[i < n_s ? i : 0]);
			r[u] = (const TR*)p.rerank_base + (size_t)row[u] * p.dim + l;
			acc[u] = 0.0f;
		}
		const uint32_t nt = p.dim / 16;
		for (uint32_t t0 = 0; t0 < nt; t0 += 8) {
			float qv[8];
			TR rv[U][8];
#pragma unroll
			for (int t = 0; t < 8; ++t)
				qv[t] = t0 + t < nt ? q[16 * (t0 + t)] : 0.0f;
#pragma unroll
			for (int u = 0; u < U; ++u)
#pragma unroll
				for (int t = 0; t < 8; ++t)
					rv[u][t] = t0 + t < nt ? r[u][16 * (t0 + t)] : (TR)0.0f;
#pragma unroll
			for (int u = 0; u < U; ++u)
#pragma unroll
				for (int t = 0; t < 8; ++t) {
					if (t0 + t >= nt)
						continue;
					if (p.metric_ip) {
						acc[u] = ref_dot<TR>(qv[t], rv[u][t], acc[u]);
					} else {
						const float diff = ref_diff<TR>(qv[t], rv[u][t]);
						acc[u] = __builtin_fmaf(diff, diff, acc[u]);
					}
				}
		}
#pragma unroll
		for (int u = 0; u < U; ++u) {
			acc[u] = reduce16_ref_order(acc[u]);
			const uint32_t i = i0 + 4 * u + grp;
			if (l == 0 && i < n_s)
				list[i] = make_key(p.metric_ip ? -acc[u] : acc[u], row[u]);
		}
	}
	asm volatile("s_waitcnt lgkmcnt(0)" ::: "memory");
	if (n_s <= 256)
		wave_emit_sorted<(PER < 4 ? PER : 4)>(p, list, n_s, qo, lane);
	else
		wave_emit_sorted<PER>(p, list, n_s, qo, lane);
}

template <int PER, int WAVES, typename TR = float>
__global__ __launch_bounds__(64 * WAVES) void select_wave_kernel(SelectParams p, uint32_t m) {
	constexpr uint32_t kSelectWaveMax = 64 * PER;
	__shared__ uint64_t lists[WAVES][kSelectWaveMax];
	const int lane = threadIdx.x & 63;
	const int wave = __builtin_amdgcn_readfirstlane(threadIdx.x >> 6);
	const uint32_t qi = blockIdx.x * WAVES + wave;
	if (qi >= m)
		return;
	const uint32_t c = p.cand_cnt ? p.cand_cnt[qi] : p.fixed_count;
	if (c > kSelectWaveMax || c > p.cap || (c <= p.wave_done && p.wave_done != 0))
		return;
	select_wave_body<PER, TR>(p, qi, c, lists[wave], lane);
}

template <typename TR>
__global__ __launch_bounds__(kBlock) void select_topk_kernel(SelectParams p) {
	extern __shared__ __attribute__((aligned(16))) unsigned char smem_raw[];
	uint64_t* keys = reinterpret_cast<uint64_t*>(smem_raw);
	const uint32_t qi = blockIdx.x;
	const uint32_t tid = threadIdx.x;
	if (p.live_slots && qi >= (*p.live_slots & kRedoCountMask))
		return;
	const uint32_t qo = p.slot_map ? p.slot_map[qi] : qi;
	uint32_t c = p.cand_cnt ? p.cand_cnt[qi] : p.fixed_count;
	if (p.redo_cand && tid == 0)
		atomicAdd(p.redo_cand, c);
	if (p.wave_done && c <= p.wave_done && c <= p.cap)
		return;
	if (p.wave0_short && c <= 2048 && c <= p.cap && 8 * (size_t)p.cap >= 16384) {
		if (tid < 64) {
			if (c <= 512)
				select_wave_body<8, TR>(p, qi, c, keys, (int)tid);
			else
				select_wave_body<32, TR>(p, qi, c, keys, (int)tid);
		}
		return;
	}
	if (c > p.cap) {
		if (tid == 0)
			atomicAdd(p.overflow, p.live_slots ? kRedoOverflowUnit : 1u);
		c = p.cap;
	}
	uint32_t n2 = 2;
	while (n2 < c)
		n2 <<= 1;
	const uint64_t* src = p.cand + (size_t)qi * p.cap;
	for (uint32_t i = tid; i < n2; i += kBlock)
		keys[i] = i < c ? src[i] : kSentinelKey;
	__syncthreads();
	auto bitonic = [&](uint32_t len) {
		for (uint32_t size = 2; size <= len; size <<= 1) {
			for (uint32_t stride = size >> 1; stride > 0; stride >>= 1) {
				for (uint32_t i = tid; i < (len >> 1); i += kBlock) {
					const uint32_t lo = 2 * i - (i & (stride - 1));
					const uint32_t hi = lo + stride;
					const bool up = ((lo & size) == 0);
					const uint64_t a = keys[lo], b = keys[hi];
					if ((a > b) == up) {
						keys[lo] = b;
						keys[hi] = a;
					}
				}
				__syncthreads();
			}
		}
	};
	if (p.rerank_base) {
		const uint32_t l = tid & 15, grp = tid >> 4;
		const float* q = p.rerank_queries + (size_t)qo * p.dim + l;
		uint32_t n_rescore = c;
		if ((p.prune_eps > 0.0f || p.row_w) && c > p.k) {
			bitonic(n2);
			float cutoff;
			if (p.row_w) {
				uint32_t* s_max = reinterpret_cast<uint32_t*>(keys + p.cap) + 1;
				if (tid == 0)
					*s_max = 0;
				__syncthreads();
				uint32_t mx = 0;
				for (uint32_t i = tid; i < p.k; i += kBlock)
					mx = max(mx, i8f_upper_ord(p, keys[i]));
				if (mx)
					atomicMax(s_max, mx);
				__syncthreads();
				cutoff = i8f_cutoff(*s_max, p.q_w[qi]);
			} else {
				float qn = 0.0f;
				for (uint32_t t = 0; t < p.dim / 16; ++t)
					qn = __builtin_fmaf(q[16 * t], q[16 * t], qn);
				qn = reduce16_ref_order(qn);
				const float bmax = p.bn_max[0];
				cutoff = key_score(keys[p.k - 1]) + p.prune_eps * (qn + 1.5f * bmax) +
				         p.prune_abs * (__builtin_sqrtf(qn) + __builtin_sqrtf(bmax));
			}
			uint32_t cnt = 0;
			for (uint32_t i = tid; i < c; i += kBlock)
				cnt += key_score(keys[i]) <= cutoff ? 1u : 0u;
			uint32_t* s_cnt = reinterpret_cast<uint32_t*>(keys + p.cap);
			if (tid == 0)
				*s_cnt = 0;
			__syncthreads();
			if (cnt)
				atomicAdd(s_cnt, cnt);
			__syncthreads();
			n_rescore = *s_cnt;
			__syncthreads();
		}
		uint32_t n2r = 2;
		while (n2r < n_rescore)
			n2r <<= 1;
		for (uint32_t i0 = 0; i0 < n2r; i0 += kBlock / 16) {
			const uint32_t i = i0 + grp;
			const bool live = i < n_rescore;
			const uint32_t row = live ? key_idx(keys[i]) : 0u;
			const TR* r = (const TR*)p.rerank_base + (size_t)row * p.dim + l;
			float acc = 0.0f;
			for (uint32_t t = 0; t < p.dim / 16; ++t) {
				if (p.metric_ip) {
					acc = ref_dot<TR>(q[16 * t], r[16 * t], acc);
				} else {
					const float diff = ref_diff<TR>(q[16 * t], r[16 * t]);
					acc = __builtin_fmaf(diff, diff, acc);
				}
			}
			acc = reduce16_ref_order(acc);
			__syncthreads();
			if (l == 0 && i < n2r)
				keys[i] = live ? make_key(p.metric_ip ? -acc : acc, row) : kSentinelKey;
		}
		__syncthreads();
		n2 = n2r;
	}
	bitonic(n2);
	for (uint32_t i = tid; i < p.k; i += kBlock) {
		const uint64_t key = i < n2 ? keys[i] : kSentinelKey;
		const bool ok = key != kSentinelKey;
		if (p.out_ids)
			p.out_ids[(size_t)qo * p.k + i] = ok ? (uint64_t)key_idx(key) + p.id_offset : ~0ull;
		if (p.out_dists)
			p.out_dists[(size_t)qo * p.k + i] = ok ? key_score(key) : __builtin_inff();
	}
	if (tid == 0) {
		const uint64_t key = (p.k - 1 < n2) ? keys[p.k - 1] : kSentinelKey;
		spec_check(p, qo, key != kSentinelKey, key_score(key));
	}
	if (tid == 0 && p.tau_out) {
		const uint64_t key = (p.k - 1 < n2) ? keys[p.k - 1] : kSentinelKey;
		p.tau_out[qi] = key != kSentinelKey ? key_score(key)
		                                    : (p.tau_prev ? p.tau_prev[qi] : __builtin_inff());
		if (p.tau_row_out)
			p.tau_row_out[qi] = key != kSentinelKey
			                        ? key_idx(key)
			                        : (p.tau_row_prev ? p.tau_row_prev[qi] : 0xFFFFFFFFu);
	}
}

__global__ __launch_bounds__(1024) void max_f32_kernel(const float* in, size_t n, float* out) {
	__shared__ float red[16];
	float m = -__builtin_inff();
	for (size_t i = threadIdx.x; i < n; i += 1024)
		m = in[i] > m ? in[i] : m;
	for (int off = 32; off > 0; off >>= 1) {
		const float o = __shfl_xor(m, off);
		m = o > m ? o : m;
	}
	if ((threadIdx.x & 63) == 0)
		red[threadIdx.x >> 6] = m;
	__syncthreads();
	if (threadIdx.x == 0) {
		for (int w = 1; w < 16; ++w)
			m = red[w] > m ? red[w] : m;
		out[0] = m;
	}
}

template <bool STAGE>
__global__ __launch_bounds__(kWave) void merge_topk_kernel(const uint64_t* in_ids, const float* in_dists,
                                                            size_t ids_stride, size_t dists_stride,
                                                            uint32_t n_lists, uint32_t m, uint32_t k,
                                                            uint64_t* out_ids, float* out_dists) {
	extern __shared__ __attribute__((aligned(16))) unsigned char merge_smem[];
	const uint32_t qi = blockIdx.x, lane = threadIdx.x;
	if (qi >= m)
		return;
	const uint32_t total = n_lists * k;
	uint64_t* const s_id = reinterpret_cast<uint64_t*>(merge_smem);
	uint32_t* const s_sc = reinterpret_cast<uint32_t*>(merge_smem + 8 * (size_t)total);
	const size_t qoff = (size_t)qi * k;
	auto load = [&](uint32_t g, uint32_t i, uint64_t& id, uint32_t& sc) {
		if (STAGE) {
			id = s_id[g * k + i];
			sc = s_sc[g * k + i];
		} else {
			id = in_ids[g * ids_stride + qoff + i];
			sc = id == ~0ull ? 0xFFFFFFFFu : float_to_ordered(in_dists[g * dists_stride + qoff + i]);
		}
	};
	uint32_t n_valid = 0;
	if (STAGE) {
		for (uint32_t e = lane; e < total; e += kWave) {
			const uint32_t g = e / k, i = e - g * k;
			const uint64_t id = in_ids[g * ids_stride + qoff + i];
			s_id[e] = id;
			s_sc[e] = id == ~0ull ? 0xFFFFFFFFu : float_to_ordered(in_dists[g * dists_stride + qoff + i]);
		}
		__syncthreads();
	}
	for (uint32_t e = lane; e < total; e += kWave) {
		const uint32_t g = e / k, i = e - g * k;
		uint64_t id;
		uint32_t sc;
		load(g, i, id, sc);
		if (id == ~0ull)
			continue;
		n_valid++;
		uint32_t rank = i;
		for (uint32_t g2 = 0; g2 < n_lists && rank < k; ++g2) {
			if (g2 == g)
				continue;
			uint32_t lo = 0, hi = k - rank;
			while (lo < hi) {
				const uint32_t mid = (lo + hi) >> 1;
				uint64_t xid;
				uint32_t xsc;
				load(g2, mid, xid, xsc);
				const bool before = xsc < sc || (xsc == sc && (xid < id || (xid == id && g2 < g)));
				if (before)
					lo = mid + 1;
				else
					hi = mid;
			}
			rank += lo;
		}
		if (rank < k) {
			out_ids[qoff + rank] = id;
			out_dists[qoff + rank] = ordered_to_float(sc);
		}
	}
	for (int off = 32; off > 0; off >>= 1)
		n_valid += __shfl_xor(n_valid, off);
	for (uint32_t r = n_valid + lane; r < k; r += kWave) {
		out_ids[qoff + r] = ~0ull;
		out_dists[qoff + r] = __builtin_inff();
	}
}

}
```

Measured before the change: 6.595 million queries/s.

## Add two-round exact rerank to cut rows re-scored in select

Rerank in select now runs in two rounds. It first re-scores the ~16 candidates with the smallest int8 bounds exactly, then uses the k-th exact distance to derive a tighter cutoff, and re-scores only the remaining candidates that pass it. The goal is fewer fp32 row reads and dot products per query in the select stage. To support this, the int8 scan log now carries a per-row bound so the candidate key can be computed without an extra gather, and the redo path stores tau. The cost is more wave-level selection logic and two serial rescore phases, plus optional counting stats.

```diff
diff --git a/expann_amd/csrc/expann_hip.hip b/expann_amd/csrc/expann_hip.hip
--- a/expann_amd/csrc/expann_hip.hip
+++ b/expann_amd/csrc/expann_hip.hip
@@ -78,6 +78,7 @@
 	DevPtr<float> d_tau[2];
 	DevPtr<float> d_tau_s;
 	GrowPtr<void> d_redo;
+	GrowPtr<void> d_rerank;
 	DevPtr<uint32_t> d_tau_row[2];
 	size_t m_alloc = 0;
 	DevPtr<uint32_t> d_overflow;
@@ -168,10 +169,13 @@
 	long opt_spec_rank = 0;
 	long opt_redo_bound = 1;
 	long opt_select_overlap = 1;
+	long opt_rerank_rounds = 2;
+	long opt_rerank_stats = 0;
 	hipStream_t side_stream = nullptr;
 	hipEvent_t side_ev[2] = {nullptr, nullptr};
 	uint64_t stat_redo_queries = 0;
 	uint64_t stat_redo_candidates = 0;
+	uint64_t stat_rerank_rows = 0;
 	uint64_t stat_redo_overflows = 0;
 	uint64_t stat_spec_rank = 0;
 	long opt_i8_filter = 1;
@@ -795,9 +799,13 @@
 void launch_select_wave(SelectParams& sel, size_t m, uint32_t cap, hipStream_t st, uint32_t longest, bool rows_f16 = false,
                         hipStream_t side = nullptr) {
 	using WaveFn = void (*)(SelectParams, uint32_t);
-	const WaveFn w8 = rows_f16 ? select_wave_kernel<8, 4, _Float16> : select_wave_kernel<8, 4>;
-	const WaveFn w16 = rows_f16 ? select_wave_kernel<16, 2, _Float16> : select_wave_kernel<16, 2>;
-	const WaveFn w32 = rows_f16 ? select_wave_kernel<32, 1, _Float16> : select_wave_kernel<32, 1>;
+	const bool two = sel.tau_f != nullptr;
+	const WaveFn w8 = rows_f16 ? select_wave_kernel<8, 4, _Float16>
+	                           : (two ? select_wave_kernel<8, 4, float, true> : select_wave_kernel<8, 4>);
+	const WaveFn w16 = rows_f16 ? select_wave_kernel<16, 2, _Float16>
+	                            : (two ? select_wave_kernel<16, 2, float, true> : select_wave_kernel<16, 2>);
+	const WaveFn w32 = rows_f16 ? select_wave_kernel<32, 1, _Float16>
+	                            : (two ? select_wave_kernel<32, 1, float, true> : select_wave_kernel<32, 1>);
 	const hipStream_t st2 = side ? side : st;
 	sel.wave_done = 0;
 	hipLaunchKernelGGL(w8, dim3((uint32_t)((m + 3) / 4)), dim3(256), 0, st, sel, (uint32_t)m);
@@ -814,7 +822,9 @@
 	}
 }
 using SelectTopkFn = void (*)(SelectParams);
-inline SelectTopkFn select_topk_fn(const expann_index* h) {
+inline SelectTopkFn select_topk_fn(const expann_index* h, const SelectParams& sel) {
+	if (sel.tau_f)
+		return select_topk_kernel<float, true>;
 	return f16_rows(h) ? select_topk_kernel<_Float16> : select_topk_kernel<float>;
 }
 int launch_select(expann_index* h, SelectParams& sel, size_t m, uint32_t cap, hipStream_t st, uint32_t longest,
@@ -834,7 +844,7 @@
 	if (sum_counts)
 		hipLaunchKernelGGL(sum_u32_kernel, dim3(1), dim3(1024), 0, st2, sel.cand_cnt, (uint32_t)m, h->d_total);
 	launch_select_wave(sel, m, cap, st, longest, f16_rows(h), side);
-	hipLaunchKernelGGL(select_topk_fn(h), dim3((uint32_t)m), dim3(kBlock), sizeof(uint64_t) * cap + 16, st2, sel);
+	hipLaunchKernelGGL(select_topk_fn(h, sel), dim3((uint32_t)m), dim3(kBlock), sizeof(uint64_t) * cap + 16, st2, sel);
 	HIP_TRY(h, hipGetLastError());
 	if (side) {
 		HIP_TRY(h, hipEventRecord(h->side_ev[1], side));
@@ -1741,7 +1751,7 @@
 }
 
 struct RedoWs {
-	size_t list, cnt, theta, qnrm, wq, thp, bound, q16, q8, cand, total;
+	size_t list, cnt, theta, qnrm, wq, thp, bound, tau, q16, q8, cand, total;
 	RedoWs(uint32_t R, int dim, uint32_t cap) {
 		list = 0;
 		cnt = 4 * (size_t)R;
@@ -1750,7 +1760,8 @@
 		wq = 16 * (size_t)R;
 		thp = 20 * (size_t)R;
 		bound = 24 * (size_t)R;
-		q16 = 28 * (size_t)R;
+		tau = 28 * (size_t)R;
+		q16 = 32 * (size_t)R;
 		q8 = q16 + 2 * (size_t)R * (size_t)dim;
 		cand = q8 + (size_t)R * (size_t)dim;
 		total = cand + 8 * (size_t)R * (size_t)cap;
@@ -1799,6 +1810,7 @@
 	uint32_t spec_j = 0;
 	bool spec_off = false;
 	uint32_t redo_slots = 0;
+	bool rerank_counted = false;
 
 	enum Next { kDone, kRestart, kRetry };
 	int choose_kernels();
@@ -2201,6 +2213,17 @@
 		sel.prune_abs = 0.0f;
 		sel.row_w = h->d_rw_i8f;
 		sel.q_w = h->d_i8f_q + 2 * h->i8f_q_m;
+		if (h->opt_rerank_rounds != 1) {
+			sel.tau_f = spec_j ? (const float*)h->d_tau_s : (const float*)h->d_tau[levels.size() & 1];
+			sel.inv_2s2 = h->i8f.inv_2s2;
+		}
+	}
+	rerank_counted = false;
+	if (last && sel.rerank_base && h->opt_rerank_stats) {
+		HIP_TRY(h, grow_ws(h, h->d_rerank, 16 + sizeof(uint32_t) * m));
+		HIP_TRY(h, hipMemsetAsync(h->d_rerank, 0, 16 + sizeof(uint32_t) * m, st));
+		sel.rerank_cnt = reinterpret_cast<uint32_t*>(h->d_rerank.as<unsigned char>() + 16);
+		rerank_counted = true;
 	}
 	sel.overflow = h->d_overflow;
 	if (last && spec_j) {
@@ -2223,7 +2246,7 @@
 			hipLaunchKernelGGL(sum_u32_kernel, dim3(1), dim3(1024), 0, st, sel.cand_cnt, (uint32_t)m, h->d_total);
 		if (m <= 64)
 			sel.wave0_short = 1;
-		hipLaunchKernelGGL(select_topk_fn(h), dim3((uint32_t)m), dim3(kBlock), sizeof(uint64_t) * cap + 16, st, sel);
+		hipLaunchKernelGGL(select_topk_fn(h, sel), dim3((uint32_t)m), dim3(kBlock), sizeof(uint64_t) * cap + 16, st, sel);
 		HIP_TRY(h, hipGetLastError());
 	}
 	if (last && spec_j)
@@ -2261,6 +2284,7 @@
 		cp.i8_wq_in = h->d_i8f_q + h->i8f_q_m;
 		cp.r_thp = reinterpret_cast<int*>(b + ws.thp);
 		cp.r_wq = reinterpret_cast<float*>(b + ws.wq);
+		cp.r_tau = reinterpret_cast<float*>(b + ws.tau);
 		cp.i8_inv_2s2 = h->i8f.inv_2s2;
 	}
 	hipLaunchKernelGGL(redo_compact_kernel, dim3(R / (kBlock / 64)), dim3(kBlock), 0, st, cp);
@@ -2363,6 +2387,10 @@
 	if (use_i8f) {
 		sel.row_w = h->d_rw_i8f;
 		sel.q_w = cp.r_wq;
+		if (h->opt_rerank_rounds != 1) {
+			sel.tau_f = cp.r_tau;
+			sel.inv_2s2 = h->i8f.inv_2s2;
+		}
 	} else {
 		sel.prune_eps = pr * gemm_f16_filter_eps(h->dim);
 		sel.prune_abs = pr * std::ldexp(1.0f, -24) / h->f16_scale * std::sqrt((float)h->dim);
@@ -2372,14 +2400,27 @@
 	sel.slot_map = cp.list;
 	sel.live_slots = word;
 	sel.redo_cand = h->d_overflow + 6;
-	hipLaunchKernelGGL(select_topk_fn(h), dim3(R), dim3(kBlock), sizeof(uint64_t) * cap + 16, st, sel);
+	if (rerank_counted)
+		sel.rerank_cnt = reinterpret_cast<uint32_t*>(h->d_rerank.as<unsigned char>() + 16);
+	hipLaunchKernelGGL(select_topk_fn(h, sel), dim3(R), dim3(kBlock), sizeof(uint64_t) * cap + 16, st, sel);
 	HIP_TRY(h, hipGetLastError());
 	return EXPANN_OK;
 }
 
 int SearchPass::check(int attempt, Next* next) {
 	*next = kDone;
+	uint64_t reranked = 0;
+	if (rerank_counted) {
+		unsigned long long* const total = h->d_rerank.as<unsigned long long>();
+		hipLaunchKernelGGL(sum_u32_kernel, dim3(1), dim3(1024), 0, st, reinterpret_cast<const uint32_t*>(total + 2),
+		                   (uint32_t)m, total);
+		unsigned long long v = 0;
+		HIP_TRY(h, hipMemcpyAsync(&v, total, sizeof(v), hipMemcpyDeviceToHost, st));
+		HIP_TRY(h, hipStreamSynchronize(st));
+		reranked = v;
+	}
 	if (defer_flags(h, st, attempt)) {
+		h->stat_rerank_rows += reranked;
 		float sc = gvf ? h->f16_scale : 0.0f;
 		uint32_t* const slot = h->h_flag_ring + kRingWords * (h->async_pending - 1);
 		std::memcpy(&slot[kRingScale], &sc, sizeof(float));
@@ -2424,6 +2465,7 @@
 	if (h->h_flags[0] == 0 && redo_word < kRedoOverflowUnit) {
 		h->stat_redo_queries += redo_word;
 		h->stat_redo_candidates += spec_j ? h->h_flags[6] : 0u;
+		h->stat_rerank_rows += reranked;
 		return EXPANN_OK;
 	}
 	h->prof.retries++;
@@ -2660,6 +2702,8 @@
 		h->opt_redo_bound = std::atol(e);
 	if (const char* e = std::getenv("EXPANN_SELECT_OVERLAP"))
 		h->opt_select_overlap = std::atol(e);
+	if (const char* e = std::getenv("EXPANN_RERANK_ROUNDS"))
+		h->opt_rerank_rounds = std::atol(e) == 1 ? 1 : 2;
 	if (const char* e = std::getenv("EXPANN_I8_FILTER"))
 		h->opt_i8_filter = std::min(2L, std::max(0L, std::atol(e)));
 	if (hipSetDevice(device) != hipSuccess || hipStreamCreate(&h->stream) != hipSuccess) {
@@ -2670,6 +2714,8 @@
 	if (hipFuncSetAttribute((const void*)select_topk_kernel<float>, hipFuncAttributeMaxDynamicSharedMemorySize,
 	                        (int)(sizeof(uint64_t) * kMaxCap + 16)) != hipSuccess ||
 	    hipFuncSetAttribute((const void*)select_topk_kernel<_Float16>, hipFuncAttributeMaxDynamicSharedMemorySize,
+	                        (int)(sizeof(uint64_t) * kMaxCap + 16)) != hipSuccess ||
+	    hipFuncSetAttribute((const void*)select_topk_kernel<float, true>, hipFuncAttributeMaxDynamicSharedMemorySize,
 	                        (int)(sizeof(uint64_t) * kMaxCap + 16)) != hipSuccess) {
 		g_create_error = "hipFuncSetAttribute(select_topk_kernel) failed";
 		hipStreamDestroy(h->stream);
@@ -2895,6 +2941,7 @@
 	const size_t qbytes = (size_t)h->dim * h->q_elem;
 	h->stat_redo_queries = 0;
 	h->stat_redo_candidates = 0;
+	h->stat_rerank_rows = 0;
 	for (size_t q0 = 0; q0 < m; q0 += kMaxQueriesPerPass) {
 		const size_t mm = std::min(kMaxQueriesPerPass, m - q0);
 		int rc = search_pass(h, (const char*)d_queries + q0 * qbytes, mm, k, d_ids + q0 * k,
@@ -3205,6 +3252,8 @@
 		*out = h->stat_redo_overflows;
 	else if (!std::strcmp(name, "spec_rank"))
 		*out = h->stat_spec_rank;
+	else if (!std::strcmp(name, "rerank_rows"))
+		*out = h->stat_rerank_rows;
 	else if (!std::strcmp(name, "base_bytes"))
 		*out = h->d_base ? (uint64_t)h->n * (uint64_t)h->dim * h->elem : 0;
 	else if (!std::strcmp(name, "filter_active"))
@@ -3326,6 +3375,10 @@
 		h->opt_redo_bound = value;
 	else if (!std::strcmp(name, "select_overlap"))
 		h->opt_select_overlap = value;
+	else if (!std::strcmp(name, "rerank_rounds"))
+		h->opt_rerank_rounds = value == 1 ? 1 : 2;
+	else if (!std::strcmp(name, "rerank_stats"))
+		h->opt_rerank_stats = value ? 1 : 0;
 	else if (!std::strcmp(name, "ip_rescale"))
 		h->opt_ip_rescale = value;
 	else if (!std::strcmp(name, "sample_pass"))
diff --git a/expann_amd/csrc/scan_gemm_f16.hpp b/expann_amd/csrc/scan_gemm_f16.hpp
--- a/expann_amd/csrc/scan_gemm_f16.hpp
+++ b/expann_amd/csrc/scan_gemm_f16.hpp
@@ -339,8 +339,9 @@
 			if (slot < p.cap) {
 				uint64_t key;
 				if (p.i_mode == 3) {
-					const float kappa = (float)(p.i_bias[e.y] - (int)e.x);
-					key = make_key(p.i_rw[e.y] < __builtin_inff() ? kappa : -__builtin_inff(), e.y);
+					const int bp = (int)e.w;
+					const float kappa = (float)(bp - (int)e.x);
+					key = make_key(bp > kI8fBpMin && bp < kI8fBpMax ? kappa : -__builtin_inff(), e.y);
 				} else if (p.i_mode) {
 					const int dot = (int)e.x - p.i_thp[e.z];
 					const int score = p.i_mode == 1 ? p.i_bias[e.y] - 2 * dot + p.i_qself[e.z] : -dot;
@@ -550,6 +551,7 @@
 	const float* i8_wq_in;
 	int* r_thp;
 	float* r_wq;
+	float* r_tau;
 	double i8_inv_2s2;
 };
 __global__ __launch_bounds__(kBlock) void redo_compact_kernel(RedoCompactParams p) {
@@ -586,6 +588,7 @@
 		if (p.q8) {
 			p.r_thp[s] = (-2147483647 - 1) / 2;
 			p.r_wq[s] = __builtin_inff();
+			p.r_tau[s] = __builtin_inff();
 		}
 		return;
 	}
@@ -595,8 +598,10 @@
 	p.r_qnrm[s] = qn;
 	p.r_theta[s] = p.ip ? (2.0f * tau_f + qn * p.eps + p.abs_coef * __builtin_sqrtf(qn)) * p.mul
 	                    : (tau_f - (qn * (1.0f - p.eps) - p.abs_coef * __builtin_sqrtf(qn))) * p.mul;
-	if (p.q8)
+	if (p.q8) {
 		i8f_thresholds(p.i8_aq[qi], p.i8_wq_in[qi], tau, p.i8_inv_2s2, p.r_thp + s, p.r_wq + s);
-}
-
-}
+		p.r_tau[s] = tau;
+	}
+}
+
+}
diff --git a/expann_amd/csrc/scan_gemm_i8w.hpp b/expann_amd/csrc/scan_gemm_i8w.hpp
--- a/expann_amd/csrc/scan_gemm_i8w.hpp
+++ b/expann_amd/csrc/scan_gemm_i8w.hpp
@@ -176,7 +176,7 @@
 				const uint32_t pos = glog_n + __builtin_amdgcn_mbcnt_hi((uint32_t)(mask >> 32),
 				                                                        __builtin_amdgcn_mbcnt_lo((uint32_t)mask, 0u));
 				if (hit[u] && pos < pw.log_cap)
-					my_log[pos] = make_uint4((uint32_t)cv[u], row[u], qi[u], 0u);
+					my_log[pos] = make_uint4((uint32_t)cv[u], row[u], qi[u], (uint32_t)queue[(base + 64 * u + lane) >> 4].bp);
 				glog_n += (uint32_t)__builtin_popcountll(mask);
 			}
 		}
diff --git a/expann_amd/csrc/select.hpp b/expann_amd/csrc/select.hpp
--- a/expann_amd/csrc/select.hpp
+++ b/expann_amd/csrc/select.hpp
@@ -29,6 +29,9 @@
 	const float* qnrm;
 	const float* row_w;
 	const float* q_w;
+	const float* tau_f;
+	double inv_2s2;
+	uint32_t* rerank_cnt;
 	const float* spec_tau;
 	uint32_t* redo_word;
 	uint32_t* redo_list;
@@ -60,6 +63,16 @@
 __device__ inline uint32_t i8f_upper_ord(const SelectParams& p, uint64_t key) {
 	const float v = key_score(key) + p.row_w[key_idx(key)];
 	return float_to_ordered(v == v ? v : __builtin_inff());
+}
+
+__device__ inline float i8f_round2_cut(float t, float tau_f, double inv_2s2) {
+	const double x = ((double)t - (double)tau_f) * inv_2s2;
+	const double xu = x + (__builtin_fabs(x) * 0x1p-40 + 0x1p-10);
+	float f = (float)xu;
+	if ((double)f < xu)
+		f = f == 0.0f ? __builtin_bit_cast(float, 1u)
+		              : __builtin_bit_cast(float, __builtin_bit_cast(uint32_t, f) + (f > 0.0f ? 1u : 0xFFFFFFFFu));
+	return f;
 }
 
 __global__ __launch_bounds__(1024) void sum_u32_kernel(const uint32_t* in, uint32_t n,
@@ -234,7 +247,7 @@
 	return make_uint2(wave_kth_largest_u32<1>(w, k), j ? wave_kth_largest_u32<1>(w, j) : 0u);
 }
 
-template <int PER, typename TR = float>
+template <int PER, typename TR = float, bool TWO = false>
 __device__ inline void select_wave_body(const SelectParams& p, uint32_t qi, uint32_t c, uint64_t* list,
                                         int lane) {
 	const uint64_t* src = p.cand + (size_t)qi * p.cap;
@@ -247,7 +260,7 @@
 	const float* q = p.rerank_queries + (size_t)qo * p.dim + l;
 	float cutoff = __builtin_inff();
 	const bool final_scores = p.rerank_base == nullptr;
-	if ((p.prune_eps > 0.0f || final_scores || p.row_w) && c > p.k) {
+	if (!TWO && (p.prune_eps > 0.0f || final_scores || p.row_w) && c > p.k) {
 		float qn = 0.0f;
 		if (final_scores || p.row_w) {
 		} else if (p.qnrm) {
@@ -289,63 +302,155 @@
 		}
 	}
 	uint32_t n_s = 0;
-#pragma unroll
-	for (int j = 0; j < PER; ++j) {
-		const bool hit = lane + 64 * j < (int)c && key_score(kk[j]) <= cutoff;
-		const unsigned long long mask = __builtin_amdgcn_ballot_w64(hit);
-		const uint32_t pos = n_s + __builtin_amdgcn_mbcnt_hi((uint32_t)(mask >> 32),
-		                                                      __builtin_amdgcn_mbcnt_lo((uint32_t)mask, 0u));
-		if (hit)
-			list[pos] = kk[j];
-		n_s += (uint32_t)__builtin_popcountll(mask);
-	}
-	asm volatile("s_waitcnt lgkmcnt(0)" ::: "memory");
-	for (uint32_t i0 = 0; p.rerank_base && i0 < n_s; i0 += 16) {
-		constexpr int U = 4;
-		float acc[U];
-		uint32_t row[U];
-		const TR* r[U];
-#pragma unroll
-		for (int u = 0; u < U; ++u) {
-			const uint32_t i = i0 + 4 * u + grp;
-			row[u] = key_idx(list[i < n_s ? i : 0]);
-			r[u] = (const TR*)p.rerank_base + (size_t)row[u] * p.dim + l;
-			acc[u] = 0.0f;
-		}
-		const uint32_t nt = p.dim / 16;
-		for (uint32_t t0 = 0; t0 < nt; t0 += 8) {
-			float qv[8];
-			TR rv[U][8];
-#pragma unroll
-			for (int t = 0; t < 8; ++t)
-				qv[t] = t0 + t < nt ? q[16 * (t0 + t)] : 0.0f;
-#pragma unroll
-			for (int u = 0; u < U; ++u)
-#pragma unroll
-				for (int t = 0; t < 8; ++t)
-					rv[u][t] = t0 + t < nt ? r[u][16 * (t0 + t)] : (TR)0.0f;
-#pragma unroll
-			for (int u = 0; u < U; ++u)
-#pragma unroll
-				for (int t = 0; t < 8; ++t) {
-					if (t0 + t >= nt)
-						continue;
-					if (p.metric_ip) {
-						acc[u] = ref_dot<TR>(qv[t], rv[u][t], acc[u]);
-					} else {
-						const float diff = ref_diff<TR>(qv[t], rv[u][t]);
-						acc[u] = __builtin_fmaf(diff, diff, acc[u]);
+	uint32_t n1 = 0;
+	if (TWO) {
+		const uint32_t r1 = p.k <= 16 ? 16u : (p.k + 15u) & ~15u;
+		if (c > r1 && p.q_w[qi] < __builtin_inff()) {
+			uint32_t sc[PER];
+#pragma unroll
+			for (int j = 0; j < PER; ++j)
+				sc[j] = (uint32_t)(kk[j] >> 32);
+			uint32_t v = 0xFFFFFFFFu;
+			if (p.k > 24) {
+				v = wave_kth_smallest_u32<PER>(sc, r1);
+			} else {
+				for (uint32_t cnt = 0; cnt < r1;) {
+					uint32_t mn = sc[0];
+#pragma unroll
+					for (int j = 1; j < PER; ++j)
+						mn = min(mn, sc[j]);
+					mn = wave_min_u32(mn);
+					if (mn == 0xFFFFFFFFu)
+						break;
+					v = mn;
+#pragma unroll
+					for (int j = 0; j < PER; ++j) {
+						const bool eq = sc[j] == mn;
+						cnt += (uint32_t)__builtin_popcountll(__builtin_amdgcn_ballot_w64(eq));
+						sc[j] = eq ? 0xFFFFFFFFu : sc[j];
 					}
 				}
-		}
-#pragma unroll
-		for (int u = 0; u < U; ++u) {
-			acc[u] = reduce16_ref_order(acc[u]);
-			const uint32_t i = i0 + 4 * u + grp;
-			if (l == 0 && i < n_s)
-				list[i] = make_key(p.metric_ip ? -acc[u] : acc[u], row[u]);
-		}
-	}
+			}
+#pragma unroll
+			for (int j = 0; j < PER; ++j) {
+				const bool hit = lane + 64 * j < (int)c && (uint32_t)(kk[j] >> 32) <= v;
+				const unsigned long long mask = __builtin_amdgcn_ballot_w64(hit);
+				const uint32_t pos = n1 + __builtin_amdgcn_mbcnt_hi((uint32_t)(mask >> 32),
+				                                                     __builtin_amdgcn_mbcnt_lo((uint32_t)mask, 0u));
+				if (hit)
+					list[pos] = kk[j];
+				n1 += (uint32_t)__builtin_popcountll(mask);
+			}
+			uint32_t n_o = n1;
+#pragma unroll
+			for (int j = 0; j < PER; ++j) {
+				const bool hit = lane + 64 * j < (int)c && (uint32_t)(kk[j] >> 32) > v;
+				const unsigned long long mask = __builtin_amdgcn_ballot_w64(hit);
+				const uint32_t pos = n_o + __builtin_amdgcn_mbcnt_hi((uint32_t)(mask >> 32),
+				                                                      __builtin_amdgcn_mbcnt_lo((uint32_t)mask, 0u));
+				if (hit)
+					list[pos] = kk[j];
+				n_o += (uint32_t)__builtin_popcountll(mask);
+			}
+			n_s = n1;
+		}
+	}
+	if (!TWO || n1 == 0) {
+		n_s = 0;
+#pragma unroll
+		for (int j = 0; j < PER; ++j) {
+			const bool hit = lane + 64 * j < (int)c && key_score(kk[j]) <= cutoff;
+			const unsigned long long mask = __builtin_amdgcn_ballot_w64(hit);
+			const uint32_t pos = n_s + __builtin_amdgcn_mbcnt_hi((uint32_t)(mask >> 32),
+			                                                      __builtin_amdgcn_mbcnt_lo((uint32_t)mask, 0u));
+			if (hit)
+				list[pos] = kk[j];
+			n_s += (uint32_t)__builtin_popcountll(mask);
+		}
+	}
+	asm volatile("s_waitcnt lgkmcnt(0)" ::: "memory");
+	auto rescore = [&](uint32_t begin) {
+		for (uint32_t i0 = begin; p.rerank_base && i0 < n_s; i0 += 16) {
+			constexpr int U = 4;
+			float acc[U];
+			uint32_t row[U];
+			const TR* r[U];
+#pragma unroll
+			for (int u = 0; u < U; ++u) {
+				const uint32_t i = i0 + 4 * u + grp;
+				row[u] = key_idx(list[i < n_s ? i : 0]);
+				r[u] = (const TR*)p.rerank_base + (size_t)row[u] * p.dim + l;
+				acc[u] = 0.0f;
+			}
+			const uint32_t nt = p.dim / 16;
+			for (uint32_t t0 = 0; t0 < nt; t0 += 8) {
+				float qv[8];
+				TR rv[U][8];
+#pragma unroll
+				for (int t = 0; t < 8; ++t)
+					qv[t] = t0 + t < nt ? q[16 * (t0 + t)] : 0.0f;
+#pragma unroll
+				for (int u = 0; u < U; ++u)
+#pragma unroll
+					for (int t = 0; t < 8; ++t)
+						rv[u][t] = t0 + t < nt ? r[u][16 * (t0 + t)] : (TR)0.0f;
+#pragma unroll
+				for (int u = 0; u < U; ++u)
+#pragma unroll
+					for (int t = 0; t < 8; ++t) {
+						if (t0 + t >= nt)
+							continue;
+						if (p.metric_ip) {
+							acc[u] = ref_dot<TR>(qv[t], rv[u][t], acc[u]);
+						} else {
+							const float diff = ref_diff<TR>(qv[t], rv[u][t]);
+							acc[u] = __builtin_fmaf(diff, diff, acc[u]);
+						}
+					}
+			}
+#pragma unroll
+			for (int u = 0; u < U; ++u) {
+				acc[u] = reduce16_ref_order(acc[u]);
+				const uint32_t i = i0 + 4 * u + grp;
+				if (l == 0 && i < n_s)
+					list[i] = make_key(p.metric_ip ? -acc[u] : acc[u], row[u]);
+			}
+		}
+	};
+	rescore(0);
+	if (TWO && n1 != 0) {
+		asm volatile("s_waitcnt lgkmcnt(0)" ::: "memory");
+		uint32_t t_ord;
+		if (n1 <= 64) {
+			const uint32_t w[1] = {lane < (int)n1 ? (uint32_t)(list[lane] >> 32) : 0xFFFFFFFFu};
+			t_ord = wave_kth_smallest_u32<1>(w, p.k);
+		} else {
+			uint32_t w[PER];
+#pragma unroll
+			for (int j = 0; j < PER; ++j)
+				w[j] = lane + 64 * j < (int)n1 ? (uint32_t)(list[lane + 64 * j] >> 32) : 0xFFFFFFFFu;
+			t_ord = wave_kth_smallest_u32<PER>(w, p.k);
+		}
+		float cut = __builtin_inff();
+		if (t_ord < 0xFF800000u)
+			cut = i8f_round2_cut(ordered_to_float(t_ord), p.tau_f[qi], p.inv_2s2);
+		for (uint32_t i0 = n1; i0 < c; i0 += 64) {
+			const uint32_t i = i0 + lane;
+			const uint64_t key = list[i < c ? i : 0];
+			const bool hit = i < c && !(key_score(key) > cut);
+			const unsigned long long mask = __builtin_amdgcn_ballot_w64(hit);
+			const uint32_t pos = n_s + __builtin_amdgcn_mbcnt_hi((uint32_t)(mask >> 32),
+			                                                      __builtin_amdgcn_mbcnt_lo((uint32_t)mask, 0u));
+			asm volatile("s_waitcnt lgkmcnt(0)" ::: "memory");
+			if (hit)
+				list[pos] = key;
+			n_s += (uint32_t)__builtin_popcountll(mask);
+		}
+		asm volatile("s_waitcnt lgkmcnt(0)" ::: "memory");
+		rescore(n1);
+	}
+	if (p.rerank_cnt && p.rerank_base && lane == 0)
+		p.rerank_cnt[qo] = (p.slot_map ? p.rerank_cnt[qo] : 0u) + n_s;
 	asm volatile("s_waitcnt lgkmcnt(0)" ::: "memory");
 	if (n_s <= 256)
 		wave_emit_sorted<(PER < 4 ? PER : 4)>(p, list, n_s, qo, lane);
@@ -353,7 +458,7 @@
 		wave_emit_sorted<PER>(p, list, n_s, qo, lane);
 }
 
-template <int PER, int WAVES, typename TR = float>
+template <int PER, int WAVES, typename TR = float, bool TWO = false>
 __global__ __launch_bounds__(64 * WAVES) void select_wave_kernel(SelectParams p, uint32_t m) {
 	constexpr uint32_t kSelectWaveMax = 64 * PER;
 	__shared__ uint64_t lists[WAVES][kSelectWaveMax];
@@ -365,10 +470,10 @@
 	const uint32_t c = p.cand_cnt ? p.cand_cnt[qi] : p.fixed_count;
 	if (c > kSelectWaveMax || c > p.cap || (c <= p.wave_done && p.wave_done != 0))
 		return;
-	select_wave_body<PER, TR>(p, qi, c, lists[wave], lane);
-}
-
-template <typename TR>
+	select_wave_body<PER, TR, TWO>(p, qi, c, lists[wave], lane);
+}
+
+template <typename TR, bool TWO = false>
 __global__ __launch_bounds__(kBlock) void select_topk_kernel(SelectParams p) {
 	extern __shared__ __attribute__((aligned(16))) unsigned char smem_raw[];
 	uint64_t* keys = reinterpret_cast<uint64_t*>(smem_raw);
@@ -385,9 +490,9 @@
 	if (p.wave0_short && c <= 2048 && c <= p.cap && 8 * (size_t)p.cap >= 16384) {
 		if (tid < 64) {
 			if (c <= 512)
-				select_wave_body<8, TR>(p, qi, c, keys, (int)tid);
+				select_wave_body<8, TR, TWO>(p, qi, c, keys, (int)tid);
 			else
-				select_wave_body<32, TR>(p, qi, c, keys, (int)tid);
+				select_wave_body<32, TR, TWO>(p, qi, c, keys, (int)tid);
 		}
 		return;
 	}
@@ -461,6 +566,8 @@
 			n_rescore = *s_cnt;
 			__syncthreads();
 		}
+		if (p.rerank_cnt && tid == 0)
+			p.rerank_cnt[qo] = (p.slot_map ? p.rerank_cnt[qo] : 0u) + n_rescore;
 		uint32_t n2r = 2;
 		while (n2r < n_rescore)
 			n2r <<= 1;
diff --git a/profiles/rerank_rounds_model.py b/profiles/rerank_rounds_model.py
--- /dev/null
+++ b/profiles/rerank_rounds_model.py
@@ -0,0 +1,57 @@
+import numpy as np
+
+N, D, M, K, J, FRAC = 1_000_000, 128, 256, 10, 4, 16
+rng = np.random.RandomState(0)
+base = rng.standard_normal((N, D)).astype(np.float32)
+queries = rng.standard_normal((M, D)).astype(np.float32)
+
+rms = float(np.sqrt(np.mean(base.astype(np.float64) ** 2)))
+s = min(float(np.abs(base).max()), 5.5 * rms) / 127.0
+lam = 1.4 * s / (np.sqrt(12.0) * rms)
+eps = (D / 8.0 + 16.0) * 2.0 ** -24
+c = 1.0 + 1.0 / lam
+
+
+def quant(x):
+    return np.clip(np.rint(x / s), -127, 127).astype(np.float32)
+
+
+bq, qq = quant(base), quant(queries)
+n_b = (base.astype(np.float64) ** 2).sum(1)
+v_b = ((base - s * bq).astype(np.float64) ** 2).sum(1)
+n_q = (queries.astype(np.float64) ** 2).sum(1)
+v_q = ((queries - s * qq).astype(np.float64) ** 2).sum(1)
+big_b = np.sqrt(n_b.max())
+m_q = np.minimum(2.0 * big_b * np.sqrt(v_q), v_q / lam)
+a_b = n_b * (1.0 - lam - eps) - c * v_b
+w_b = (2.0 * (lam + eps) * n_b + 2.0 * c * v_b) / (2.0 * s * s)
+a_q = n_q * (1.0 - lam - eps) - m_q - v_q
+w_q = (2.0 * (lam + eps) * n_q + 2.0 * m_q + 2.0 * v_q) / (2.0 * s * s) + 4.0
+
+out = {name: [] for name in ("list", "cut", "two_kappa", "two_upper", "two_k")}
+for i in range(M):
+    S = n_q[i] + n_b - 2.0 * (base @ queries[i]).astype(np.float64)
+    L = a_q[i] + a_b - 2.0 * s * s * (bq @ qq[i]).astype(np.float64)
+    tau = np.sort(S[::FRAC])[J - 1]
+    cand = np.nonzero(L <= tau)[0]
+    kappa = (L[cand] - tau) / (2.0 * s * s)
+    upper = kappa + w_b[cand]
+    out["list"].append(len(cand))
+    if len(cand) <= K:
+        for name in ("cut", "two_kappa", "two_upper", "two_k"):
+            out[name].append(len(cand))
+        continue
+    out["cut"].append(int((kappa <= np.sort(upper)[K - 1] + w_q[i]).sum()))
+    for name, order, r1 in (("two_kappa", kappa, 16), ("two_upper", upper, 16), ("two_k", kappa, K)):
+        first = np.argsort(order, kind="stable")[:r1]
+        T = np.sort(S[cand[first]])[K - 1]
+        rest = np.ones(len(cand), bool)
+        rest[first] = False
+        out[name].append(len(first) + int((rest & (tau + 2.0 * s * s * kappa <= T)).sum()))
+print(f"rms {rms:.4f}  s {s:.5f}  lambda {lam:.5f}  c {c:.1f}")
+for name, what in (("list", "list length per query"), ("cut", "rows kept by the single cut"),
+                   ("two_kappa", "two rounds, first round the 16 smallest kappa"),
+                   ("two_upper", "two rounds, first round the 16 smallest upper bounds"),
+                   ("two_k", "two rounds, first round of only k = 10 rows")):
+    v = np.array(out[name])
+    print(f"{what:55s} mean {v.mean():7.1f}  p99 {np.percentile(v, 99):7.1f}")
diff --git a/profiles/rerank_rows_c2.py b/profiles/rerank_rows_c2.py
--- /dev/null
+++ b/profiles/rerank_rows_c2.py
@@ -0,0 +1,34 @@
+import os
+import sys
+
+import numpy as np
+import torch
+
+sys.path.insert(0, os.path.join(os.path.dirname(os.path.abspath(__file__)), ".."))
+from expann_amd import GpuBruteForceEngine
+
+n, d, m, k = 1_000_000, 128, 10_000, 10
+dev = torch.device("cuda", 0)
+g = torch.Generator(device=dev)
+g.manual_seed(1234)
+base = torch.randn(n, d, device=dev, dtype=torch.float32, generator=g).cpu().numpy()
+g.manual_seed(4321)
+queries = torch.randn(m, d, device=dev, dtype=torch.float32, generator=g).cpu().numpy()
+res = {}
+for rounds in (2, 1):
+    eng = GpuBruteForceEngine(d, "l2")
+    eng.store_many_vectors(base)
+    eng.build()
+    eng.set_option("rerank_rounds", rounds)
+    eng.set_option("rerank_stats", 1)
+    eng.set_profiling(True)
+    ids, dists = eng.query_k_batch(queries, k)
+    prof = eng.get_profile()
+    rows = eng.get_stat("rerank_rows")
+    print(f"rerank_rounds {rounds}: {prof['scan_kernel']}, spec_rank {eng.get_stat('spec_rank')}, redo_queries "
+          f"{eng.get_stat('redo_queries')}, {prof['candidates'] / m:.1f} candidates per query, "
+          f"{rows / m:.1f} rows re-scored per query ({rows} in all), retries {prof['retries']}")
+    res[rounds] = (ids, dists, rows)
+    eng.close()
+assert np.array_equal(res[1][0], res[2][0]) and np.array_equal(res[1][1].view(np.uint32), res[2][1].view(np.uint32))
+print(f"same ids and distance bits; rows re-scored, two rounds / one: {res[2][2] / max(1, res[1][2]):.3f}")
```

Result: faster. 6.935 million queries/s, median of 6 (+5.2%).
